# brunohs1993/Nanokappa

Measured on AMD Instinct MI355X. Metric: phonon-steps/sec (whole node), higher is better.
Workload: dtype f64

## Files before the change

nanokappa_amd/csrc/nk_device.h:

```cpp
#pragma once
#include <hip/hip_runtime.h>
#include <stdint.h>

#define NK_WG 256
#ifndef NK_NREP
#define NK_NREP 8
#endif
#define NK_PLANE_DOUBLES 6
#define NK_FACE_DOUBLES 16
#define NK_LDS_FACES 256
#define NK_LDS_RESFACES 64
#define NK_TAU_ROWS 3
#define NK_MAX_SEGMENTS 16384
#define NK_EMIT_CHUNK 128
#define NK_LREC 128
#define NK_NEWBORN 0x80000000u
#define NK_LOST 0x40000000u

#define NK_TAG_REFLECT 0x00000u
#define NK_TAG_EMIT 0x10000u
#define NK_TAG_RESAMP 0x20000u
#define NK_TAG_DICE 0x30000u
#define NK_TAG_INIT 0x40000u

// ... 8 lines not shown
    __host__ __device__ __forceinline__ explicit operator bool() const { return p != nullptr; }
};

template <bool NTS, bool PID>
struct NkBlock {
    static constexpr int NF = 4 + (NTS ? 1 : 0) + (PID ? 1 : 0);
    static constexpr int BD = NF * 64 + 32;
    static constexpr int O_Y = 64, O_Z = 128, O_OCC = 192, O_NTS = 256, O_PID = 64 * (NTS ? 5 : 4), O_W0 = 64 * NF;
    static __device__ __forceinline__ double *slot(double *s0, int64_t i) { return s0 + (i >> 6) * (int64_t)BD + (i & 63); }
    static __device__ __forceinline__ double *tile(double *s0, int64_t i0, int lane) { return s0 + (i0 >> 6) * (int64_t)BD + lane; }
    static __device__ __forceinline__ uint32_t *word(double *s0, int64_t i) { return reinterpret_cast<uint32_t *>(s0 + (i >> 6) * (int64_t)BD + O_W0) + (i & 63); }
};

struct __attribute__((aligned(16))) NkFacet {
    double cx, cy, cz;
    double nx, ny, nz;
    double tx, ty, tz;
    int32_t bc;
    int32_t partner;
    int32_t res;
    int32_t rough;
    int32_t pad[2];
};

struct __attribute__((aligned(64))) NkMode {
    double omega, vx, vy, vz;
    double E0;
    double tau[NK_TAU_ROWS];
};

struct NkDev {
    int32_t Q, J, NT, M;
    const NkMode *modetab;
    const NkMode *modetab_p;
    const int32_t *m2s;
    const int32_t *s2m;
    const int32_t *seg_nl;
    int32_t tau_row0;
    double tau_g[NK_TAU_ROWS];
    double tau_ig[NK_TAU_ROWS - 1];
    double T0, invT0;
    double c_hk;
    const double *tau;
    const double *Tgrid;
    int32_t nE;
    const double *Tarr, *Earr;
    double Tfill_lo, Tfill_hi;
    double hbar, kb, QV;
    double active_modes;
    int32_t F, Fc, NP;
    const float *tree_boxes;
    double tree_bound;
    const int32_t *tree_tags;
    const double *facet_skip;
    const double *tree_faces;
    int32_t tree_base[8];
    int32_t tree_top, tree_leaves;
    int32_t tree_nfam, tree_lds_fam0, tree_lds_off;
    int32_t NG;
    const double *planes;
    const double *faces;
    const NkFacet *facets;
    double tol;
    double bbox[6];
    int32_t box;
    double box_k[6];
    uint64_t box_ids;
    double inv_dt;
    const double *face_verts;
    const int32_t *facet_face_off;
    const int32_t *facet_face_idx;
    const double *facet_face_cdf;
    int32_t nS;
    const double *simplex_pts;
    const double *simplex_cdf;
    int32_t S, sv_kind, sv_axis, sv_interp;
    const double *centers;
    const double *sv_volume;
    double sv_lo, sv_invL;
    double *T_sv;
    const double *rbf_inv;
    int32_t rbf_P, rbf_used[3];
    double rbf_shift[3], rbf_scale[3];
    int32_t R, res_gen;
    const int32_t *res_facet;
    const double *res_T;
    const int32_t *res_face_off;
    const double *res_face_cdf;
    const double *res_face_verts;
    int32_t res_nf;
    int32_t res_lds;
    const double *enter_prob;
    double *res_counter;
    const double *ep_p;
    double *rc_p;
    int64_t rc_len;
    const double *res_roulette;
    int32_t *nleave_prev;
    uint64_t *sp_inbox;
    int32_t *sp_inbox_n;
    int32_t sp_icap;
    int32_t Fr;
    const double *specularity;
    const uint8_t *true_spec;
    const int32_t *spec_map;
    const double *roulette;
    const int32_t *roul_lut;
    int32_t roul_nlut;
    const int32_t *degen_j2;
    double dt;
    int32_t norm_fixed, T_ref_local;
    double particle_density, T_ref;
    uint64_t seed;
    int32_t rank, nranks;
    int64_t cap;
    int32_t nseg, segcap;
    int32_t *seg_count;
    int32_t *seg_new;
    int32_t *seg_lo;
    int32_t down;
    int32_t *seg_bound;
    NkField<double> x, y, z, occ, nts;
    NkField<uint32_t> w0;
    NkField<uint64_t> pid;
    int32_t part;
    int32_t lb;
    int32_t nlmax;
    int32_t nlrec;
    int32_t *ticket;
    int32_t *overflow;
    int32_t *halt;
    double *qx, *qy, *qz, *qocc, *qnts;
    uint32_t *qw0;
    uint64_t *qpid;
    int32_t *seg_evq;
    int32_t *ev_ticket;
    double2 *mig_buf;
    int32_t *mig_n;
    int32_t mig_cap;
    double *partials;
    int32_t NB;
    unsigned long long *stamps;
};

struct NkSlot { int64_t od, ow; };
__device__ __forceinline__ NkSlot nk_slot(const NkDev &d, int64_t i) {
    const int64_t b = i >> 6, l = i & 63;
    NkSlot s;
    s.od = b * (int64_t)d.x.blk + l;
    s.ow = b * (int64_t)d.w0.blk + l;
    return s;
}

__device__ __forceinline__ void nk_philox(uint32_t c0, uint32_t c1, uint32_t c2, uint32_t c3, uint32_t k0, uint32_t k1,
                                          uint32_t o[4]) {
#pragma unroll
    for (int r = 0; r < 10; ++r) {
        uint32_t hi0 = __umulhi(0xD2511F53u, c0), lo0 = 0xD2511F53u * c0;
        uint32_t hi1 = __umulhi(0xCD9E8D57u, c2), lo1 = 0xCD9E8D57u * c2;
        uint32_t n0 = hi1 ^ c1 ^ k0, n2 = hi0 ^ c3 ^ k1;
        c0 = n0; c1 = lo1; c2 = n2; c3 = lo0;
        k0 += 0x9E3779B9u; k1 += 0xBB67AE85u;
    }
    o[0] = c0; o[1] = c1; o[2] = c2; o[3] = c3;
}
__device__ __forceinline__ double nk_u53(uint32_t hi, uint32_t lo) {
    uint64_t w = ((uint64_t)hi << 32) | lo;
    return (double)(w >> 11) * (1.0 / 9007199254740992.0);
}
__device__ __forceinline__ void nk_uniform2_dev(uint64_t seed, uint64_t pid, uint32_t step, uint32_t tag, double &u0,
                                                double &u1) {
    uint32_t o[4];
    nk_philox((uint32_t)pid, (uint32_t)(pid >> 32), step, tag, (uint32_t)seed, (uint32_t)(seed >> 32), o);
    u0 = nk_u53(o[0], o[1]);
    u1 = nk_u53(o[2], o[3]);
}

__device__ __forceinline__ int nk_ss_left(const double *a, int n, double x) {
    int lo = 0, hi = n;
    while (lo < hi) { int mid = (lo + hi) >> 1; if (a[mid] < x) lo = mid + 1; else hi = mid; }
    return lo;
}
__device__ __forceinline__ int nk_ss_right(const double *a, int n, double x) {
    int lo = 0, hi = n;
    while (lo < hi) { int mid = (lo + hi) >> 1; if (a[mid] <= x) lo = mid + 1; else hi = mid; }
    return lo;
}
__device__ __forceinline__ int nk_ss_left_hint(const double *a, int n, double x, int hint) {
    int lo, hi;
    hint = hint < 0 ? 0 : (hint > n - 1 ? n - 1 : hint);
    if (a[hint] < x) {
        int stepw = 1;
        lo = hint + 1; hi = lo;
        while (hi < n && a[hi] < x) { lo = hi + 1; hi += stepw; stepw <<= 1; }
        if (hi > n) hi = n;
    } else {
        int stepw = 1;
        hi = hint; lo = hint;
        while (lo > 0 && !(a[lo - 1] < x)) { hi = lo - 1; lo -= stepw; stepw <<= 1; if (lo < 0) lo = 0; }
        if (lo > 0 && !(a[lo - 1] < x)) lo = 0;
    }
    while (lo < hi) { int mid = (lo + hi) >> 1; if (a[mid] < x) lo = mid + 1; else hi = mid; }
    return lo;
}
__device__ __forceinline__ double nk_interp_lin_hint(const double *xs, const double *ys, int n, double x, int hint, int &idx_out) {
    int idx = nk_ss_left_hint(xs, n, x, hint);
    idx_out = idx;
    idx = idx < 1 ? 1 : (idx > n - 1 ? n - 1 : idx);
    double xlo = xs[idx - 1], xhi = xs[idx], ylo = ys[idx - 1], yhi = ys[idx];
    return (yhi - ylo) / (xhi - xlo) * (x - xlo) + ylo;
}
__device__ __forceinline__ double nk_rcp(double x) {
    double y = __builtin_amdgcn_rcp(x);
    double e = __builtin_fma(-x, y, 1.0);
    y = __builtin_fma(y, e, y);
    e = __builtin_fma(-x, y, 1.0);
    return __builtin_fma(y, e, y);
}
__device__ __forceinline__ double nk_fma_c(double p, double r, double c) {
    double o;
    asm("v_fma_f64 %0, %1, %2, %3" : "=v"(o) : "v"(p), "v"(r), "v"(c));
    return o;
}
__device__ __forceinline__ double nk_exp(double x) {
    const double k = __builtin_rint(x * 1.4426950408889634);
    double r = __builtin_fma(-k, 6.93147180369123816490e-01, x);
    r = __builtin_fma(-k, 1.90821492927058770002e-10, r);
    double p = 1.6059043836821613e-10;
    p = nk_fma_c(p, r, 2.08767569878681e-09);
    p = nk_fma_c(p, r, 2.505210838544172e-08);
    p = nk_fma_c(p, r, 2.755731922398589e-07);
    p = nk_fma_c(p, r, 2.7557319223985893e-06);
    p = nk_fma_c(p, r, 2.48015873015873e-05);
    p = nk_fma_c(p, r, 1.984126984126984e-04);
    p = nk_fma_c(p, r, 0.001388888888888889);
    p = nk_fma_c(p, r, 0.008333333333333333);
    p = nk_fma_c(p, r, 0.041666666666666664);
    p = nk_fma_c(p, r, 0.16666666666666666);
    p = __builtin_fma(p, r, 0.5);
    p = __builtin_fma(p, r, 1.0);
    p = __builtin_fma(p, r, 1.0);
    const double kc = k < -2000.0 ? -2000.0 : (k > 2000.0 ? 2000.0 : k);
    return __builtin_ldexp(p, (int)kc);
}
__device__ __forceinline__ double nk_exp_small(double dl) {
    double p = 2.755731922398589e-07;
    p = nk_fma_c(p, dl, 2.7557319223985893e-06);
    p = nk_fma_c(p, dl, 2.48015873015873e-05);
    p = nk_fma_c(p, dl, 1.984126984126984e-04);
    p = nk_fma_c(p, dl, 0.001388888888888889);
    p = nk_fma_c(p, dl, 0.008333333333333333);
    p = nk_fma_c(p, dl, 0.041666666666666664);
    p = nk_fma_c(p, dl, 0.16666666666666666);
    p = __builtin_fma(p, dl, 0.5);
    p = __builtin_fma(p, dl, 1.0);
    p = __builtin_fma(p, dl, 1.0);
    return p;
}
__device__ __forceinline__ double nk_be(double a, double E0, double invT, double invT0) {
    if (!(a > 0.0) || !(invT > 0.0)) return 0.0;
    const double dl = a * (invT - invT0);
    double em1;
    if (fabs(dl) < 0.125) em1 = __builtin_fma(E0, nk_exp_small(dl), -1.0);
    else {
        const double xx = a * invT;
        if (!(xx < 700.0)) return 0.0;
        em1 = nk_exp(xx) - 1.0;
    }
    return nk_rcp(em1);
}
__device__ __forceinline__ double nk_occupation(const NkDev &d, double T, double omega, double E0) {
    if (!(T > 0.0) || !(omega > 0.0)) return 0.0;
    return nk_be(omega * d.c_hk, E0, 1.0 / T, d.invT0);
}
__device__ __forceinline__ double nk_interp_lin(const double *xs, const double *ys, int n, double x) {
    int idx = nk_ss_left(xs, n, x);
    idx = idx < 1 ? 1 : (idx > n - 1 ? n - 1 : idx);
    double xlo = xs[idx - 1], xhi = xs[idx], ylo = ys[idx - 1], yhi = ys[idx];
    return (yhi - ylo) / (xhi - xlo) * (x - xlo) + ylo;
}
__device__ __forceinline__ double nk_T_of_E(const NkDev &d, double E) {
    if (E < d.Earr[0]) return d.Tfill_lo;
    if (E > d.Earr[d.nE - 1]) return d.Tfill_hi;
    return nk_interp_lin(d.Earr, d.Tarr, d.nE, E);
}
__device__ __forceinline__ double nk_E_of_T(const NkDev &d, double T) {
    if (T < d.Tarr[0]) return d.Earr[0];
    if (T > d.Tarr[d.nE - 1]) return d.Earr[d.nE - 1];
    return nk_interp_lin(d.Tarr, d.Earr, d.nE, T);
}
struct NkTauWin {
    double g0, g1, g2, i0, i1;
    __device__ __forceinline__ void load(const NkDev &d, bool park) {
        g0 = d.tau_g[0]; g1 = d.tau_g[1]; g2 = d.tau_g[2]; i0 = d.tau_ig[0]; i1 = d.tau_ig[1];
        if (park) asm volatile("" : "+v"(g0), "+v"(g1), "+v"(g2), "+v"(i0), "+v"(i1));
    }
};
template <class SegModes>
__device__ __forceinline__ double nk_lifetime(const NkDev &d, const NkTauWin &w, double ta, double tb, double tc, double T, const SegModes &sm, int idx) {
    if (T > w.g0 && T <= w.g2) {
        const bool b = T > w.g1;
        const double glo = b ? w.g1 : w.g0;
        const double ig = b ? w.i1 : w.i0;
        const double t0 = b ? tb : ta, t1 = b ? tc : tb;
        const double y = (T - glo) * ig;
        return t0 * (1.0 - y) + t1 * y;
    }
    const int NT = d.NT;
    const double *g = d.Tgrid;
    if (!(T >= g[0]) || !(T <= g[NT - 1])) return __builtin_nan("");
    int i = (int)((T - g[0]) / (g[1] - g[0]));
    i = i < 0 ? 0 : (i > NT - 1 ? NT - 1 : i);
    while (i < NT && g[i] < T) ++i;
    while (i > 0 && g[i - 1] >= T) --i;
    i -= 1;
    i = i < 0 ? 0 : (i > NT - 2 ? NT - 2 : i);
    const double y = (T - g[i]) / (g[i + 1] - g[i]);
    const int mode = sm.mode(idx);
    const double t0 = d.tau[(int64_t)i * d.M + mode];
    const double t1 = d.tau[(int64_t)(i + 1) * d.M + mode];
    return t0 * (1.0 - y) + t1 * y;
}

struct __attribute__((aligned(16))) NkSv { double c, T, slope, invT; };
struct NkSvTab {
    const double *cen;
// ... 544 lines not shown
```

nanokappa_amd/csrc/nk_engine.hip:

```cpp
#include <hip/hip_runtime.h>
#include <dlfcn.h>
#include <math.h>
#include <stdio.h>
#include <stdlib.h>
#include <string.h>
#include <algorithm>
#include <functional>
#include <queue>
#include <string>
#include <type_traits>
#include <chrono>
#include <time.h>
#include <vector>

#include <rccl/rccl.h>

#include "../../include/nanokappa_hip.h"
#include "nk_kernels.h"
#include "nk_field.h"
#include "nk_fgroups.h"
#include "nk_modes.h"
#include "nk_group.h"
#ifndef NK_PLAIN_IN_ENGINE
extern template __global__ void k_sweep<1, false, false, false, false, true, 1>(NkDev, uint32_t, int, int);
extern template __global__ void k_sweep<1, false, false, false, false, true, 2>(NkDev, uint32_t, int, int);
extern template __global__ void k_sweep<1, false, false, false, false, false, 1>(NkDev, uint32_t, int, int);
extern template __global__ void k_sweep<1, false, false, false, false, false, 2>(NkDev, uint32_t, int, int);
extern template __global__ void k_sweep<1, false, false, false, false, true, 1, true>(NkDev, uint32_t, int, int);
extern template __global__ void k_sweep<1, false, false, false, false, true, 2, true>(NkDev, uint32_t, int, int);
extern template __global__ void k_sweep<1, false, false, false, false, false, 1, true>(NkDev, uint32_t, int, int);
extern template __global__ void k_sweep<1, false, false, false, false, false, 2, true>(NkDev, uint32_t, int, int);
#endif

struct NkRccl {
    void *lib = nullptr;
    ncclResult_t (*GetUniqueId)(ncclUniqueId *) = nullptr;
    ncclResult_t (*CommInitRank)(ncclComm_t *, int, ncclUniqueId, int) = nullptr;
    ncclResult_t (*AllReduce)(const void *, void *, size_t, ncclDataType_t, ncclRedOp_t, ncclComm_t, hipStream_t) = nullptr;
    ncclResult_t (*CommDestroy)(ncclComm_t) = nullptr;
    ncclResult_t (*CommCount)(const ncclComm_t, int *) = nullptr;
    ncclResult_t (*CommUserRank)(const ncclComm_t, int *) = nullptr;
    ncclResult_t (*CommAbort)(ncclComm_t) = nullptr;
};

static thread_local std::string g_create_error;

struct nk_ctx {
    int device = 0;
    hipStream_t stream = nullptr;
    std::string err;
    NkDev d;
    std::vector<void *> allocs;
    std::vector<void *> pallocs;
    void *store_buf = nullptr;
    size_t store_pad = 0;
    bool store_pid = false;
    bool store_nts = true;
    bool mesh_box = false;
    bool box_forbidden = false;
    int32_t *anomalies = nullptr;
    bool have_material = false, have_mesh = false, have_sv = false, have_params = false;
    int64_t step = 0;
    bool pending_relax = false;
    int g_sweep = 0;
    std::vector<int32_t> h_seg_count;
    std::vector<hipEvent_t> evpool;
    int g_sweep_key = -1;
    size_t g_sweep_lds = 0;
    int layout_key = -1;
    std::vector<double> h_enter_prob;
    int64_t spec_M = 0;
    double *spec_v = nullptr, *spec_om = nullptr, *spec_dl = nullptr, *spec_svx = nullptr;
    int32_t *spec_rank = nullptr;
    double spec_vmax = 0.0;
    NkSpecMode *spec_modes = nullptr;
    int32_t *spec_in = nullptr, *spec_out = nullptr;
    unsigned long long *spec_count = nullptr;
    double *ks_kv = nullptr, *ks_mat = nullptr;
    double ks_tol[3] = {0, 0, 0};
    int64_t ks_Q = 0;
    int64_t spec_cap = 0;
    int64_t spec_last = 0;
    int rb_Fr = 0;
    double *rb_k2 = nullptr, *rb_nin = nullptr, *rb_eta = nullptr, *rb_sub = nullptr, *rb_spec = nullptr, *rb_roul = nullptr;
    uint8_t *rb_ts = nullptr;
    unsigned int *rb_map = nullptr;
    std::vector<int32_t> rb_facet;
    int64_t o2o_first = 0;
    bool stepped = false;
    int64_t emitted_for = -1;
    std::vector<double> h_vg;
    std::vector<int32_t> h_m2s, h_s2m;
    int32_t *m2s_dev = nullptr, *s2m_dev = nullptr, *nl_dev = nullptr;
    unsigned int *rbar = nullptr;
    bool walked = false;
    int64_t ev_lds_set = -1;
    int map_nseg = 0;
    NkMode *modetab_p = nullptr;
    int64_t modetab_p_len = 0;
    void *inbox = nullptr, *inbox_n = nullptr;
    void *mig_buf = nullptr, *mig_n = nullptr;
    double *ep_p = nullptr, *rc_p = nullptr;
    int rm_nseg = 0, rm_nlmax = 0;
    void *pin = nullptr;
    size_t pin_bytes = 0;
    int32_t halt_words[4] = {0, 0, 0, 0};
    double *acc = nullptr;
    double *hist = nullptr;
    int hist_cap = 0;
    nk_params params;
    nk_timing timing;
    NkRccl rccl;
    ncclComm_t comm = nullptr;
    int comm_rank = -1, comm_nranks = 0;
    double comm_selftest = 0.0;
    int num_cu = 256;
    std::vector<int32_t> h_ffo, h_ffi;
    std::vector<double> h_fcdf, h_verts;
    std::vector<double> h_rbf_inv;
    std::vector<NkFacet> host_facets;
    const double *d_omega = nullptr, *d_vg = nullptr;
    std::vector<double> h_Tgrid;
    double T_lo = 0.0, T_hi = 0.0;
    int32_t band_B = 0;
    int32_t *band_map = nullptr;
    double *band_slabs = nullptr;
    size_t band_slabs_n = 0;
    double *band_rows_d = nullptr;
    size_t band_rows_n = 0;
    std::vector<double> band_rows;
    std::vector<int64_t> band_steps;
    NkFieldHost field;
    NkFGroupsHost fgroups;
    int64_t map_gen = 0;
    NkModesHost modes;
    double res_T_max = 0.0;
};

#define NK_HIP(call)                                                                                   \
    do {                                                                                               \
        hipError_t e_ = (call);                                                                        \
        if (e_ != hipSuccess) {                                                                        \
            ctx->err = std::string(#call) + ": " + hipGetErrorString(e_);                              \
            return NK_ERR_HIP;                                                                         \
        }                                                                                              \
    } while (0)
#define NK_ARG(cond, msg)                                                                              \
    do {                                                                                               \
        if (!(cond)) { ctx->err = msg; return NK_ERR_ARG; }                                            \
    } while (0)

template <class T>
static int nk_upload(nk_ctx *ctx, const T *src, size_t n, const T **dst, bool particle = false) {
    void *p = nullptr;
    size_t bytes = (n ? n : 1) * sizeof(T);
    NK_HIP(hipMalloc(&p, bytes));
    (particle ? ctx->pallocs : ctx->allocs).push_back(p);
    if (src && n) NK_HIP(hipMemcpy(p, src, n * sizeof(T), hipMemcpyHostToDevice));
    else NK_HIP(hipMemset(p, 0, bytes));
    *dst = (const T *)p;
    return NK_OK;
}
#define NK_UP(src, n, dst)                                                                             \
    do { int rc_ = nk_upload(ctx, src, n, dst); if (rc_) return rc_; } while (0)

static inline bool nk_layout_soa() { return false; }
static inline int nk_particle_bytes(bool with_pid, bool with_nts) { return 36 + (with_nts ? 8 : 0) + (with_pid ? 8 : 0); }
static inline size_t nk_store_bytes(int64_t cap, bool with_pid, bool with_nts) {
    const int64_t nblk = (cap + 63) / 64;
    const int nf = 4 + (with_nts ? 1 : 0) + (with_pid ? 1 : 0);
    const int bd = nf * 64 + 32;
    const size_t bytes = nk_layout_soa() ? (size_t)nblk * 64 * (nf * 8 + 4) : (size_t)nblk * bd * 8;
    return bytes ? bytes : 64;
}
static void nk_point_fields(NkDev &d, double *b, int64_t cap, bool with_pid, bool with_nts) {
    const int64_t nblk = (cap + 63) / 64;
    const int nf = 4 + (with_nts ? 1 : 0) + (with_pid ? 1 : 0);
    const int bd = nf * 64 + 32;
    if (nk_layout_soa()) {
        const int64_t n = nblk * 64;
        int k = 4;
        d.x = {b, 64}; d.y = {b + n, 64}; d.z = {b + 2 * n, 64}; d.occ = {b + 3 * n, 64};
        d.nts = {with_nts ? b + (k++) * n : nullptr, 64};
        d.pid = {with_pid ? (uint64_t *)(b + (k++) * n) : nullptr, 64};
        d.w0 = {(uint32_t *)(b + k * n), 64};
    } else {
        int k = 4;
        d.x = {b, bd}; d.y = {b + 64, bd}; d.z = {b + 128, bd}; d.occ = {b + 192, bd};
        d.nts = {with_nts ? b + 64 * (k++) : nullptr, bd};
        d.pid = {with_pid ? (uint64_t *)(b + 64 * (k++)) : nullptr, bd};
        d.w0 = {(uint32_t *)(b + 64 * k), 2 * bd};
    }
}
static int nk_alloc_fields(nk_ctx *ctx, NkDev &d, int64_t cap, bool with_pid, bool with_nts) {
    const size_t bytes = nk_store_bytes(cap, with_pid, with_nts);
    void *buf = nullptr;
    const size_t pad = getenv("NK_STORE_PAD_KB") ? (size_t)atol(getenv("NK_STORE_PAD_KB")) * 1024 : 0;
    NK_HIP(hipMalloc(&buf, bytes + pad));
    ctx->pallocs.push_back(buf);
    NK_HIP(hipMemsetAsync(buf, 0, bytes + pad, ctx->stream));
    ctx->store_buf = buf; ctx->store_pad = pad; ctx->store_pid = with_pid; ctx->store_nts = with_nts;
    nk_point_fields(d, (double *)((char *)buf + pad), cap, with_pid, with_nts);
    return NK_OK;
}
template <class T>
static int nk_field_download(nk_ctx *ctx, const NkDev &d, const NkField<T> &f, std::vector<T> &out) {
    out.resize((size_t)d.cap);
    const int64_t nblk = d.cap / 64;
    if (nblk == 0) return NK_OK;
    NK_HIP(hipMemcpy2D(out.data(), 64 * sizeof(T), f.p, (size_t)f.blk * sizeof(T), 64 * sizeof(T), (size_t)nblk, hipMemcpyDeviceToHost));
    return NK_OK;
}
template <class T>
static int nk_field_upload(nk_ctx *ctx, const NkDev &d, const NkField<T> &f, const T *src) {
    const int64_t nblk = d.cap / 64;
    if (nblk == 0) return NK_OK;
    NK_HIP(hipMemcpy2D(f.p, (size_t)f.blk * sizeof(T), src, 64 * sizeof(T), 64 * sizeof(T), (size_t)nblk, hipMemcpyHostToDevice));
    return NK_OK;
}

static inline int nk_geom_mode(const nk_ctx *ctx) { return (ctx->d.F <= NK_LDS_FACES && ctx->d.Fc <= NK_LDS_FACES) ? 1 : 2; }
static inline bool nk_want_split(const nk_ctx *ctx);
static inline size_t nk_lds(const nk_ctx *ctx, bool geom, int kind = 0) {
    const NkDev &d = ctx->d;
    const int gm = geom ? nk_geom_mode(ctx) : 0;
    return nk_lds_bytes(d.S, d.R, d.F, d.NP, d.Fc, gm, kind, (gm == 1 && d.res_lds) ? d.res_nf : 0, d.rbf_P, d.nlrec, nk_want_split(ctx) ? 0 : 1);
}
#define NK_GEOM_LAUNCH(kernel, grid, lds, ...)                                                        \
    do {                                                                                               \
        if (nk_geom_mode(ctx) == 1) kernel<1><<<grid, NK_WG, lds, ctx->stream>>>(__VA_ARGS__);         \
        else kernel<2><<<grid, NK_WG, lds, ctx->stream>>>(__VA_ARGS__);                                \
    } while (0)
#define NK_EMIT_LAUNCH(kernel, grid, lds, ...)                                                        \
    do {                                                                                               \
        if (ctx->d.box) kernel<1, true><<<grid, NK_WG, lds, ctx->stream>>>(__VA_ARGS__);               \
        else if (nk_geom_mode(ctx) == 1) kernel<1, false><<<grid, NK_WG, lds, ctx->stream>>>(__VA_ARGS__);   \
        else kernel<2, false><<<grid, NK_WG, lds, ctx->stream>>>(__VA_ARGS__);                         \
    } while (0)
static inline int nk_sweep_grid(const nk_ctx *ctx) { return ctx->num_cu * 8; }
#define NK_SWEEP_CASE(G, R, B, P, S, lrec, STMT) { if (lrec) { auto KERNEL = k_sweep<G, R, B, P, S, true>; STMT; } else { auto KERNEL = k_sweep<G, R, B, P, S, false>; STMT; } }
#define NK_SWEEP_CASE_FAST(lrec, fast, STMT)                                                                                   \
    { if (lrec) { if ((fast) == 1) { auto KERNEL = k_sweep<1, false, false, false, false, true, 1>; STMT; } else { auto KERNEL = k_sweep<1, false, false, false, false, true, 2>; STMT; } } \
      else { if ((fast) == 1) { auto KERNEL = k_sweep<1, false, false, false, false, false, 1>; STMT; } else { auto KERNEL = k_sweep<1, false, false, false, false, false, 2>; STMT; } } }
#define NK_SWEEP_CASE_S(G, R, B, P, split, lrec, STMT) { if (split) NK_SWEEP_CASE(G, R, B, P, true, lrec, STMT) else NK_SWEEP_CASE(G, R, B, P, false, lrec, STMT) }
#define NK_SWEEP_CASE_RP(G, B, rough, pid, split, lrec, STMT)                                         \
    { if (rough) NK_SWEEP_CASE_S(G, true, B, true, split, lrec, STMT) else if (pid) NK_SWEEP_CASE_S(G, false, B, true, split, lrec, STMT) else NK_SWEEP_CASE_S(G, false, B, false, split, lrec, STMT) }
#define NK_SWEEP_CASE_BOX(R, B, P, lrec, STMT) { if (lrec) { auto KERNEL = k_sweep<1, R, B, P, false, true, 0, true>; STMT; } else { auto KERNEL = k_sweep<1, R, B, P, false, false, 0, true>; STMT; } }
#define NK_SWEEP_CASE_BOX_RP(B, rough, pid, lrec, STMT)                                               \
    { if (rough) NK_SWEEP_CASE_BOX(true, B, true, lrec, STMT) else if (pid) NK_SWEEP_CASE_BOX(false, B, true, lrec, STMT) else NK_SWEEP_CASE_BOX(false, B, false, lrec, STMT) }
#define NK_SWEEP_CASE_FAST_BOX(lrec, fast, STMT)                                                                               \
    { if (lrec) { if ((fast) == 1) { auto KERNEL = k_sweep<1, false, false, false, false, true, 1, true>; STMT; } else { auto KERNEL = k_sweep<1, false, false, false, false, true, 2, true>; STMT; } } \
      else { if ((fast) == 1) { auto KERNEL = k_sweep<1, false, false, false, false, false, 1, true>; STMT; } else { auto KERNEL = k_sweep<1, false, false, false, false, false, 2, true>; STMT; } } }
#define NK_SWEEP_DISPATCH(gm, rough, rbf, pid, split, lrec, STMT)                                     \
    do {                                                                                               \
        const int fast_ = ((gm) == 1 && !(rough) && !(rbf) && !(pid) && !(split)) ? nk_sweep_fast(ctx) : 0;   \
        if (ctx->d.box && (gm) == 1 && !(split)) {                                                     \
            if (fast_) { NK_SWEEP_CASE_FAST_BOX(lrec, fast_, STMT) break; }                            \
            if (rbf) NK_SWEEP_CASE_BOX_RP(true, rough, pid, lrec, STMT) else NK_SWEEP_CASE_BOX_RP(false, rough, pid, lrec, STMT)   \
            break;                                                                                     \
        }                                                                                              \
        if (fast_) { NK_SWEEP_CASE_FAST(lrec, fast_, STMT) break; }                                    \
        if ((gm) == 1) { if (rbf) NK_SWEEP_CASE_RP(1, true, rough, pid, split, lrec, STMT) else NK_SWEEP_CASE_RP(1, false, rough, pid, split, lrec, STMT) }   \
        else { if (rbf) NK_SWEEP_CASE_RP(2, true, rough, pid, split, lrec, STMT) else NK_SWEEP_CASE_RP(2, false, rough, pid, split, lrec, STMT) }             \
    } while (0)
static inline int nk_sweep_fast(const nk_ctx *ctx) {
    const NkDev &d = ctx->d;
    if (getenv("NK_NO_FAST")) return 0;
    return (d.sv_kind == 0 && d.T_ref_local && (d.sv_interp == 0 || d.sv_interp == 1)) ? 1 + d.sv_interp : 0;
}
static inline bool nk_want_lrec(const nk_ctx *ctx) { return ctx->d.nlrec > 0; }
#define NK_EVENTS_CASE(G, R, B, P, STMT) { auto KERNEL = k_events<G, R, B, P>; STMT; }
#define NK_EVENTS_CASE_RP(G, B, rough, pid, STMT)                                                     \
    { if (rough) NK_EVENTS_CASE(G, true, B, true, STMT) else if (pid) NK_EVENTS_CASE(G, false, B, true, STMT) else NK_EVENTS_CASE(G, false, B, false, STMT) }
#define NK_EVENTS_DISPATCH(gm, rough, rbf, pid, STMT)                                                 \
    do {                                                                                               \
        if ((gm) == 1) { if (rbf) NK_EVENTS_CASE_RP(1, true, rough, pid, STMT) else NK_EVENTS_CASE_RP(1, false, rough, pid, STMT) }   \
        else { if (rbf) NK_EVENTS_CASE_RP(2, true, rough, pid, STMT) else NK_EVENTS_CASE_RP(2, false, rough, pid, STMT) }             \
    } while (0)

static int nk_update_tau_window(nk_ctx *ctx, bool force) {
    NkDev &d = ctx->d;
    if (!ctx->have_material) return NK_OK;
    const std::vector<double> &g = ctx->h_Tgrid;
    const double Tm = 0.5 * (ctx->T_lo + ctx->T_hi);
    int i = (int)(std::lower_bound(g.begin(), g.end(), Tm) - g.begin()) - 1;
    if (i < 0) i = 0;
    int row0 = (i + 1 < d.NT && ctx->T_hi - g[std::min(i + 1, d.NT - 1)] > g[i] - ctx->T_lo) ? i : i - 1;
    if (row0 > d.NT - NK_TAU_ROWS) row0 = d.NT - NK_TAU_ROWS;
    if (row0 < 0) row0 = 0;
    const bool window_ok = d.tau_row0 >= 0 && ctx->T_lo > g[d.tau_row0] &&
                           ctx->T_hi <= g[std::min(d.tau_row0 + NK_TAU_ROWS - 1, d.NT - 1)];
    const bool window_best = d.tau_row0 == row0;
    const bool t0_ok = d.T0 > 0.0 && fabs(ctx->T_lo - d.T0) <= 0.02 * d.T0 && fabs(ctx->T_hi - d.T0) <= 0.02 * d.T0;
    const bool t0_best = d.T0 > 0.0 && fabs(Tm - d.T0) <= 0.002 * d.T0;
    if (!force && (window_ok || window_best) && (t0_ok || t0_best)) return NK_OK;
    d.T0 = Tm > 0.0 ? Tm : 300.0;
    d.invT0 = 1.0 / d.T0;
    d.c_hk = d.hbar / d.kb;
    NkMode *tp = nullptr;
    if (d.part && d.nseg > 0 && d.m2s) {
        const int64_t need = (int64_t)d.nseg * d.nlmax;
        if (need > ctx->modetab_p_len) {
            if (ctx->modetab_p) hipFree(ctx->modetab_p);
            ctx->modetab_p = nullptr; ctx->modetab_p_len = 0;
            NK_HIP(hipMalloc((void **)&ctx->modetab_p, (size_t)need * sizeof(NkMode)));
            NK_HIP(hipMemset(ctx->modetab_p, 0, (size_t)need * sizeof(NkMode)));
            ctx->modetab_p_len = need;
        }
        tp = ctx->modetab_p;
    }
    d.modetab_p = tp;
    k_build_modetab<<<(d.M + 255) / 256, 256, 0, ctx->stream>>>(ctx->d_omega, ctx->d_vg, d.tau, d.M, d.NT, row0, d.c_hk, d.invT0,
                                                                  d.nseg > 0 ? d.nseg : 1, d.nlmax, d.m2s, (NkMode *)d.modetab, tp);
    NK_HIP(hipGetLastError());
    d.tau_row0 = row0;
    ctx->timing.tau_rebuilds += 1;
    for (int k = 0; k < NK_TAU_ROWS; ++k) d.tau_g[k] = (row0 + k < d.NT) ? g[row0 + k] : INFINITY;
    for (int k = 0; k + 1 < NK_TAU_ROWS; ++k) d.tau_ig[k] = 1.0 / (d.tau_g[k + 1] - d.tau_g[k]);
    if (d.NT < NK_TAU_ROWS) d.tau_g[0] = INFINITY;
    return NK_OK;
}

static void nk_track_T(nk_ctx *ctx, const double *T, int S) {
    double lo = T[0], hi = T[0];
    for (int i = 1; i < S; ++i) { lo = std::min(lo, T[i]); hi = std::max(hi, T[i]); }
    ctx->T_lo = lo; ctx->T_hi = hi;
}

extern "C" {

const char *nk_last_error(const nk_ctx *ctx) { return ctx ? ctx->err.c_str() : g_create_error.c_str(); }

int nk_device_count(void) {
    int ndev = 0;
    return hipGetDeviceCount(&ndev) == hipSuccess ? ndev : 0;
}

int nk_create(nk_ctx **out, int device_id, uint64_t seed) {
    if (!out) { g_create_error = "nk_create: out is NULL"; return NK_ERR_ARG; }
    *out = nullptr;
    int ndev = 0;
    hipError_t e = hipGetDeviceCount(&ndev);
    if (e != hipSuccess || ndev <= 0) {
        g_create_error = std::string("nk_create: no HIP device available (") + hipGetErrorString(e) +
                         "); this library has no CPU fallback";
        return NK_ERR_NODEVICE;
    }
    if (device_id < 0 || device_id >= ndev) { g_create_error = "nk_create: device_id out of range"; return NK_ERR_ARG; }
    nk_ctx *ctx = new nk_ctx();
    memset(&ctx->d, 0, sizeof(NkDev));
    memset(&ctx->params, 0, sizeof(nk_params));
    memset(&ctx->timing, 0, sizeof(nk_timing));
    ctx->device = device_id;
    if ((e = hipSetDevice(device_id)) != hipSuccess || (e = hipStreamCreate(&ctx->stream)) != hipSuccess) {
        g_create_error = std::string("nk_create: ") + hipGetErrorString(e);
        delete ctx;
        return NK_ERR_HIP;
    }
    hipDeviceProp_t prop;
    if (hipGetDeviceProperties(&prop, device_id) == hipSuccess) {
        ctx->num_cu = prop.multiProcessorCount;
        if (strncmp(prop.gcnArchName, "gfx950", 6) != 0) {
            g_create_error = std::string("nk_create: device is ") + prop.gcnArchName + ", this build targets gfx950 only";
            hipStreamDestroy(ctx->stream);
            delete ctx;
            return NK_ERR_NODEVICE;
        }
    }
    ctx->d.seed = seed;
    ctx->d.rank = 0;
    ctx->d.nranks = 1;
    ctx->d.tau_row0 = -1;
    ctx->d.stamps = nullptr;
    ctx->params.dt = 1.0; ctx->params.T_ref_local = 1; ctx->params.flux_every = 10; ctx->params.contains_every = 100;
    ctx->d.dt = 1.0; ctx->d.inv_dt = 1.0; ctx->d.T_ref_local = 1;
    const int32_t *p32 = nullptr;
    int rc;
    if ((rc = nk_upload<int32_t>(ctx, nullptr, 16, &p32))) {
        g_create_error = ctx->err;
        delete ctx;
        return rc;
    }
    ctx->d.halt = (int32_t *)p32;
    ctx->d.overflow = (int32_t *)p32 + 4;
    ctx->d.ticket = (int32_t *)p32 + 5;
    ctx->d.ev_ticket = (int32_t *)p32 + 6;
    ctx->anomalies = (int32_t *)p32 + 7;
    *out = ctx;
    return NK_OK;
}
// ... 704 lines not shown
    NK_HIP(hipStreamSynchronize(ctx->stream));
    std::vector<int32_t> cnt((size_t)d.nseg);
    NK_HIP(hipMemcpy(cnt.data(), d.seg_count, (size_t)d.nseg * 4, hipMemcpyDeviceToHost));
    int64_t live = 0;
    for (int c : cnt) live += c;
    ctx->h_seg_count = cnt;
    if (!want_all) { h.x.resize((size_t)live); return NK_OK; }
    std::vector<double> bd;
    std::vector<uint32_t> bw;
    std::vector<uint64_t> bu;
    auto keep = [&](const auto &all, auto *dst) {
        for (int sgm = 0; sgm < d.nseg; ++sgm) {
            memcpy(dst, all.data() + (size_t)sgm * d.segcap, (size_t)cnt[sgm] * sizeof(*dst));
            dst += cnt[sgm];
        }
    };
    h.x.resize(live); h.y.resize(live); h.z.resize(live); h.occ.resize(live); h.nts.resize(live);
    h.mode.resize(live); h.facet.resize(live); h.pid.assign(live, 0);
    std::vector<uint32_t> w0((size_t)live);
    int rc;
    if ((rc = nk_field_download(ctx, d, d.x, bd))) return rc; keep(bd, h.x.data());
    if ((rc = nk_field_download(ctx, d, d.y, bd))) return rc; keep(bd, h.y.data());
    if ((rc = nk_field_download(ctx, d, d.z, bd))) return rc; keep(bd, h.z.data());
    if ((rc = nk_field_download(ctx, d, d.occ, bd))) return rc; keep(bd, h.occ.data());
    std::vector<int32_t> bfc;
    if (d.nts) { if ((rc = nk_field_download(ctx, d, d.nts, bd))) return rc; keep(bd, h.nts.data()); }
    else {
        if (ctx->have_material && ctx->have_mesh && ctx->have_sv && d.modetab) {
            double *dn = nullptr; int32_t *df = nullptr;
            NK_HIP(hipMalloc((void **)&dn, (size_t)d.cap * 8));
            if (hipMalloc((void **)&df, (size_t)d.cap * 4) != hipSuccess) { hipFree(dn); ctx->err = "nk_gather_live: out of memory"; return NK_ERR_HIP; }
            hipMemsetAsync(dn, 0, (size_t)d.cap * 8, ctx->stream); hipMemsetAsync(df, 0xff, (size_t)d.cap * 4, ctx->stream);
            k_next_hit<1><<<nk_sweep_grid(ctx), NK_WG, nk_lds(ctx, true), ctx->stream>>>(d, dn, df);
            bd.resize((size_t)d.cap); bfc.resize((size_t)d.cap);
            hipError_t e1 = hipGetLastError();
            if (e1 == hipSuccess) e1 = hipMemcpy(bd.data(), dn, (size_t)d.cap * 8, hipMemcpyDeviceToHost);
            if (e1 == hipSuccess) e1 = hipMemcpy(bfc.data(), df, (size_t)d.cap * 4, hipMemcpyDeviceToHost);
            hipFree(dn); hipFree(df);
            if (e1 != hipSuccess) { ctx->err = std::string("nk_gather_live: ") + hipGetErrorString(e1); return NK_ERR_HIP; }
            keep(bd, h.nts.data());
        } else { std::fill(h.nts.begin(), h.nts.end(), 0.0); }
    }
    if ((rc = nk_field_download(ctx, d, d.w0, bw))) return rc; keep(bw, w0.data());
    if (d.pid) { if ((rc = nk_field_download(ctx, d, d.pid, bu))) return rc; keep(bu, h.pid.data()); }
    const uint32_t lbmask = (1u << d.lb) - 1u;
    int64_t k = 0;
    for (int sgm = 0; sgm < d.nseg; ++sgm)
        for (int j = 0; j < cnt[sgm]; ++j, ++k) {
            const uint32_t idx = w0[(size_t)k] & lbmask;
            h.mode[(size_t)k] = d.part ? ctx->h_s2m[(size_t)sgm * d.nlmax + idx] : (int32_t)idx;
            if (d.nts) h.facet[(size_t)k] = (int32_t)(w0[(size_t)k] >> d.lb) - 1;
            else h.facet[(size_t)k] = (w0[(size_t)k] & NK_LOST) ? -1 : (bfc.empty() ? 0 : bfc[(size_t)sgm * d.segcap + j]);
        }
    return NK_OK;
}

static int nk_scatter(nk_ctx *ctx, int64_t N, const double *x, const double *y, const double *z, const int32_t *mode,
                      const double *occ, const double *n_ts, const int32_t *facet, const uint64_t *pid, uint64_t pid_offset) {
    if (ctx) ctx->emitted_for = -1;
    NkDev &d = ctx->d;
    const int M = d.M;
    for (int64_t i = 0; i < N; ++i) NK_ARG(mode[i] >= 0 && mode[i] < M, "nk_upload_particles: mode index out of range");
    std::vector<int64_t> order((size_t)N);
    std::vector<int64_t> start((size_t)d.nseg + 1, 0);
    if (d.part) {
        const std::vector<int32_t> &m2s = ctx->h_m2s;
        for (int64_t i = 0; i < N; ++i) start[(size_t)(m2s[(size_t)mode[i]] % d.nseg) + 1] += 1;
        for (int sgm = 0; sgm < d.nseg; ++sgm) start[(size_t)sgm + 1] += start[(size_t)sgm];
        std::vector<int64_t> key((size_t)N);
        for (int64_t i = 0; i < N; ++i) { order[(size_t)i] = i; key[(size_t)i] = (int64_t)(m2s[(size_t)mode[i]] % d.nseg) * ((int64_t)d.nlmax + 1) + m2s[(size_t)mode[i]] / d.nseg; }
        std::stable_sort(order.begin(), order.end(), [&](int64_t a, int64_t b) { return key[(size_t)a] < key[(size_t)b]; });
    } else {
        std::vector<int64_t> mstart((size_t)M + 1, 0);
        for (int64_t i = 0; i < N; ++i) mstart[(size_t)mode[i] + 1] += 1;
        for (int m = 0; m < M; ++m) mstart[(size_t)m + 1] += mstart[(size_t)m];
        std::vector<int64_t> cur(mstart.begin(), mstart.end() - 1);
        for (int64_t i = 0; i < N; ++i) order[(size_t)cur[(size_t)mode[i]]++] = i;
        for (int sgm = 0; sgm <= d.nseg; ++sgm) start[(size_t)sgm] = (N * sgm) / d.nseg;
    }
    std::vector<int32_t> cnt((size_t)d.nseg);
    for (int sgm = 0; sgm < d.nseg; ++sgm) {
        cnt[(size_t)sgm] = (int32_t)(start[(size_t)sgm + 1] - start[(size_t)sgm]);
        NK_ARG(cnt[(size_t)sgm] <= d.segcap, "nk_upload_particles: segment capacity too small");
    }
    auto put = [&](const auto *src, const auto &field) -> int {
        typedef typename std::remove_const<typename std::remove_pointer<decltype(src)>::type>::type T;
        std::vector<T> all((size_t)d.cap, T(0));
        for (int sgm = 0; sgm < d.nseg; ++sgm) {
            const int64_t lo = start[(size_t)sgm], n = cnt[(size_t)sgm];
            T *o = all.data() + (size_t)sgm * d.segcap;
            for (int64_t k = 0; k < n; ++k) o[k] = src[order[(size_t)(lo + k)]];
        }
        return nk_field_upload(ctx, d, field, all.data());
    };
    int rc;
    if ((rc = put(x, d.x)) || (rc = put(y, d.y)) || (rc = put(z, d.z)) || (rc = put(occ, d.occ))) return rc;
    if (n_ts && d.nts && (rc = put(n_ts, d.nts))) return rc;
    {
        std::vector<uint32_t> w0((size_t)N);
        for (int64_t i = 0; i < N; ++i) {
            const int32_t fc = facet ? facet[i] : -1;
            NK_ARG(fc >= -1 && fc < d.Fc, "nk_upload_particles: facet index out of range");
            const uint32_t idx = d.part ? (uint32_t)(ctx->h_m2s[(size_t)mode[i]] / d.nseg) : (uint32_t)mode[i];
            w0[(size_t)i] = d.nts ? (((uint32_t)(fc + 1) << d.lb) | idx) : (((facet && fc < 0) ? NK_LOST : 0u) | idx);
        }
        if ((rc = put((const uint32_t *)w0.data(), d.w0))) return rc;
    }
    if (d.pid) {
        if (pid) { if ((rc = put(pid, d.pid))) return rc; }
        else {
            std::vector<uint64_t> ids((size_t)N);
            for (int64_t i = 0; i < N; ++i) ids[(size_t)i] = pid_offset + (uint64_t)i;
            if ((rc = put((const uint64_t *)ids.data(), d.pid))) return rc;
        }
    }
    NK_HIP(hipMemcpy(d.seg_count, cnt.data(), (size_t)d.nseg * 4, hipMemcpyHostToDevice));
    if (d.seg_lo) NK_HIP(hipMemset(d.seg_lo, 0, (size_t)d.nseg * 4));
    ctx->walked = false;
    ctx->h_seg_count = cnt;
    return NK_OK;
}

static inline bool nk_want_pid(const nk_ctx *ctx) { return ctx->d.Fr > 0 || ctx->params.track_ids != 0; }
static inline bool nk_want_split(const nk_ctx *ctx) {
    if (const char *e = getenv("NK_SPLIT")) return atoi(e) != 0;
    return ctx->have_mesh && !(ctx->d.F <= NK_LDS_FACES && ctx->d.Fc <= NK_LDS_FACES);
}
static inline bool nk_want_part(const nk_ctx *ctx) { return !getenv("NK_NO_PARTITION"); }

static int nk_sweep_blocks(nk_ctx *ctx) {
    NkDev &d = ctx->d;
    if (!(ctx->have_material && ctx->have_mesh && ctx->have_sv)) return ctx->num_cu * NK_SWEEP_OCC;
    const int gm_ = nk_geom_mode(ctx);
    const bool rough_ = d.Fr > 0, rbf_ = d.sv_interp == 3, pid_ = nk_want_pid(ctx), split_ = nk_want_split(ctx);
    const bool lrec_ = nk_want_lrec(ctx);
    const int key = gm_ | (rough_ << 2) | (rbf_ << 3) | (pid_ << 4) | (split_ << 5) | (lrec_ << 6) | (nk_sweep_fast(ctx) << 7) | ((d.box ? 1 : 0) << 9);
    const size_t lds_w = nk_lds(ctx, true, pid_ ? 3 : 2);
    if (ctx->g_sweep == 0 || ctx->g_sweep_key != key || ctx->g_sweep_lds != lds_w) {
        int per_cu = 0;
        hipError_t e_ = hipSuccess;
        NK_SWEEP_DISPATCH(gm_, rough_, rbf_, pid_, split_, lrec_, (e_ = hipOccupancyMaxActiveBlocksPerMultiprocessor(&per_cu, KERNEL, NK_WG, lds_w)));
        if (e_ != hipSuccess || per_cu < 1) per_cu = 1;
        if (per_cu > 8) per_cu = 8;
        { const int bound = NK_SWEEP_BOUND(gm_, rough_, rbf_, split_); if (per_cu > bound) per_cu = bound; }
        if (const char *e = getenv("NK_SWEEP_PER_CU")) { int v = atoi(e); if (v >= 1 && v < per_cu) per_cu = v; }
        ctx->g_sweep = ctx->num_cu * per_cu;
        ctx->g_sweep_key = key;
        ctx->g_sweep_lds = lds_w;
        if (getenv("NK_VERBOSE")) fprintf(stderr, "[nanokappa_hip] sweep: %d workgroups per CU (occupancy query rc %d), %zu B LDS each\n", per_cu, (int)e_, lds_w);
    }
    return ctx->g_sweep;
}

static inline int nk_mode_seg(const nk_ctx *ctx, int m, int nseg) {
    return (ctx->map_nseg == nseg && !ctx->h_m2s.empty()) ? ctx->h_m2s[(size_t)m] % nseg : m % nseg;
}

static int nk_build_mode_map(nk_ctx *ctx) {
    NkDev &d = ctx->d;
    if (ctx->m2s_dev) { hipFree(ctx->m2s_dev); ctx->m2s_dev = nullptr; }
    if (ctx->s2m_dev) { hipFree(ctx->s2m_dev); ctx->s2m_dev = nullptr; }
    if (ctx->nl_dev) { hipFree(ctx->nl_dev); ctx->nl_dev = nullptr; }
    d.m2s = nullptr; d.s2m = nullptr; d.seg_nl = nullptr;
    ctx->h_m2s.clear(); ctx->h_s2m.clear(); ctx->map_nseg = 0;
    ctx->map_gen += 1;
    if (d.M <= 0 || d.nseg <= 0) return NK_OK;
    const int M = d.M, nseg = d.nseg, nlmax = d.nlmax;
    const bool plain = !d.part;
    std::vector<int32_t> nl((size_t)nseg, 0);
    ctx->h_m2s.assign((size_t)M, 0);
    ctx->h_s2m.assign((size_t)nseg * nlmax, -1);
    auto place = [&](int m, int seg) {
        const int l = nl[(size_t)seg]++;
        ctx->h_m2s[(size_t)m] = l * nseg + seg;
        ctx->h_s2m[(size_t)seg * nlmax + l] = m;
    };
    if (plain) {
        for (int m = 0; m < M; ++m) place(m, m % nseg);
    } else {
        std::vector<double> rate((size_t)M, 0.0);
        std::vector<char> active((size_t)M, 1);
        const bool have_v = ctx->h_vg.size() == (size_t)M * 3;
        if (have_v) {
            double inv[3] = {0, 0, 0};
            if (ctx->have_mesh) for (int a = 0; a < 3; ++a) { const double e = d.bbox[3 + a] - d.bbox[a]; inv[a] = e > 0.0 ? 1.0 / e : 0.0; }
            for (int m = 0; m < M; ++m) {
                const double *v = &ctx->h_vg[3 * (size_t)m];
                active[(size_t)m] = (v[0] != 0.0 || v[1] != 0.0 || v[2] != 0.0) ? 1 : 0;
                rate[(size_t)m] = fabs(v[0]) * inv[0] + fabs(v[1]) * inv[1] + fabs(v[2]) * inv[2];
            }
        }
        double rsum = 0.0; int64_t nact = 0;
        for (int m = 0; m < M; ++m) if (active[(size_t)m]) { rsum += rate[(size_t)m]; ++nact; }
        const double rmean = nact > 0 && rsum > 0.0 ? rsum / (double)nact : 1.0;
        const double beta = getenv("NK_EVENT_WEIGHT") ? atof(getenv("NK_EVENT_WEIGHT")) : 0.45;
        std::vector<double> share((size_t)nseg, 1.0);
        const int g = ctx->g_sweep, per_cu = ctx->num_cu > 0 ? g / ctx->num_cu : 0;
        const double skew = getenv("NK_AGE_SKEW") ? atof(getenv("NK_AGE_SKEW")) : 0.14;
        if (per_cu > 1 && g == per_cu * ctx->num_cu && nseg == g * (NK_WG / 64) && skew != 0.0)
            for (int sg = 0; sg < nseg; ++sg) {
                const int k = (sg / (NK_WG / 64)) / ctx->num_cu;
                share[(size_t)sg] = 1.0 + skew * (1.0 - 2.0 * (double)k / (double)(per_cu - 1));
            }
        std::vector<int32_t> order((size_t)M);
        for (int m = 0; m < M; ++m) order[(size_t)m] = m;
        std::stable_sort(order.begin(), order.end(), [&](int32_t a, int32_t b) {
            if (active[(size_t)a] != active[(size_t)b]) return active[(size_t)a] > active[(size_t)b];
            return rate[(size_t)a] > rate[(size_t)b];
        });
        typedef std::pair<double, int> Key;
        std::priority_queue<Key, std::vector<Key>, std::greater<Key>> heap;
        std::vector<double> load((size_t)nseg, 0.0);
        for (int sg = 0; sg < nseg; ++sg) heap.push(Key(0.0, sg));
        int k = 0;
        for (; k < M && active[(size_t)order[(size_t)k]]; ++k) {
            const int m = order[(size_t)k];
            int sg = -1;
            while (!heap.empty()) { const Key top = heap.top(); heap.pop(); if (nl[(size_t)top.second] < nlmax) { sg = top.second; break; } }
            if (sg < 0) { ctx->err = "nk_build_mode_map: the segments' slot ranges are full (internal sizing error)"; return NK_ERR_ARG; }
            place(m, sg);
            load[(size_t)sg] += 1.0 + beta * rate[(size_t)m] / rmean;
            heap.push(Key(load[(size_t)sg] / share[(size_t)sg], sg));
        }
        std::priority_queue<std::pair<int, int>, std::vector<std::pair<int, int>>, std::greater<std::pair<int, int>>> room;
        for (int sg = 0; sg < nseg; ++sg) room.push(std::make_pair((int)nl[(size_t)sg], sg));
        for (; k < M; ++k) {
            const std::pair<int, int> top = room.top(); room.pop();
            if (top.first >= nlmax) { ctx->err = "nk_build_mode_map: no room for the inactive modes (internal sizing error)"; return NK_ERR_ARG; }
            place(order[(size_t)k], top.second);
            room.push(std::make_pair(top.first + 1, top.second));
        }
    }
    NK_HIP(hipMalloc((void **)&ctx->m2s_dev, (size_t)M * 4));
    NK_HIP(hipMalloc((void **)&ctx->s2m_dev, (size_t)nseg * nlmax * 4));
    NK_HIP(hipMalloc((void **)&ctx->nl_dev, (size_t)nseg * 4));
    NK_HIP(hipMemcpy(ctx->m2s_dev, ctx->h_m2s.data(), (size_t)M * 4, hipMemcpyHostToDevice));
    NK_HIP(hipMemcpy(ctx->s2m_dev, ctx->h_s2m.data(), (size_t)nseg * nlmax * 4, hipMemcpyHostToDevice));
    NK_HIP(hipMemcpy(ctx->nl_dev, nl.data(), (size_t)nseg * 4, hipMemcpyHostToDevice));
    d.m2s = ctx->m2s_dev; d.s2m = ctx->s2m_dev; d.seg_nl = ctx->nl_dev;
    ctx->map_nseg = nseg;
    return NK_OK;
}

static int64_t nk_spawn_bound(const nk_ctx *ctx, int nseg) {
    const NkDev &d = ctx->d;
    if (d.R <= 0) return 0;
    if (d.res_gen == 2) return 4 * (ctx->o2o_first / std::max(nseg, 1) + 64);
    std::vector<int64_t> per((size_t)nseg, 0);
    for (int r = 0; r < d.R; ++r)
        for (int m = 0; m < d.M; ++m) per[(size_t)(nk_mode_seg(ctx, m, nseg))] += (int64_t)floor(ctx->h_enter_prob[(size_t)r * d.M + m]) + 1;
    int64_t mx = 0;
    for (int64_t v : per) mx = std::max(mx, v);
    return (mx + d.nranks - 1) / d.nranks + d.R;
}

static int nk_place_store(nk_ctx *ctx) {
    NkDev &d = ctx->d;
    ctx->timing.place_tries = 0; ctx->timing.place_gbps = 0.0; ctx->timing.place_worst_gbps = 0.0;
    const int tries = getenv("NK_PLACE_TRIES") ? atoi(getenv("NK_PLACE_TRIES")) : 1;
    const size_t bytes = nk_store_bytes(d.cap, ctx->store_pid, ctx->store_nts);
    const int pbytes = nk_particle_bytes(ctx->store_pid, ctx->store_nts);
    const size_t min_mb = getenv("NK_PLACE_MIN_MB") ? (size_t)atol(getenv("NK_PLACE_MIN_MB")) : 64;
    const bool force = getenv("NK_PLACE_FORCE") != nullptr;
    if (tries < 1 || !ctx->store_buf || ctx->store_pad != 0 || bytes < (min_mb << 20) || d.nseg <= 0 || d.segcap < 64) return NK_OK;
    size_t free_b = 0, total_b = 0;
    NK_HIP(hipMemGetInfo(&free_b, &total_b));
    const auto wall0 = std::chrono::steady_clock::now();
    const int g = std::max(1, std::min(nk_sweep_blocks(ctx), (d.nseg + NK_WG / 64 - 1) / (NK_WG / 64)));
    const int tiles = d.segcap / 64;
    hipEvent_t e0, e1;
    NK_HIP(hipEventCreate(&e0)); NK_HIP(hipEventCreate(&e1));
    auto probe = [&](void *buf, double &ms) -> int {
        NkDev t = d;
        nk_point_fields(t, (double *)buf, d.cap, ctx->store_pid, ctx->store_nts);
        k_probe_place<<<g, NK_WG, 0, ctx->stream>>>(t, tiles);
        NK_HIP(hipEventRecord(e0, ctx->stream));
        for (int k = 0; k < 3; ++k) k_probe_place<<<g, NK_WG, 0, ctx->stream>>>(t, tiles);
        NK_HIP(hipEventRecord(e1, ctx->stream));
        NK_HIP(hipGetLastError());
        NK_HIP(hipStreamSynchronize(ctx->stream));
        float f = 0.f;
        NK_HIP(hipEventElapsedTime(&f, e0, e1));
        ms = (double)f / 3.0;
        return NK_OK;
    };
    std::vector<void *> cand(1, ctx->store_buf);
    std::vector<double> ms(1, 0.0);
    int rc = probe(cand[0], ms[0]);
    while (!rc && (int)cand.size() < tries) {
        double lo = ms[0], hi = ms[0];
        for (double v : ms) { lo = std::min(lo, v); hi = std::max(hi, v); }
        if (hi > 1.12 * lo && !force) break;
        if (bytes * cand.size() > free_b / 3) break;
        if (std::chrono::duration<double, std::milli>(std::chrono::steady_clock::now() - wall0).count() > 1000.0) break;
        void *buf = nullptr;
        if (hipMalloc(&buf, bytes) != hipSuccess) { (void)hipGetLastError(); break; }
        cand.push_back(buf); ms.push_back(0.0);
        if (hipMemsetAsync(buf, 0, bytes, ctx->stream) != hipSuccess) { rc = NK_ERR_HIP; ctx->err = "nk_place_store: hipMemsetAsync failed"; break; }
        rc = probe(buf, ms.back());
    }
    hipEventDestroy(e0); hipEventDestroy(e1);
    size_t best = 0, worst = 0;
    for (size_t k = 1; k < cand.size(); ++k) { if (ms[k] < ms[best]) best = k; if (ms[k] > ms[worst]) worst = k; }
    if (force) best = cand.size() - 1;
    if (!rc && best != 0 && (ms[best] < 0.97 * ms[0] || force)) {
        if (hipMemcpyAsync(cand[best], cand[0], bytes, hipMemcpyDeviceToDevice, ctx->stream) != hipSuccess ||
// ... 399 lines not shown
    NkFieldHost &F = ctx->field;
    NK_HIP(hipMemcpy(st, F.status, 4 * sizeof(long long), hipMemcpyDeviceToHost));
    if (st[2] || st[3]) {
        long long z[2] = {0, 0};
        NK_HIP(hipMemcpy(F.status + 2, z, sizeof(z), hipMemcpyHostToDevice));
        ctx->err = std::string(who) + ": field overflow: " + std::to_string(st[2]) + " term(s) of E above B_E = " + std::to_string(F.BE) +
                   " eV, " + std::to_string(st[3]) + " term(s) of F above B_F = " + std::to_string(F.BF) +
                   " (occupations outside the material's temperature range?); they were left out of the sums";
        return NK_ERR_CAPACITY;
    }
    return NK_OK;
}

static int nk_fgroups_refresh(nk_ctx *ctx) {
    const hipError_t e = nk_fgroups_permute(ctx->fgroups, ctx->d, ctx->map_gen, ctx->stream);
    if (e != hipSuccess) {
        (void)hipGetLastError();
        ctx->err = "nk_set_field_groups: the table in the segments' order (" + std::to_string((long long)ctx->d.nseg * ctx->d.nlmax * 4) +
                   " bytes): " + hipGetErrorString(e);
        return NK_ERR_HIP;
    }
    return NK_OK;
}
static int nk_fgroups_sample(nk_ctx *ctx, bool state) {
    NkFGroupsHost &Gh = ctx->fgroups;
    NK_HIP(nk_fgroups_pass(Gh, ctx->field, ctx->d, state, nk_lds(ctx, false), ctx->num_cu, ctx->stream));
    if (ctx->comm) {
        ncclResult_t nrc = ctx->rccl.AllReduce(Gh.grid, Gh.grid, ((size_t)Gh.lines + 1) * 8, ncclInt64, ncclSum, ctx->comm, ctx->stream);
        if (nrc != ncclSuccess) { ctx->err = "ncclAllReduce of the field groups' grid failed"; return NK_ERR_COMM; }
    }
    return NK_OK;
}
static std::string nk_fgroups_overflow(const nk_ctx *ctx, const char *who, long long ovE, long long ovF) {
    return std::string(who) + ": field groups overflow: " + std::to_string(ovE) + " term(s) of E above B_E = " + std::to_string(ctx->field.BE) +
           " eV, " + std::to_string(ovF) + " term(s) of F above B_F = " + std::to_string(ctx->field.BF) +
           " (occupations outside the material's temperature range?); they were left out of the sums";
}
static int nk_fgroups_status(nk_ctx *ctx, long long st[8], const char *who) {
    NkFGroupsHost &Gh = ctx->fgroups;
    NK_HIP(hipMemcpy(st, Gh.status, 8 * sizeof(long long), hipMemcpyDeviceToHost));
    if (st[NK_FG_ST_OVE] || st[NK_FG_ST_OVF]) {
        long long z[2] = {0, 0};
        NK_HIP(hipMemcpy(Gh.status + NK_FG_ST_OVE, z, sizeof(z), hipMemcpyHostToDevice));
        ctx->err = nk_fgroups_overflow(ctx, who, st[NK_FG_ST_OVE], st[NK_FG_ST_OVF]);
        return NK_ERR_CAPACITY;
    }
    return NK_OK;
}

static double nk_modes_T_hi(const nk_ctx *ctx) {
    const NkDev &d = ctx->d;
    double T_hi = std::max(ctx->h_Tgrid.empty() ? 0.0 : ctx->h_Tgrid.back(), d.Tfill_hi);
    if (!d.T_ref_local) T_hi = std::max(T_hi, d.T_ref);
    if (d.R > 0) T_hi = std::max(T_hi, ctx->res_T_max);
    return T_hi;
}
static int nk_modes_refresh(nk_ctx *ctx) {
    NkModesHost &Mo = ctx->modes;
    const NkDev &d = ctx->d;
    const int fe = ctx->params.flux_every;
    NK_ARG(fe > 0 && Mo.cfg.every % fe == 0, "modes: every must be a positive multiple of flux_every");
    const double T_hi = nk_modes_T_hi(ctx);
    if (T_hi != Mo.T_hi) nk_modes_bound(Mo, d.kb, T_hi);
    double cap = (double)d.cap;
    if (ctx->comm) { int rc = nk_comm_allreduce(ctx, &cap, 1); if (rc) return rc; }
    const int64_t slots = std::max<int64_t>((int64_t)cap, Mo.cfg.capacity);
    if (slots != Mo.capacity) nk_modes_scale(Mo, slots);
    return NK_OK;
}
static int nk_modes_sample(nk_ctx *ctx, bool state) {
    NkModesHost &Mo = ctx->modes;
    NK_HIP(nk_modes_pass(Mo, ctx->d, state, nk_lds(ctx, false), ctx->num_cu, ctx->stream));
    if (ctx->comm) {
        ncclResult_t nrc = ctx->rccl.AllReduce(Mo.hdr, Mo.hdr, 8, ncclInt64, ncclSum, ctx->comm, ctx->stream);
        if (nrc != ncclSuccess) { ctx->err = "ncclAllReduce of the mode tally's header failed"; return NK_ERR_COMM; }
    }
    return NK_OK;
}
static int nk_modes_status(nk_ctx *ctx, long long st[4], const char *who) {
    NkModesHost &Mo = ctx->modes;
    NK_HIP(hipMemcpy(st, Mo.status, 4 * sizeof(long long), hipMemcpyDeviceToHost));
    if (st[2]) {
        long long z = 0;
        NK_HIP(hipMemcpy(Mo.status + 2, &z, sizeof(z), hipMemcpyHostToDevice));
        ctx->err = std::string(who) + ": mode tally overflow: " + std::to_string(st[2]) + " term(s) of E above B_E = " + std::to_string(Mo.BE) +
                   " eV (occupations outside the material's temperature range?); they were left out of the sums";
        return NK_ERR_CAPACITY;
    }
    return NK_OK;
}

extern "C++" {
template <typename TI, typename TO>
static void nk_modes_transpose(const TI *in, TO *out, int M, int S) {
    for (int m = 0; m < M; ++m)
        for (int s = 0; s < S; ++s) out[(size_t)s * M + m] = (TO)in[(size_t)m * S + s];
}
}

static int nk_batch_hist(nk_ctx *ctx, int32_t nsteps) {
    const int HROW = ctx->d.NB + 2 * ctx->d.S + 8;
    if (nsteps > ctx->hist_cap) {
        if (ctx->hist) hipHostFree(ctx->hist);
        ctx->hist = nullptr;
        ctx->hist_cap = 0;
        const int rows_alloc = nsteps < 1024 ? 1024 : nsteps;
        NK_HIP(hipHostMalloc((void **)&ctx->hist, (size_t)rows_alloc * HROW * sizeof(double), hipHostMallocMapped));
        ctx->hist_cap = rows_alloc;
    }
    ctx->timing.batches += 1;
    memset(ctx->hist, 0, (size_t)nsteps * HROW * sizeof(double));
    return NK_OK;
}
static int nk_batch_prelude(nk_ctx *ctx, int64_t stepno, bool &pending, bool &flushed, int64_t *launches) {
    NkDev &d = ctx->d;
    if (!(ctx->params.contains_every > 0 && (stepno % ctx->params.contains_every) == 0 && d.nS > 0)) return NK_OK;
    const bool anchors = ctx->walked && d.seg_lo;
    { int rcn_ = nk_normalize(ctx, 1); if (rcn_) return rcn_; }
    int64_t n = anchors ? 1 : 0;
    if (pending) {
        k_relax<<<nk_sweep_grid(ctx), NK_WG, nk_lds(ctx, false), ctx->stream>>>(d, 1);
        pending = false;
        flushed = true;
        n += 1;
    }
    NK_GEOM_LAUNCH(k_contains, nk_sweep_grid(ctx), nk_lds(ctx, true), d, (uint32_t)stepno);
    if (launches) *launches += n + 1;
    return NK_OK;
}
static int nk_batch_collect(nk_ctx *ctx, int32_t nsteps, std::vector<double> &h, int32_t *done) {
    const NkDev &d = ctx->d;
    const int S = d.S, NB = d.NB, HROW = NB + 2 * S + 8;
    h.resize((size_t)nsteps * HROW);
    memcpy(h.data(), ctx->hist, (size_t)nsteps * HROW * sizeof(double));
    int32_t nd = 0;
    while (nd < nsteps && h[(size_t)nd * HROW + NB + 2 * S + 1] != 0.0) ++nd;
    if (nd > 0) for (int k_ = 0; k_ < 4; ++k_) ctx->halt_words[k_] = (int32_t)h[(size_t)(nd - 1) * HROW + NB + 2 * S + 4 + k_];
    else NK_HIP(hipMemcpy(ctx->halt_words, d.halt, 16, hipMemcpyDeviceToHost));
    *done = nd;
    return NK_OK;
}
static void nk_batch_leave(nk_ctx *ctx, int32_t nsteps, int32_t nd, bool tail_emit, bool relax0, bool flushed_first) {
    const int32_t *hw_ = ctx->halt_words;
    ctx->emitted_for = (tail_emit && nd == nsteps && !hw_[0] && !hw_[2] && !hw_[3]) ? ctx->step + nsteps : -1;
    if (nd > 0) ctx->pending_relax = true;
    else ctx->pending_relax = relax0 && !flushed_first;
}

static int nk_step_batch(nk_ctx *ctx, int32_t nsteps, std::vector<double> &h, int32_t *done) {
    NkDev &d = ctx->d;
    const int S = d.S, R = d.R, NB = d.NB;
    const int HROW = NB + 2 * S + 8;
    { int rch_ = nk_batch_hist(ctx, nsteps); if (rch_) return rch_; }
    const size_t lds_g = nk_lds(ctx, true), lds_w = nk_lds(ctx, true, d.pid ? 3 : 2), lds_e = nk_lds(ctx, true, 1);
    const int gm_ = nk_geom_mode(ctx);
    const bool rough_ = d.Fr > 0, rbf_ = d.sv_interp == 3, pid_ = (bool)d.pid, split_ = d.qx != nullptr;
    const bool lrec_ = nk_want_lrec(ctx);
    (void)nk_sweep_blocks(ctx);
    const int g_sweep = ctx->g_sweep < (d.nseg + 3) / 4 ? ctx->g_sweep : (d.nseg + 3) / 4;
    const int g_emit = ctx->num_cu * 8 < (d.nseg + 3) / 4 ? ctx->num_cu * 8 : (d.nseg + 3) / 4;
    const int g_ev = split_ ? ctx->num_cu * NK_EV_PER_CU : 0;
    size_t lds_ev = lds_g;
    d.tree_lds_fam0 = d.tree_nfam; d.tree_lds_off = 0;
    if (split_ && gm_ == 2 && d.NG > 0 && d.tree_nfam > 0) {
        const size_t off = (lds_g + 15) & ~(size_t)15, fixed = off + (size_t)NK_EVENTS_PEND * NK_EV_WG * 4 + 1024;
        size_t budget = (size_t)160 * 1024 / NK_EV_PER_CU > fixed ? (size_t)160 * 1024 / NK_EV_PER_CU - fixed : 0;
        if (const char *e = getenv("NK_EVENTS_TREE_LDS")) { const size_t v = (size_t)atol(e); if (v < budget) budget = v; }
        for (int l = 0; l <= d.tree_top; ++l) {
            const int fam0 = d.tree_base[l] >> 2;
            const size_t bytes = (size_t)(d.tree_nfam - fam0) * NK_TREE_FAMILY_FLOATS * 4;
            if (bytes <= budget) { d.tree_lds_fam0 = fam0; d.tree_lds_off = (int32_t)off; lds_ev = off + bytes; break; }
        }
        if (getenv("NK_VERBOSE") && ctx->timing.batches <= 1)
            fprintf(stderr, "[nanokappa_hip] k_events: families %d .. %d of the face tree in LDS (%zu B of %zu B per workgroup)\n", d.tree_lds_fam0, d.tree_nfam, lds_ev - off, lds_ev);
    }
    const int rows = g_sweep + g_ev;
    const int nev = nsteps < 4 ? 0 : 4;
    if (ctx->evpool.empty()) {
        ctx->evpool.resize(16 * 4 + 2);
        for (auto &e : ctx->evpool) NK_HIP(hipEventCreate(&e));
    }
    hipEvent_t *ev = ctx->evpool.data();
    hipEvent_t t0 = ctx->evpool[64], t1 = ctx->evpool[65];
    const bool relax0 = ctx->pending_relax;
    NK_HIP(hipEventRecord(t0, ctx->stream));
    bool pending = ctx->pending_relax;
    std::vector<char> relax_flushed((size_t)nsteps, 0);
    const bool tail_emit = R > 0 && d.res_gen != 2 && !getenv("NK_NO_TAIL_EMIT");
    const size_t lds_t = lds_e > (size_t)(NK_WG * 8 + 16) ? lds_e : (size_t)(NK_WG * 8 + 16);
    bool emitted_ahead = tail_emit && ctx->emitted_for == ctx->step;
    ctx->emitted_for = -1;
    ctx->timing.emit_fused = tail_emit ? 1 : 0;
    const bool alt = d.seg_lo && gm_ == 1 && !split_ && !getenv("NK_NO_ALTERNATE");
    if (!alt) { int rcn_ = nk_normalize(ctx); if (rcn_) return rcn_; }
    d.down = 0;
    const bool bands_ = ctx->band_B > 0;
    std::vector<int> band_s;
    if (bands_) {
        const int fe = ctx->params.flux_every;
        int nflux = 0;
        for (int s = 0; s < nsteps; ++s) nflux += (fe > 0 && ((ctx->step + s + 1) % fe) == 0) ? 1 : 0;
        if (nflux > 0) { int rcb_ = nk_band_ensure(ctx, nflux); if (rcb_) return rcb_; }
    }
    for (int s = 0; s < nsteps; ++s) {
        const int64_t stepno = ctx->step + s;
        const uint32_t step = (uint32_t)stepno;
        { bool fl_ = false; int rcp_ = nk_batch_prelude(ctx, stepno, pending, fl_, nullptr); if (rcp_) return rcp_; if (fl_) relax_flushed[(size_t)s] = 1; }
        const int fe = ctx->params.flux_every;
        const int do_flux = (fe > 0 && ((stepno + 1) % fe) == 0) ? 1 : 0;
        if (s < nev) NK_HIP(hipEventRecord(ev[4 * s], ctx->stream));
        if (R > 0 && d.res_gen == 2) k_emit_one_to_one<<<ctx->num_cu * 4, NK_WG, 0, ctx->stream>>>(d, step);
        if (R > 0 && !emitted_ahead) NK_EMIT_LAUNCH(k_emit, g_emit, lds_e, d, step);
        if (s < nev) NK_HIP(hipEventRecord(ev[4 * s + 1], ctx->stream));
        {
            const int rl = pending ? 1 : 0;
            if (alt) { d.down = (int32_t)(stepno & 1); ctx->walked = true; }
            NK_SWEEP_DISPATCH(gm_, rough_, rbf_, pid_, split_, lrec_, (KERNEL<<<g_sweep, NK_WG, lds_w, ctx->stream>>>(d, step, rl, do_flux)));
            d.down = 0;
            if (split_) {
                k_events_begin<<<1, 1024, 0, ctx->stream>>>(d);
                const int64_t ev_key = (int64_t)lds_ev * 64 + (gm_ | (rough_ << 2) | (rbf_ << 3) | (pid_ << 4));
                if (ctx->ev_lds_set != ev_key) {
                    hipError_t ea_ = hipSuccess;
                    NK_EVENTS_DISPATCH(gm_, rough_, rbf_, pid_, (ea_ = hipFuncSetAttribute((const void *)KERNEL, hipFuncAttributeMaxDynamicSharedMemorySize, (int)lds_ev)));
                    NK_HIP(ea_);
                    ctx->ev_lds_set = ev_key;
                }
                NK_EVENTS_DISPATCH(gm_, rough_, rbf_, pid_, (KERNEL<<<g_ev, NK_EV_WG, lds_ev, ctx->stream>>>(d, step, do_flux, g_sweep)));
                k_events_end<<<(d.nseg + 255) / 256, 256, 0, ctx->stream>>>(d);
            }
        }
        if (d.mig_buf) k_deliver<<<g_emit, NK_WG, 0, ctx->stream>>>(d, 1);
        if (s < nev) NK_HIP(hipEventRecord(ev[4 * s + 2], ctx->stream));
        if (bands_ && do_flux) {
            int rcb_ = nk_band_pass(ctx, false, ctx->band_rows_d + band_s.size() * 4 * (size_t)S * ctx->band_B);
            if (rcb_) return rcb_;
            band_s.push_back(s);
        }
        if (ctx->field.on && do_flux && ((stepno + 1) % ctx->field.cfg.every) == 0) {
            int rcf_ = nk_field_sample(ctx, false);
            if (rcf_) return rcf_;
            NK_HIP(nk_field_accumulate(ctx->field, ctx->comm ? ctx->comm_nranks : 1, ctx->stream));
            if (ctx->fgroups.on) {
                int rcg_ = nk_fgroups_sample(ctx, false);
                if (rcg_) return rcg_;
                NK_HIP(nk_fgroups_accumulate(ctx->fgroups, ctx->field, ctx->comm ? ctx->comm_nranks : 1, ctx->stream));
            }
        }
        if (ctx->modes.on && do_flux && ((stepno + 1) % ctx->modes.cfg.every) == 0) {
            int rcm_ = nk_modes_sample(ctx, false);
            if (rcm_) return rcm_;
            NK_HIP(nk_modes_accumulate(ctx->modes, ctx->comm ? ctx->comm_nranks : 1, ctx->num_cu, ctx->stream));
        }
        double *hrow = ctx->hist + (size_t)s * HROW;
        const bool ahead = tail_emit;
        if (ctx->comm) {
            if (ahead) NK_EMIT_LAUNCH(k_tail, NB + g_emit, lds_t, d, step + 1u, rows, ctx->acc, hrow, do_flux, 0, NB);
            else k_reduce<<<NB, NK_WG, 0, ctx->stream>>>(d, rows, ctx->acc, hrow, do_flux, 0);
            ncclResult_t nrc = ctx->rccl.AllReduce(ctx->acc, ctx->acc, (size_t)NB + 2, ncclDouble, ncclSum, ctx->comm, ctx->stream);
            if (nrc != ncclSuccess) { ctx->err = "ncclAllReduce failed"; return NK_ERR_COMM; }
            k_update<<<1, NK_WG, 0, ctx->stream>>>(d, ctx->acc, hrow, do_flux);
        } else if (ahead) {
            NK_EMIT_LAUNCH(k_tail, NB + g_emit, lds_t, d, step + 1u, rows, ctx->acc, hrow, do_flux, 1, NB);
        } else {
            k_reduce<<<NB, NK_WG, 0, ctx->stream>>>(d, rows, ctx->acc, hrow, do_flux, 1);
        }
        emitted_ahead = ahead;
        if (s < nev) NK_HIP(hipEventRecord(ev[4 * s + 3], ctx->stream));
        pending = true;
        if ((s & 63) == 0) NK_HIP(hipGetLastError());
    }
    NK_HIP(hipEventRecord(t1, ctx->stream));
    NK_HIP(hipGetLastError());
    if (nsteps <= 4) { hipError_t q_; while ((q_ = hipStreamQuery(ctx->stream)) == hipErrorNotReady) { } if (q_ != hipSuccess) { ctx->err = std::string("hipStreamQuery: ") + hipGetErrorString(q_); return NK_ERR_HIP; } }
    NK_HIP(hipStreamSynchronize(ctx->stream));
    { int rcc_ = nk_batch_collect(ctx, nsteps, h, done); if (rcc_) return rcc_; }
#ifdef NK_STAMPS
    if (d.stamps) {
        std::vector<unsigned long long> st((size_t)d.nseg * 16);
        NK_HIP(hipMemcpy(st.data(), d.stamps, st.size() * 8, hipMemcpyDeviceToHost));
        double sum[7] = {0, 0, 0, 0, 0, 0, 0};
        for (int sgm = 0; sgm < d.nseg; ++sgm) for (int k = 0; k < 7; ++k) sum[k] += (double)st[(size_t)sgm * 8 + k];
        double tot = 0; for (int k = 0; k < 6; ++k) tot += sum[k];
        {
            std::vector<unsigned long long> clk;
            for (int sgm = 0; sgm < d.nseg; ++sgm) clk.push_back(st[(size_t)sgm * 8 + 7]);
            std::sort(clk.begin(), clk.end());
            unsigned long long e0 = ~0ull, x1 = 0;
            std::vector<double> pro, loop, epi, fin;
            for (int sgm = 0; sgm < d.nseg; ++sgm) {
                const unsigned long long *w = &st[((size_t)d.nseg + sgm) * 8];
                if (!w[0] || !w[3]) continue;
                e0 = std::min(e0, w[0]); x1 = std::max(x1, w[3]);
            }
            for (int sgm = 0; sgm < d.nseg; ++sgm) {
                const unsigned long long *w = &st[((size_t)d.nseg + sgm) * 8];
                if (!w[0] || !w[3]) continue;
                pro.push_back((double)(w[1] - w[0]) * 0.01); loop.push_back((double)(w[2] - w[1]) * 0.01);
                epi.push_back((double)(w[3] - w[2]) * 0.01); fin.push_back((double)(w[3] - e0) * 0.01);
            }
            auto q = [](std::vector<double> v, const char *nm) {
                if (v.empty()) return;
                std::sort(v.begin(), v.end());
                double sm = 0; for (double x : v) sm += x;
                fprintf(stderr, "[stamps] %s [us]: min %.1f  p10 %.1f  median %.1f  mean %.1f  p90 %.1f  max %.1f\n", nm, v.front(), v[v.size() / 10], v[v.size() / 2], sm / v.size(), v[v.size() * 9 / 10], v.back());
            };
            {
                unsigned long long m0 = ~0ull, m3 = 0;
                std::vector<double> a, b, c, fin2;
                for (int sgm = 0; sgm < d.nseg; ++sgm) { const unsigned long long *w = &st[((size_t)d.nseg + sgm) * 8 + 4]; if (w[0] && w[3]) { m0 = std::min(m0, w[0]); m3 = std::max(m3, w[3]); } }
                for (int sgm = 0; sgm < d.nseg; ++sgm) {
                    const unsigned long long *w = &st[((size_t)d.nseg + sgm) * 8 + 4];
                    if (!w[0] || !w[3]) continue;
                    a.push_back((double)(w[1] - w[0]) * 0.01); b.push_back((double)(w[2] - w[1]) * 0.01); c.push_back((double)(w[3] - w[2]) * 0.01);
                    fin2.push_back((double)(w[3] - m0) * 0.01);
                }
                auto q2 = [](std::vector<double> v, const char *nm) {
                    if (v.empty()) return;
                    std::sort(v.begin(), v.end());
                    double sm = 0; for (double x : v) sm += x;
                    fprintf(stderr, "[stamps] k_emit %s [us]: min %.1f  median %.1f  mean %.1f  p90 %.1f  max %.1f\n", nm, v.front(), v[v.size() / 2], sm / v.size(), v[v.size() * 9 / 10], v.back());
                };
                if (!a.empty()) {
                    fprintf(stderr, "[stamps] k_emit first entry -> last wave done: %.1f us\n", (double)(m3 - m0) * 0.01);
                    q2(a, "entry -> tables in LDS"); q2(b, "-> first chunk of entries evaluated"); q2(c, "-> particles built and stored"); q2(fin2, "wave done, after the first entry");
                }
            }
            fprintf(stderr, "[stamps] first entry -> last exit: %.1f us over %zu waves\n", (double)(x1 - e0) * 0.01, pro.size());
            {
                double xs[8] = {0}, xn[8] = {0}, ws[4] = {0}, wn[4] = {0}, gs[4] = {0}, gn[4] = {0}, rs[8] = {0}, rn[8] = {0};
                for (int sgm = 0; sgm < d.nseg; ++sgm) {
                    const unsigned long long *w = &st[((size_t)d.nseg + sgm) * 8];
                    if (!w[0] || !w[3]) continue;
                    const double t = (double)(w[2] - w[1]) * 0.01;
                    const int wg = sgm / 4;
                    xs[wg % 8] += t; xn[wg % 8] += 1; ws[sgm % 4] += t; wn[sgm % 4] += 1;
                    const int third = (int)((int64_t)sgm * 4 / d.nseg); gs[third] += t; gn[third] += 1;
                    const int rk = wg / ctx->num_cu; if (rk < 8) { rs[rk] += t; rn[rk] += 1; }
                }
                fprintf(stderr, "[stamps] tile loop mean [us] by workgroup %% 8:");
                for (int k = 0; k < 8; ++k) fprintf(stderr, " %.1f", xn[k] ? xs[k] / xn[k] : 0.0);
                fprintf(stderr, " | by wave of the workgroup:");
                for (int k = 0; k < 4; ++k) fprintf(stderr, " %.1f", wn[k] ? ws[k] / wn[k] : 0.0);
                fprintf(stderr, " | by quarter of the grid:");
                for (int k = 0; k < 4; ++k) fprintf(stderr, " %.1f", gn[k] ? gs[k] / gn[k] : 0.0);
                fprintf(stderr, " | by workgroup / CUs (the k-th workgroup of a CU under in-order dispatch):");
                for (int k = 0; k < 8; ++k) if (rn[k]) fprintf(stderr, " %.1f", rs[k] / rn[k]);
                fprintf(stderr, "\n");
            }
            q(pro, "entry -> tile loop (tables into LDS, records)"); q(loop, "tile loop"); q(epi, "tile loop end -> wave through (flush, workgroup barrier, tally row)");
            q(fin, "wave through, after the first entry");
            fprintf(stderr, "[stamps] shader clock inside k_sweep: median %.0f MHz (min %.0f, max %.0f)\n", clk[clk.size() / 2] / 10.0, clk.front() / 10.0, clk.back() / 10.0);
        }
        fprintf(stderr, "[stamps] cycles per tile: arrive %.0f  relax+drift %.0f  tally+store %.0f  pack/merge %.0f  event %.0f  event tally/store/repack %.0f  | total %.0f (tiles %.0f)\n",
                sum[0] / sum[6], sum[1] / sum[6], sum[2] / sum[6], sum[3] / sum[6], sum[4] / sum[6], sum[5] / sum[6], tot / sum[6], sum[6]);
        if (d.qx) {
            std::vector<double> cyc, wk, qq, ps;
            for (int sgm = 0; sgm < d.nseg; ++sgm) {
                cyc.push_back((double)st[(size_t)sgm * 8 + 3]); wk.push_back((double)st[(size_t)sgm * 8 + 4]);
                qq.push_back((double)(st[(size_t)sgm * 8 + 5] >> 32)); ps.push_back((double)(st[(size_t)sgm * 8 + 5] & 0xffffffffull));
            }
            auto stat = [](std::vector<double> v, const char *nm) {
                std::sort(v.begin(), v.end());
                double sm = 0; for (double x : v) sm += x;
                fprintf(stderr, "[stamps] k_events per segment %s: min %.0f  median %.0f  mean %.0f  p99 %.0f  max %.0f\n", nm, v.front(), v[v.size() / 2], sm / v.size(), v[(size_t)(v.size() * 0.99)], v.back());
            };
            stat(cyc, "cycles"); stat(wk, "cycles in walks"); stat(qq, "queue entries"); stat(ps, "walk passes");
            std::vector<double> lc, ln;
            for (int sgm = 0; sgm < d.nseg; ++sgm) { lc.push_back((double)(st[(size_t)sgm * 8 + 6] & ((1ull << 40) - 1))); ln.push_back((double)(st[(size_t)sgm * 8 + 6] >> 40)); }
            stat(lc, "cycles in faces passes"); stat(ln, "faces passes");
        }
    }
#endif
    const int32_t nd = *done;
    if (!band_s.empty()) {
        const size_t rl = 4 * (size_t)S * ctx->band_B;
        std::vector<double> br(band_s.size() * rl);
        NK_HIP(hipMemcpyAsync(br.data(), ctx->band_rows_d, br.size() * sizeof(double), hipMemcpyDeviceToHost, ctx->stream));
        NK_HIP(hipStreamSynchronize(ctx->stream));
        const int unseen = ctx->halt_words[2] ? nd - 1 : -1;
        for (size_t r = 0; r < band_s.size(); ++r) {
            if (band_s[r] >= nd || band_s[r] == unseen) continue;
            ctx->band_rows.insert(ctx->band_rows.end(), br.begin() + r * rl, br.begin() + (r + 1) * rl);
            ctx->band_steps.push_back(ctx->step + band_s[r]);
        }
    }
    nk_batch_leave(ctx, nsteps, nd, tail_emit, relax0, nsteps > 0 && relax_flushed[0]);
    float ms = 0.f;
    double sk = 0.0, ek = 0.0, vk = 0.0;
    const int nt = nd < nev ? nd : nev;
    for (int s = 0; s < nt; ++s) {
        NK_HIP(hipEventElapsedTime(&ms, ev[4 * s], ev[4 * s + 1])); ek += ms;
        NK_HIP(hipEventElapsedTime(&ms, ev[4 * s + 1], ev[4 * s + 2])); sk += ms;
        NK_HIP(hipEventElapsedTime(&ms, ev[4 * s + 2], ev[4 * s + 3])); vk += ms;
    }
    NK_HIP(hipEventElapsedTime(&ms, t0, t1));
    if (nt > 0 && nd == nsteps) {
        ctx->timing.step_kernel_ms = sk / nt;
        ctx->timing.emit_kernel_ms = ek / nt;
        ctx->timing.events_kernel_ms = vk / nt;
        ctx->timing.total_ms = ms;
    }
    return NK_OK;
}

static inline bool nk_want_resident(const nk_ctx *ctx) {
    const NkDev &d = ctx->d;
    if (!getenv("NK_RESIDENT") || getenv("NK_NO_RESIDENT") || ctx->comm || d.nranks != 1 || d.Fr > 0 || d.mig_buf || d.qx || nk_geom_mode(ctx) != 1) return false;
    if (ctx->band_B > 0) return false;
    if (ctx->field.on) return false;
    if (ctx->modes.on) return false;
    if (d.res_gen == 2 || d.sv_interp == 3 || d.NB > 254 || d.S > 128 || d.nseg <= 0) return false;
    const int64_t lim = getenv("NK_RESIDENT_MAX") ? atoll(getenv("NK_RESIDENT_MAX")) : 1200000;
    return d.cap <= lim && nk_lds(ctx, true, 5) <= 160 * 1024;
}
#define NK_RESIDENT_CASE(B, P, lrec, STMT) { if (lrec) { auto KERNEL = k_resident<B, P, true>; STMT; } else { auto KERNEL = k_resident<B, P, false>; STMT; } }
// ... 175 lines not shown
            NK_HIP(hipStreamSynchronize(ctx->stream));
            int32_t again[4];
            NK_HIP(hipMemcpy(again, d.halt, 16, hipMemcpyDeviceToHost));
            if (again[2]) { ctx->err = "nk_step: migrating particles do not fit their segment after growing it"; return NK_ERR_CAPACITY; }
            NK_HIP(hipMemcpy(d.halt, zero4, 16, hipMemcpyHostToDevice));
        }
        if (d.mig_buf && (hw[3] || !only_inbox)) {
            const int64_t want = std::max<int64_t>(hw[3] ? 2 * (int64_t)d.mig_cap : 0, d.segcap / 2);
            if ((rc = nk_ensure_migration(ctx, want))) return rc;
        }
        if ((rc = nk_update_tau_window(ctx, false))) return rc;
        if (ctx->field.on && (rc = nk_field_refresh(ctx))) return rc;
        if (ctx->fgroups.on && (rc = nk_fgroups_refresh(ctx))) return rc;
        if (ctx->modes.on && (rc = nk_modes_refresh(ctx))) return rc;
    }
    return NK_OK;
}
static int nk_step_end(nk_ctx *ctx, int overflow) {
    int rc = NK_OK;
    ctx->timing.slots = ctx->d.cap;
    if (overflow & 256) {
        uint32_t z2[2] = {0u, 0u};
        NK_HIP(hipMemcpy(ctx->anomalies + 1, z2, 8, hipMemcpyHostToDevice));
        int32_t z = 0;
        NK_HIP(hipMemcpy(ctx->d.overflow, &z, 4, hipMemcpyHostToDevice));
        ctx->err = "nk_step: the resident kernel's grid barrier timed out; set NK_NO_RESIDENT=1";
        return NK_ERR_HIP;
    }
    if (overflow) {
        ctx->err = "particle capacity exceeded during nk_step (reason mask " + std::to_string(overflow) +
                   "): particles were dropped; call nk_reserve with a larger capacity";
        return NK_ERR_CAPACITY;
    }
    if (ctx->comm && !ctx->band_rows.empty()) {
        if ((rc = nk_comm_allreduce(ctx, ctx->band_rows.data(), (int64_t)ctx->band_rows.size()))) return rc;
    }
    if (ctx->field.on) {
        long long st[4];
        rc = nk_field_status(ctx, st, "nk_step");
        if (ctx->fgroups.on) {
            const std::string ef = ctx->err;
            long long sg[8];
            const int rcg = nk_fgroups_status(ctx, sg, "nk_step");
            if (rc && rcg == NK_ERR_CAPACITY) ctx->err = ef + "; " + ctx->err;
            else if (rc) ctx->err = ef;
            if (!rc) rc = rcg;
        }
        if (rc) return rc;
    }
    if (ctx->modes.on) {
        long long st[4];
        if ((rc = nk_modes_status(ctx, st, "nk_step"))) return rc;
    }
    return NK_OK;
}

int nk_step(nk_ctx *ctx, int32_t nsteps, nk_tally *out) {
    NK_ARG(ctx && nsteps > 0, "nk_step: bad arguments");
    int rc = nk_step_begin(ctx);
    if (rc) return rc;
    NkStepRun run;
    std::vector<double> h;
    while (run.s_out < nsteps) {
        int32_t nd = 0;
        if ((rc = nk_want_resident(ctx) ? nk_step_resident(ctx, nsteps - run.s_out, h, &nd) : nk_step_batch(ctx, nsteps - run.s_out, h, &nd))) return rc;
        if ((rc = nk_step_consume(ctx, nsteps, out, run, h, nd))) return rc;
    }
    return nk_step_end(ctx, run.overflow);
}

struct nk_group {
    int R = 0;
    std::vector<nk_ctx *> m;
    int device = 0;
    std::string err;
    unsigned char *dev = nullptr;
    unsigned char *stage = nullptr;
    NkGroupRec *recs_d = nullptr, *recs_h = nullptr;
    int recs_cap = 0;
    std::vector<hipEvent_t> ev;
    std::vector<char> halted, alone;
    nk_group_report rep = {};
};
static thread_local std::string g_group_error;

#define NK_GHIP(call)                                                                                  \
    do {                                                                                               \
        hipError_t e_ = (call);                                                                        \
        if (e_ != hipSuccess) {                                                                        \
            g->err = std::string(#call) + ": " + hipGetErrorString(e_);                                \
            return NK_ERR_HIP;                                                                         \
        }                                                                                              \
    } while (0)

struct NkGroupKey {
    NkGroupKind kind;
    int S, R, NB, flux_every, contains_every, res_gen;
    double dt;
    int64_t step;
};
static NkGroupKey nk_group_key(nk_ctx *ctx) {
    const NkDev &d = ctx->d;
    NkGroupKey k;
    k.kind.pid = (bool)d.pid;
    k.kind.lrec = nk_want_lrec(ctx);
    k.kind.fast = k.kind.pid ? 0 : nk_sweep_fast(ctx);
    k.kind.box = d.box != 0;
    k.S = d.S; k.R = d.R; k.NB = d.NB;
    k.flux_every = ctx->params.flux_every; k.contains_every = ctx->params.contains_every; k.res_gen = d.res_gen;
    k.dt = d.dt;
    k.step = ctx->step;
    return k;
}
struct NkGroupPlan { NkGroupKey key; size_t lds_w = 0, lds_t = 0; int device = 0; };
static std::string nk_group_scope(nk_ctx *ctx) {
    const NkDev &d = ctx->d;
    if (!(ctx->have_material && ctx->have_mesh && ctx->have_sv && ctx->have_params)) return "it is not ready (engine not configured: need material, mesh, subvolumes and params)";
    if (ctx->comm || d.nranks != 1) return "it belongs to a communicator (several ranks)";
    if (d.Fr > 0 || d.mig_buf) return "it has rough facets (their migrants are delivered between the sweep and the tail)";
    if (nk_geom_mode(ctx) != 1) return "its mesh is too large for tables in LDS";
    if (nk_want_split(ctx) || d.qx) return "it uses the split sweep";
    if (d.sv_interp == 3) return "it uses RBF temperatures";
    if (d.res_gen == 2) return "its generator is 'one_to_one'";
    if (ctx->band_B > 0) return "its band-resolved flux is on (nk_set_bands)";
    if (ctx->field.on) return "its field maps are on (nk_set_field)";
    if (ctx->modes.on) return "its mode tally is on (nk_set_modes)";
    if (d.R > 0 && getenv("NK_NO_TAIL_EMIT")) return "NK_NO_TAIL_EMIT is set (the emission would need a launch of its own)";
    return "";
}
static int nk_group_check(nk_ctx *const *m, int R, NkGroupPlan *plan, std::string &err) {
    if (R < 1 || R > NK_GROUP_MAX_MEMBERS) { err = "nk_group: R = " + std::to_string(R) + " is outside 1 .. " + std::to_string(NK_GROUP_MAX_MEMBERS); return NK_ERR_ARG; }
    if (!m) { err = "nk_group: NULL members"; return NK_ERR_ARG; }
    for (int r = 0; r < R; ++r) {
        if (!m[r]) { err = "nk_group: member " + std::to_string(r) + " is NULL"; return NK_ERR_ARG; }
        for (int q = 0; q < r; ++q)
            if (m[q] == m[r]) { err = "nk_group: member " + std::to_string(r) + " is the same context as member " + std::to_string(q) + " (given twice)"; return NK_ERR_ARG; }
    }
    for (int r = 1; r < R; ++r)
        if (m[r]->device != m[0]->device) {
            err = "nk_group: member " + std::to_string(r) + " is on device " + std::to_string(m[r]->device) + ", member 0 on device " + std::to_string(m[0]->device);
            return NK_ERR_ARG;
        }
    for (int r = 0; r < R; ++r) {
        const std::string why = nk_group_scope(m[r]);
        if (!why.empty()) { err = "nk_group: member " + std::to_string(r) + " is outside the grouped path: " + why; return NK_ERR_ARG; }
    }
    for (int r = 0; r < R; ++r) {
        if (nk_check_ready(m[r])) { err = "nk_group: member " + std::to_string(r) + " is not ready: " + m[r]->err; return NK_ERR_ARG; }
        const std::string why = nk_group_scope(m[r]);
        if (!why.empty()) { err = "nk_group: member " + std::to_string(r) + " is outside the grouped path: " + why; return NK_ERR_ARG; }
    }
    size_t lds_w = 0, lds_t = 0;
    for (int r = 0; r < R; ++r) {
        const size_t w = nk_lds(m[r], true, m[r]->d.pid ? 3 : 2), e = nk_lds(m[r], true, 1);
        const size_t tl = e > (size_t)(NK_WG * 8 + 16) ? e : (size_t)(NK_WG * 8 + 16);
        if (w > 64 * 1024 || tl > 64 * 1024) { err = "nk_group: member " + std::to_string(r) + " is outside the grouped path: its tables need more than 64 KB of LDS"; return NK_ERR_ARG; }
        lds_w = std::max(lds_w, w); lds_t = std::max(lds_t, tl);
    }
    const NkGroupKey k0 = nk_group_key(m[0]);
    for (int r = 1; r < R; ++r) {
        const NkGroupKey k = nk_group_key(m[r]);
        const char *what = nullptr;
        std::string a, b;
#define NK_GROUP_SAME(field, name) if (!what && !(k.field == k0.field)) { what = name; a = std::to_string(k.field); b = std::to_string(k0.field); }
        NK_GROUP_SAME(step, "current step")
        NK_GROUP_SAME(S, "subvolumes")
        NK_GROUP_SAME(R, "reservoirs")
        NK_GROUP_SAME(NB, "tally bins")
        NK_GROUP_SAME(flux_every, "flux_every")
        NK_GROUP_SAME(contains_every, "contains_every")
        NK_GROUP_SAME(dt, "dt")
        NK_GROUP_SAME(res_gen, "generator")
        NK_GROUP_SAME(kind.pid, "kernel instantiation (particle ids)")
        NK_GROUP_SAME(kind.lrec, "kernel instantiation (mode records in LDS)")
        NK_GROUP_SAME(kind.fast, "kernel instantiation (subvolume fast path)")
        NK_GROUP_SAME(kind.box, "kernel instantiation (box store)")
#undef NK_GROUP_SAME
        if (what) {
            err = "nk_group: member " + std::to_string(r) + " disagrees with member 0 on the " + what + " (" + a + " against " + b + ")";
            return NK_ERR_ARG;
        }
    }
    if (plan) { plan->key = k0; plan->lds_w = lds_w; plan->lds_t = lds_t; plan->device = m[0]->device; }
    return NK_OK;
}

int nk_group_create(nk_group **out, nk_ctx *const *members, int32_t R) {
    if (!out) { g_group_error = "nk_group_create: NULL out"; return NK_ERR_ARG; }
    *out = nullptr;
    NkGroupPlan plan;
    int rc = nk_group_check(members, R, &plan, g_group_error);
    if (rc) return rc;
    const int device = plan.device;
    nk_group *g = new nk_group();
    g->R = R;
    g->m.assign(members, members + R);
    g->halted.assign((size_t)R, 0);
    g->alone.assign((size_t)R, 0);
    g->device = device;
    g->rep.R = R;
    const size_t bytes = sizeof(NkGroupHead) + (size_t)NK_GROUP_MAX * sizeof(NkDev);
    hipError_t e = hipSetDevice(device);
    if (e == hipSuccess) e = hipMalloc((void **)&g->dev, bytes);
    if (e == hipSuccess) e = hipHostMalloc((void **)&g->stage, bytes, hipHostMallocDefault);
    if (e == hipSuccess) {
        g->ev.resize(3 * 4 + 2);
        for (auto &v : g->ev) { v = nullptr; if (e == hipSuccess) e = hipEventCreate(&v); }
    }
    if (e != hipSuccess) {
        g_group_error = std::string("nk_group_create: ") + hipGetErrorString(e);
        (void)hipGetLastError();
        nk_group_destroy(g);
        return NK_ERR_HIP;
    }
    *out = g;
    return NK_OK;
}

void nk_group_destroy(nk_group *g) {
    if (!g) return;
    (void)hipSetDevice(g->device);
    for (auto &v : g->ev) if (v) hipEventDestroy(v);
    if (g->dev) hipFree(g->dev);
    if (g->stage) hipHostFree(g->stage);
    if (g->recs_d) hipFree(g->recs_d);
    if (g->recs_h) hipHostFree(g->recs_h);
    delete g;
}

const char *nk_group_last_error(const nk_group *g) { return g ? g->err.c_str() : g_group_error.c_str(); }

int nk_group_info(nk_group *g, nk_group_report *out) {
    if (!g || !out) { if (g) g->err = "nk_group_info: NULL argument"; return NK_ERR_ARG; }
    *out = g->rep;
    return NK_OK;
}

static int nk_group_batch(nk_group *g, const NkGroupPlan &plan, hipStream_t stream, int32_t nsteps, std::vector<std::vector<double>> &hs,
                          std::vector<int32_t> &nds) {
    const int R = g->R;
    const NkGroupKey &key = plan.key;
    const size_t lds_w = plan.lds_w, lds_t = plan.lds_t;
    const int S = key.S, NB = key.NB, HROW = NB + 2 * S + 8;
    NkGroupHead *head = reinterpret_cast<NkGroupHead *>(g->stage);
    NkDev *devs = reinterpret_cast<NkDev *>(g->stage + sizeof(NkGroupHead));
    for (int k = 0; k <= NK_GROUP_MAX; ++k) head->pre_sweep[k] = head->pre_tail[k] = INT32_MAX;
    for (int k = 0; k < NK_GROUP_MAX; ++k) head->rows[k] = 0;
    head->NB = NB; head->pad_ = 0;
    if (nsteps > g->recs_cap) {
        if (g->recs_d) hipFree(g->recs_d);
        if (g->recs_h) hipHostFree(g->recs_h);
        g->recs_d = g->recs_h = nullptr; g->recs_cap = 0;
        const int cap = nsteps < 1024 ? 1024 : nsteps;
        NK_GHIP(hipMalloc((void **)&g->recs_d, (size_t)cap * R * sizeof(NkGroupRec)));
        NK_GHIP(hipHostMalloc((void **)&g->recs_h, (size_t)cap * R * sizeof(NkGroupRec), hipHostMallocDefault));
        g->recs_cap = cap;
    }
    struct Member { int g_sweep = 0, g_emit = 0; bool alt = false, pending = false, relax0 = false, flushed0 = false, emitted_ahead = false, tail_emit = false; };
    std::vector<Member> mem((size_t)R);
    int grid_sweep = 0, grid_tail = 0;
    for (int r = 0; r < R; ++r) {
        nk_ctx *ctx = g->m[r];
        NkDev &d = ctx->d;
        Member &me = mem[(size_t)r];
        if (nk_batch_hist(ctx, nsteps)) { g->err = "member " + std::to_string(r) + ": " + ctx->err; return NK_ERR_HIP; }
        (void)nk_sweep_blocks(ctx);
        me.g_sweep = ctx->g_sweep < (d.nseg + 3) / 4 ? ctx->g_sweep : (d.nseg + 3) / 4;
        me.tail_emit = d.R > 0;
        me.g_emit = me.tail_emit ? (ctx->num_cu * 8 < (d.nseg + 3) / 4 ? ctx->num_cu * 8 : (d.nseg + 3) / 4) : 0;
        d.tree_lds_fam0 = d.tree_nfam; d.tree_lds_off = 0;
        me.relax0 = me.pending = ctx->pending_relax;
        me.emitted_ahead = me.tail_emit && ctx->emitted_for == ctx->step;
        ctx->emitted_for = -1;
        ctx->timing.emit_fused = me.tail_emit ? 1 : 0;
        me.alt = d.seg_lo && !getenv("NK_NO_ALTERNATE");
        if (!me.alt) {
            const bool launches = ctx->walked && d.seg_lo;
            if (nk_normalize(ctx)) { g->err = "member " + std::to_string(r) + ": " + ctx->err; return NK_ERR_HIP; }
            if (launches) g->rep.member_launches += 1;
        }
        d.down = 0;
        head->pre_sweep[r] = grid_sweep; head->pre_tail[r] = grid_tail; head->rows[r] = me.g_sweep;
        grid_sweep += me.g_sweep;
        grid_tail += NB + me.g_emit;
        devs[r] = d;
    }
    head->pre_sweep[R] = grid_sweep; head->pre_tail[R] = grid_tail;
    for (int r = 0; r < R; ++r) {
        nk_ctx *ctx = g->m[r];
        const NkDev &d = ctx->d;
        bool pending = mem[(size_t)r].pending;
        for (int s = 0; s < nsteps; ++s) {
            const int64_t stepno = ctx->step + s;
            if (key.contains_every > 0 && (stepno % key.contains_every) == 0 && d.nS > 0) pending = false;
            NkGroupRec &rec = g->recs_h[(size_t)s * R + r];
            rec.step = (uint32_t)stepno;
            rec.do_relax = pending ? 1 : 0;
            rec.do_flux = (key.flux_every > 0 && ((stepno + 1) % key.flux_every) == 0) ? 1 : 0;
            rec.down = mem[(size_t)r].alt ? (int32_t)(stepno & 1) : 0;
            rec.hist_row = ctx->hist + (size_t)s * HROW;
            rec.acc = ctx->acc;
            pending = true;
        }
    }
    NkGroupHead *head_d = reinterpret_cast<NkGroupHead *>(g->dev);
    NkDev *devs_d = reinterpret_cast<NkDev *>(g->dev + sizeof(NkGroupHead));
    NK_GHIP(hipMemcpyAsync(g->dev, g->stage, sizeof(NkGroupHead) + (size_t)R * sizeof(NkDev), hipMemcpyHostToDevice, stream));
    NK_GHIP(hipMemcpyAsync(g->recs_d, g->recs_h, (size_t)nsteps * R * sizeof(NkGroupRec), hipMemcpyHostToDevice, stream));
    const int nev = nsteps < 4 ? 0 : 4;
    hipEvent_t *ev = g->ev.data();
    hipEvent_t t0 = g->ev[12], t1 = g->ev[13];
    NK_GHIP(hipEventRecord(t0, stream));
    for (int s = 0; s < nsteps; ++s) {
        for (int r = 0; r < R; ++r) {
            nk_ctx *ctx = g->m[r];
            NkDev &d = ctx->d;
            Member &me = mem[(size_t)r];
            const int64_t stepno = ctx->step + s;
            {
                bool fl_ = false;
                if (nk_batch_prelude(ctx, stepno, me.pending, fl_, &g->rep.member_launches)) { g->err = "member " + std::to_string(r) + ": " + ctx->err; return NK_ERR_HIP; }
                if (fl_ && s == 0) me.flushed0 = true;
            }
            if (d.R > 0 && !me.emitted_ahead) {
                NK_EMIT_LAUNCH(k_emit, me.g_emit, nk_lds(ctx, true, 1), d, (uint32_t)stepno);
                g->rep.member_launches += 1;
            }
            if (me.alt) ctx->walked = true;
            me.emitted_ahead = me.tail_emit;
            me.pending = true;
        }
        if (s < nev) NK_GHIP(hipEventRecord(ev[3 * s], stream));
        NK_GHIP(nk_group_launch_sweep(key.kind, grid_sweep, lds_w, stream, head_d, devs_d, g->recs_d + (size_t)s * R));
        if (s < nev) NK_GHIP(hipEventRecord(ev[3 * s + 1], stream));
        NK_GHIP(nk_group_launch_tail(key.kind.box, grid_tail, lds_t, stream, head_d, devs_d, g->recs_d + (size_t)s * R));
        if (s < nev) NK_GHIP(hipEventRecord(ev[3 * s + 2], stream));
        g->rep.sweep_launches += 1;
        g->rep.tail_launches += 1;
    }
    NK_GHIP(hipEventRecord(t1, stream));
    NK_GHIP(hipGetLastError());
    g->rep.grid_sweep = grid_sweep;
    g->rep.grid_tail = grid_tail;
    if (nsteps <= 4) { hipError_t q_; while ((q_ = hipStreamQuery(stream)) == hipErrorNotReady) { } if (q_ != hipSuccess) { g->err = std::string("hipStreamQuery: ") + hipGetErrorString(q_); return NK_ERR_HIP; } }
    NK_GHIP(hipStreamSynchronize(stream));
    bool all_ran = true;
    for (int r = 0; r < R; ++r) {
        nk_ctx *ctx = g->m[r];
        const Member &me = mem[(size_t)r];
        int32_t nd = 0;
        if (nk_batch_collect(ctx, nsteps, hs[(size_t)r], &nd)) { g->err = "member " + std::to_string(r) + ": " + ctx->err; return NK_ERR_HIP; }
        nds[(size_t)r] = nd;
        nk_batch_leave(ctx, nsteps, nd, me.tail_emit, me.relax0, me.flushed0);
        if (nd < nsteps) all_ran = false;
    }
    float ms = 0.f;
    if (nev > 0 && all_ran) {
        double sk = 0.0, tk = 0.0;
        for (int s = 0; s < nev; ++s) {
            NK_GHIP(hipEventElapsedTime(&ms, ev[3 * s], ev[3 * s + 1])); sk += ms;
            NK_GHIP(hipEventElapsedTime(&ms, ev[3 * s + 1], ev[3 * s + 2])); tk += ms;
        }
        g->rep.sweep_kernel_ms = sk / nev;
        g->rep.tail_kernel_ms = tk / nev;
    }
    NK_GHIP(hipEventElapsedTime(&ms, t0, t1));
    g->rep.total_ms = ms;
    return NK_OK;
}

int nk_group_step(nk_group *g, int32_t nsteps, nk_tally *outs) {
    if (!g) return NK_ERR_ARG;
    if (nsteps <= 0) { g->err = "nk_group_step: bad arguments"; return NK_ERR_ARG; }
    const int R = g->R;
    NkGroupPlan plan;
    int rc = nk_group_check(g->m.data(), R, &plan, g->err);
    if (rc) return rc;
    NK_GHIP(hipSetDevice(g->device));
    const hipStream_t stream = g->m[0]->stream;
    std::vector<hipStream_t> own((size_t)R);
    for (int r = 0; r < R; ++r) { own[(size_t)r] = g->m[r]->stream; g->m[r]->stream = stream; }
    auto leave = [&](int code) { for (int r = 0; r < R; ++r) g->m[r]->stream = own[(size_t)r]; return code; };
    for (int r = 0; r < R; ++r)
        if ((rc = nk_step_begin(g->m[r]))) { g->err = "member " + std::to_string(r) + ": " + g->m[r]->err; return leave(rc); }
    std::vector<std::vector<double>> hs((size_t)R);
    std::vector<int32_t> nds((size_t)R, 0);
    if ((rc = nk_group_batch(g, plan, stream, nsteps, hs, nds))) return leave(rc);
    g->rep.steps += nsteps;
    for (int r = 0; r < R; ++r) {
        nk_ctx *ctx = g->m[r];
        NkStepRun run;
        nk_tally *out = outs ? &outs[r] : nullptr;
        const int64_t halts0 = ctx->timing.halts;
        if ((rc = nk_step_consume(ctx, nsteps, out, run, hs[(size_t)r], nds[(size_t)r]))) { g->err = "member " + std::to_string(r) + ": " + ctx->err; return leave(rc); }
        if (ctx->timing.halts != halts0 && !g->halted[(size_t)r]) { g->halted[(size_t)r] = 1; g->rep.halted += 1; }
        if (run.s_out < nsteps) {
            if (!g->alone[(size_t)r]) { g->alone[(size_t)r] = 1; g->rep.finished_alone += 1; }
            std::vector<double> h;
            while (run.s_out < nsteps) {
                int32_t nd = 0;
                if ((rc = nk_step_batch(ctx, nsteps - run.s_out, h, &nd)) || (rc = nk_step_consume(ctx, nsteps, out, run, h, nd))) {
                    g->err = "member " + std::to_string(r) + ": " + ctx->err;
                    return leave(rc);
                }
                g->rep.member_launches += 2 * (int64_t)nd;
            }
        }
        if ((rc = nk_step_end(ctx, run.overflow))) { g->err = "member " + std::to_string(r) + ": " + ctx->err; return leave(rc); }
    }
    return leave(NK_OK);
}

int nk_download_particles(nk_ctx *ctx, int64_t capacity, double *x, double *y, double *z, int32_t *mode, double *occ,
                          double *n_ts, int32_t *facet, uint64_t *pid, int64_t *N_out) {
    NK_ARG(ctx && N_out, "nk_download_particles: NULL argument");
    NK_HIP(hipSetDevice(ctx->device));
    NkDev &d = ctx->d;
    *N_out = 0;
    if (d.cap == 0) return NK_OK;
    if (ctx->have_material && ctx->have_sv && ctx->have_mesh) { int rc = nk_flush_relax(ctx, 0); if (rc) return rc; }
    NkHostParticles h;
    int rc = nk_gather_live(ctx, h, capacity != 0);
    if (rc) return rc;
    const int64_t live = (int64_t)h.x.size();
    *N_out = live;
    if (capacity == 0) return NK_OK;
    NK_ARG(capacity >= live, "nk_download_particles: capacity smaller than the live particle count");
    if (x) memcpy(x, h.x.data(), live * 8);
    if (y) memcpy(y, h.y.data(), live * 8);
    if (z) memcpy(z, h.z.data(), live * 8);
    if (occ) memcpy(occ, h.occ.data(), live * 8);
    if (n_ts) memcpy(n_ts, h.nts.data(), live * 8);
    if (mode) memcpy(mode, h.mode.data(), live * 4);
    if (facet) memcpy(facet, h.facet.data(), live * 4);
    if (pid) memcpy(pid, h.pid.data(), live * 8);
    return NK_OK;
}

int nk_get_subvol_temperature(nk_ctx *ctx, double *T_sv) {
    NK_ARG(ctx && T_sv && ctx->have_sv, "nk_get_subvol_temperature: bad arguments");
    NK_HIP(hipSetDevice(ctx->device));
    NK_HIP(hipStreamSynchronize(ctx->stream));
    NK_HIP(hipMemcpy(T_sv, ctx->d.T_sv, (size_t)ctx->d.S * 8, hipMemcpyDeviceToHost));
    return NK_OK;
}
int nk_set_subvol_temperature(nk_ctx *ctx, const double *T_sv) {
    NK_ARG(ctx && T_sv && ctx->have_sv, "nk_set_subvol_temperature: bad arguments");
    NK_HIP(hipSetDevice(ctx->device));
    NK_HIP(hipStreamSynchronize(ctx->stream));
    std::vector<double> t(T_sv, T_sv + ctx->d.S);
    if (ctx->d.sv_interp == 3) nk_rbf_coefficients(ctx, t);
    NK_HIP(hipMemcpy(ctx->d.T_sv, t.data(), t.size() * 8, hipMemcpyHostToDevice));
    nk_track_T(ctx, T_sv, ctx->d.S);
    return NK_OK;
}
int nk_get_step(nk_ctx *ctx, int64_t *step) {
    NK_ARG(ctx && step, "nk_get_step: NULL argument");
    *step = ctx->step;
    return NK_OK;
}
int nk_get_timing(nk_ctx *ctx, nk_timing *t) {
    NK_ARG(ctx && t, "nk_get_timing: NULL argument");
    *t = ctx->timing;
    t->box_store = (ctx->d.cap > 0 && ctx->d.box) ? 1 : 0;
    return NK_OK;
}

static int nk_load_rccl(NkRccl &r, std::string &err) {
    if (r.lib) return NK_OK;
    const char *names[] = {"librccl.so.1", "librccl.so", "/opt/rocm/lib/librccl.so.1", "/opt/rocm/lib/librccl.so"};
    for (const char *n : names) { r.lib = dlopen(n, RTLD_NOW | RTLD_GLOBAL); if (r.lib) break; }
    if (!r.lib) { err = std::string("cannot load librccl: ") + dlerror(); return NK_ERR_COMM; }
    r.GetUniqueId = (decltype(r.GetUniqueId))dlsym(r.lib, "ncclGetUniqueId");
    r.CommInitRank = (decltype(r.CommInitRank))dlsym(r.lib, "ncclCommInitRank");
    r.AllReduce = (decltype(r.AllReduce))dlsym(r.lib, "ncclAllReduce");
    r.CommDestroy = (decltype(r.CommDestroy))dlsym(r.lib, "ncclCommDestroy");
    r.CommCount = (decltype(r.CommCount))dlsym(r.lib, "ncclCommCount");
    r.CommUserRank = (decltype(r.CommUserRank))dlsym(r.lib, "ncclCommUserRank");
// ... 901 lines not shown
```

nanokappa_amd/csrc/nk_group.h:

```cpp
#pragma once
#include <hip/hip_runtime.h>
#include <stdint.h>

struct NkDev;

#define NK_GROUP_MAX 32

struct NkGroupHead {
    int32_t pre_sweep[NK_GROUP_MAX + 1];
    int32_t pre_tail[NK_GROUP_MAX + 1];
    int32_t rows[NK_GROUP_MAX];
    int32_t NB;
    int32_t pad_;
};
struct NkGroupRec {
    uint32_t step;
    int32_t do_relax, do_flux;
    int32_t down;
    double *hist_row, *acc;
};

struct NkGroupKind { bool pid, lrec; int fast; bool box; };

hipError_t nk_group_launch_sweep(const NkGroupKind &k, int grid, size_t lds, hipStream_t stream, const NkGroupHead *head, const NkDev *devs,
                                 const NkGroupRec *recs);
hipError_t nk_group_launch_sweep_fast(const NkGroupKind &k, int grid, size_t lds, hipStream_t stream, const NkGroupHead *head, const NkDev *devs,
                                      const NkGroupRec *recs);
hipError_t nk_group_launch_tail(bool box, int grid, size_t lds, hipStream_t stream, const NkGroupHead *head, const NkDev *devs, const NkGroupRec *recs);
```

nanokappa_amd/csrc/nk_group.hip:

```cpp
#include <hip/hip_runtime.h>
#include <stdint.h>
#include "../../include/nanokappa_hip.h"
#define NK_KERNEL_LINKAGE template <int NK_NOT_IN_THIS_TU = 0>
#include "nk_kernels.h"
#include "nk_group.h"

#define NK_CONSTANT_AS __attribute__((address_space(4)))

__device__ __forceinline__ int nk_group_member(const NK_CONSTANT_AS int32_t *pre, int b) {
    int r = 0;
#pragma unroll
    for (int k = 1; k < NK_GROUP_MAX; ++k) r += (b >= pre[k]) ? 1 : 0;
    return r;
}
__device__ __forceinline__ void nk_group_dev(NkDev &d, const NkDev *devs, int r) {
    const NK_CONSTANT_AS NkDev *c = (const NK_CONSTANT_AS NkDev *)devs + r;
    __builtin_memcpy(&d, c, sizeof(NkDev));
}

template <bool PID, bool LREC, int FAST, bool BOX>
__global__ __launch_bounds__(NK_WG, NK_SWEEP_BOUND(1, false, false, false)) void k_sweep_group(const NkGroupHead *head_, const NkDev *devs,
                                                                                               const NkGroupRec *recs_) {
    extern __shared__ __align__(16) unsigned char smem[];
    const NK_CONSTANT_AS NkGroupHead *head = (const NK_CONSTANT_AS NkGroupHead *)head_;
    const int b = (int)blockIdx.x;
    const int r = nk_group_member(head->pre_sweep, b);
    const int wg = b - head->pre_sweep[r], nwg = head->pre_sweep[r + 1] - head->pre_sweep[r];
    const NK_CONSTANT_AS NkGroupRec *rec = (const NK_CONSTANT_AS NkGroupRec *)recs_ + r;
    NkDev d;
    nk_group_dev(d, devs, r);
    if (d.halt[0]) return;
    d.down = rec->down;
    if (FAST) { d.sv_kind = 0; d.sv_interp = FAST - 1; d.T_ref_local = 1; }
    NkLds L;
    nk_lds_setup<1, PID ? 3 : 2>(d, smem, L);
    nk_sweep_body<1, false, false, PID, false, LREC, FAST, BOX>(d, L, rec->step, rec->do_relax, rec->do_flux, wg, nwg);
    nk_lds_flush(d, L, wg);
}

#ifdef NK_GROUP_PLAIN

#define NK_GROUP_SWEEP(P, L, F, B) k_sweep_group<P, L, F, B><<<grid, NK_WG, lds, stream>>>(head, devs, recs)
hipError_t nk_group_launch_sweep_fast(const NkGroupKind &k, int grid, size_t lds, hipStream_t stream, const NkGroupHead *head, const NkDev *devs,
                                      const NkGroupRec *recs) {
    if (k.pid || (k.fast != 1 && k.fast != 2)) return hipErrorInvalidValue;
    if (k.box) {
        if (k.lrec) { if (k.fast == 1) NK_GROUP_SWEEP(false, true, 1, true); else NK_GROUP_SWEEP(false, true, 2, true); }
        else { if (k.fast == 1) NK_GROUP_SWEEP(false, false, 1, true); else NK_GROUP_SWEEP(false, false, 2, true); }
    } else {
        if (k.lrec) { if (k.fast == 1) NK_GROUP_SWEEP(false, true, 1, false); else NK_GROUP_SWEEP(false, true, 2, false); }
        else { if (k.fast == 1) NK_GROUP_SWEEP(false, false, 1, false); else NK_GROUP_SWEEP(false, false, 2, false); }
    }
    return hipGetLastError();
}

#else

template <bool BOX>
__global__ __launch_bounds__(NK_WG) void k_tail_group(const NkGroupHead *head_, const NkDev *devs, const NkGroupRec *recs_) {
    extern __shared__ __align__(16) unsigned char smem[];
    const NK_CONSTANT_AS NkGroupHead *head = (const NK_CONSTANT_AS NkGroupHead *)head_;
    const int b = (int)blockIdx.x;
    const int r = nk_group_member(head->pre_tail, b);
    const int wg = b - head->pre_tail[r], nwg = head->pre_tail[r + 1] - head->pre_tail[r];
    const int n_reduce = head->NB;
    const NK_CONSTANT_AS NkGroupRec *rec = (const NK_CONSTANT_AS NkGroupRec *)recs_ + r;
    NkDev d;
    nk_group_dev(d, devs, r);
    if (wg < n_reduce) {
        double *sh = reinterpret_cast<double *>(smem);
        int &last = *reinterpret_cast<int *>(smem + NK_WG * sizeof(double));
        nk_reduce_body(d, head->rows[r], rec->acc, rec->hist_row, rec->do_flux, 1, wg, n_reduce, sh, last);
    } else {
        nk_emit_body<1, BOX>(d, rec->step + 1u, smem, wg - n_reduce, nwg - n_reduce, true);
    }
}

#define NK_GROUP_SWEEP(P, L, B) k_sweep_group<P, L, 0, B><<<grid, NK_WG, lds, stream>>>(head, devs, recs)
hipError_t nk_group_launch_sweep(const NkGroupKind &k, int grid, size_t lds, hipStream_t stream, const NkGroupHead *head, const NkDev *devs,
                                 const NkGroupRec *recs) {
    if (k.fast) return nk_group_launch_sweep_fast(k, grid, lds, stream, head, devs, recs);
    if (k.box) {
        if (k.pid) { if (k.lrec) NK_GROUP_SWEEP(true, true, true); else NK_GROUP_SWEEP(true, false, true); }
        else { if (k.lrec) NK_GROUP_SWEEP(false, true, true); else NK_GROUP_SWEEP(false, false, true); }
    } else {
        if (k.pid) { if (k.lrec) NK_GROUP_SWEEP(true, true, false); else NK_GROUP_SWEEP(true, false, false); }
        else { if (k.lrec) NK_GROUP_SWEEP(false, true, false); else NK_GROUP_SWEEP(false, false, false); }
    }
    return hipGetLastError();
}

hipError_t nk_group_launch_tail(bool box, int grid, size_t lds, hipStream_t stream, const NkGroupHead *head, const NkDev *devs, const NkGroupRec *recs) {
    if (box) k_tail_group<true><<<grid, NK_WG, lds, stream>>>(head, devs, recs);
    else k_tail_group<false><<<grid, NK_WG, lds, stream>>>(head, devs, recs);
    return hipGetLastError();
}

#endif
```

nanokappa_amd/csrc/nk_kernels.h:

```cpp
#pragma once
#ifndef NK_KERNEL_LINKAGE
#define NK_KERNEL_LINKAGE
#endif
#include "nk_device.h"

#define NK_TILE 64
#ifndef NK_NT
#define NK_NT 0
#endif
#if NK_NT
#define NK_LD(p) __builtin_nontemporal_load(p)
#define NK_ST(p, v) __builtin_nontemporal_store(v, p)
#else
#define NK_LD(p) (*(p))
#define NK_ST(p, v) (*(p) = (v))
#endif
#ifdef NK_STAMPS
#define NK_STAMP(k)                                                                                    \
    do {                                                                                               \
        unsigned long long t_;                                                                         \
        __builtin_amdgcn_sched_barrier(0);                                                             \
        asm volatile("s_memtime %0\n\ts_waitcnt lgkmcnt(0)" : "=s"(t_)::"memory");                     \
        __builtin_amdgcn_sched_barrier(0);                                                             \
        st_acc[k] += t_ - st_last;                                                                     \
        st_last = t_;                                                                                  \
    } while (0)
#else
#define NK_STAMP(k) do { } while (0)
#endif

__device__ __forceinline__ int nk_rank(unsigned long long m) {
    return (int)__builtin_amdgcn_mbcnt_hi((unsigned int)(m >> 32), __builtin_amdgcn_mbcnt_lo((unsigned int)m, 0u));
}

struct NkLds {
    NkSvTab tb;
    NkBins bins;
    const double *planes, *faces;
    const NkFacet *facets;
    const double *resT;
    const int *rf_off;
    const double *rf_cdf, *rf_verts;
    unsigned int *sp_pref, *sp_cnt, *sp_rm;
    double *sp_cv, *sp_pr;
    double *lrec;
    double *carry;
    double *oring;
    unsigned int *oring_w;
    double *colsum;
};

#ifndef NK_LREC_STRIDE
#define NK_LREC_STRIDE 5
#endif
#ifndef NK_OUT_RING
#define NK_OUT_RING 0
#endif
#define NK_ORING (NK_OUT_RING ? 128 : 0)
#define NK_CARRY_DOUBLES(kind) (((kind) == 3 || (kind) == 5) ? 576 : 448)
#ifndef NK_BOX_GENERAL_CAST
#define NK_BOX_GENERAL_CAST 0
#endif
#define NK_COLSUM_DOUBLES 768
__host__ __device__ inline size_t nk_lds_bytes(int S, int R, int F, int NP, int Fc, int geom, int kind, int nrf, int rbfP, int nlrec = 0, int carry = 0) {
    const bool emit = kind == 1 || kind >= 4;
    int Fl = geom == 1 ? F : 0;
    int Pl = Fl ? NP : 0;
    int Fcl = geom == 1 ? Fc : 0;
    size_t nd = (size_t)S + (size_t)((rbfP + 1) & ~1) + 3 * S + ((3 * S) & 1) + 4 * (size_t)S + NK_NREP * S + NK_NREP * 3 * S + 4 * R +
                (size_t)Fl * NK_FACE_DOUBLES + (size_t)Pl * NK_PLANE_DOUBLES + 2 * (size_t)R + 10 * (size_t)nrf +
                (emit ? 2 * (size_t)(NK_WG / 64) * NK_EMIT_CHUNK : 0) + (kind >= 2 ? (size_t)(NK_WG / 64) * ((size_t)nlrec * 2 * NK_LREC_STRIDE + (carry ? NK_CARRY_DOUBLES(kind) : 0) + NK_ORING * ((kind == 3 || kind == 5) ? 6 : 5)) : 0) +
                (kind >= 4 ? NK_COLSUM_DOUBLES : 0) + 4;
    size_t bytes = nd * 8 + (size_t)Fcl * sizeof(NkFacet) +
                   (size_t)(NK_NREP * S + R + 1 + (R + 1) + (emit ? 3 * (NK_WG / 64) * NK_EMIT_CHUNK : 0) + (kind >= 2 ? (NK_WG / 64) * NK_ORING : 0)) * 4 + 32;
    return (bytes + 15) & ~(size_t)15;
}

template <int GEOM, int KIND>
__device__ __forceinline__ void nk_lds_carve(const NkDev &d, unsigned char *smem, NkLds &L) {
    constexpr bool EMIT = KIND == 1 || KIND >= 4;
    const int S = d.S, R = d.R;
    const int Fl = GEOM == 1 ? d.F : 0;
    const int Pl = Fl ? d.NP : 0;
    const int Fcl = GEOM == 1 ? d.Fc : 0;
    const int nrf = (GEOM == 1 && d.res_lds) ? d.res_nf : 0;
    double *p = (double *)smem;
    L.tb.Tsv = p; p += S + ((d.rbf_P + 1) & ~1);
    L.tb.cen = p; p += 3 * S + ((3 * S) & 1);
    p += ((size_t)S & 1);
    L.tb.sv = (const NkSv *)p; p += 4 * S;
    L.bins.E = p; p += NK_NREP * S;
    L.bins.flux = p; p += NK_NREP * 3 * S;
    L.bins.resb = p; p += 4 * R;
    p += ((size_t)(p - (double *)smem) & 1);
    double *faces = p; p += (size_t)Fl * NK_FACE_DOUBLES;
    double *planes = p; p += (size_t)Pl * NK_PLANE_DOUBLES;
    double *resT = p; p += 2 * R;
    double *rf_cdf = p; p += nrf;
    double *rf_verts = p; p += 9 * (size_t)nrf;
    if (EMIT) { L.sp_cv = p; p += (NK_WG / 64) * NK_EMIT_CHUNK; L.sp_pr = p; p += (NK_WG / 64) * NK_EMIT_CHUNK; } else L.sp_cv = L.sp_pr = nullptr;
    p += ((size_t)(p - (double *)smem) & 1);
    if (KIND >= 2) {
        L.lrec = p; p += (NK_WG / 64) * (size_t)d.nlrec * 2 * NK_LREC_STRIDE;
        L.carry = p; p += d.qx ? 0 : (NK_WG / 64) * NK_CARRY_DOUBLES(KIND);
        L.oring = p; p += (NK_WG / 64) * NK_ORING * ((KIND == 3 || KIND == 5) ? 6 : 5);
    } else { L.lrec = nullptr; L.carry = nullptr; L.oring = nullptr; }
    if (KIND >= 4) { L.colsum = p; p += NK_COLSUM_DOUBLES; } else L.colsum = nullptr;
    NkFacet *facets = (NkFacet *)p;
    unsigned int *u = (unsigned int *)(facets + Fcl);
    L.bins.N = u; u += NK_NREP * S;
    L.bins.nleave = u; u += R;
    L.bins.misc = u; u += 1;
    int *rf_off = (int *)u; u += R + 1;
    if (EMIT) {
        L.sp_pref = u; u += (NK_WG / 64) * NK_EMIT_CHUNK;
        L.sp_cnt = u; u += (NK_WG / 64) * NK_EMIT_CHUNK;
        L.sp_rm = u; u += (NK_WG / 64) * NK_EMIT_CHUNK;
    } else { L.sp_pref = L.sp_cnt = L.sp_rm = nullptr; }
    if (KIND >= 2) { L.oring_w = u; u += (NK_WG / 64) * NK_ORING; } else L.oring_w = nullptr;
    L.resT = resT;
    L.rf_off = rf_off; L.rf_cdf = rf_cdf; L.rf_verts = rf_verts;
    if (GEOM == 1) { L.faces = faces; L.planes = planes; L.facets = facets; }
    else { L.faces = d.faces; L.planes = d.planes; L.facets = d.facets; }
}
template <int GEOM, int KIND>
__device__ __forceinline__ void nk_lds_setup(const NkDev &d, unsigned char *smem, NkLds &L) {
    nk_lds_carve<GEOM, KIND>(d, smem, L);
    const int S = d.S, R = d.R;
    const int Fl = GEOM == 1 ? d.F : 0;
    const int Pl = Fl ? d.NP : 0;
    const int Fcl = GEOM == 1 ? d.Fc : 0;
    const int nrf = (GEOM == 1 && d.res_lds) ? d.res_nf : 0;
    double *faces = const_cast<double *>(L.faces), *planes = const_cast<double *>(L.planes);
    NkFacet *facets = const_cast<NkFacet *>(L.facets);
    double *resT = const_cast<double *>(L.resT), *rf_cdf = const_cast<double *>(L.rf_cdf), *rf_verts = const_cast<double *>(L.rf_verts);
    int *rf_off = const_cast<int *>(L.rf_off);
    double *Tsv = const_cast<double *>(L.tb.Tsv), *cen = const_cast<double *>(L.tb.cen);
    NkSv *sv = const_cast<NkSv *>(L.tb.sv);
    const int t = threadIdx.x, nth = blockDim.x;
    const int nT = S + d.rbf_P, a = d.sv_axis, nface = Fl * NK_FACE_DOUBLES, nplane = Pl * NK_PLANE_DOUBLES;
    const int nfw = Fcl * (int)(sizeof(NkFacet) / 4);
    const int jn = t + 1 < S ? t + 1 : t;
    const double l_T = t < nT ? d.T_sv[t] : 0.0;
    const double l_cen = t < 3 * S ? d.centers[t] : 0.0;
    const double l_c = t < S ? d.centers[3 * t + a] : 0.0, l_cn = t < S ? d.centers[3 * jn + a] : 0.0, l_Tn = t < S ? d.T_sv[jn] : 0.0;
    const double l_rT = t < R ? d.res_T[t] : 1.0;
    const double l_face = t < nface ? d.faces[t] : 0.0;
    const double l_plane = t < nplane ? d.planes[t] : 0.0;
    const int l_off = (nrf > 0 && t <= R) ? d.res_face_off[t] : 0;
    const double l_cdf = t < nrf ? d.res_face_cdf[t] : 0.0;
    const double l_vert = t < 9 * nrf ? d.res_face_verts[t] : 0.0;
    const int32_t l_fw = t < nfw ? ((const int32_t *)d.facets)[t] : 0;
    if (t < nT) Tsv[t] = l_T;
    if (t < 3 * S) cen[t] = l_cen;
    if (t < S) {
        NkSv q;
        q.c = l_c; q.T = l_T; q.slope = jn > t ? (l_Tn - l_T) / (l_cn - l_c) : 0.0; q.invT = 1.0 / l_T;
        sv[t] = q;
    }
    if (t < R) { L.bins.nleave[t] = 0u; resT[2 * t] = l_rT; resT[2 * t + 1] = 1.0 / l_rT; }
    if (t < nface) faces[t] = l_face;
    if (t < nplane) planes[t] = l_plane;
    if (nrf > 0 && t <= R) rf_off[t] = l_off;
    if (t < nrf) rf_cdf[t] = l_cdf;
    if (t < 9 * nrf) rf_verts[t] = l_vert;
    if (t < nfw) ((int32_t *)facets)[t] = l_fw;
    for (int i = t; i < NK_NREP * S; i += nth) { L.bins.E[i] = 0.0; L.bins.N[i] = 0u; }
    for (int i = t; i < NK_NREP * 3 * S; i += nth) L.bins.flux[i] = 0.0;
    for (int i = t; i < 4 * R; i += nth) L.bins.resb[i] = 0.0;
    if (t == 0) L.bins.misc[0] = 0u;
    for (int i = t + nth; i < nT; i += nth) Tsv[i] = d.T_sv[i];
    for (int i = t + nth; i < 3 * S; i += nth) cen[i] = d.centers[i];
    for (int i = t + nth; i < S; i += nth) {
        const int j = i + 1 < S ? i + 1 : i;
        const double c = d.centers[3 * i + a], cn = d.centers[3 * j + a], T = d.T_sv[i], Tn = d.T_sv[j];
        NkSv q;
        q.c = c; q.T = T; q.slope = j > i ? (Tn - T) / (cn - c) : 0.0; q.invT = 1.0 / T;
        sv[i] = q;
    }
    for (int i = t + nth; i < R; i += nth) { L.bins.nleave[i] = 0u; const double T = d.res_T[i]; resT[2 * i] = T; resT[2 * i + 1] = 1.0 / T; }
    for (int i = t + nth; i < nface; i += nth) faces[i] = d.faces[i];
    for (int i = t + nth; i < nplane; i += nth) planes[i] = d.planes[i];
    if (nrf > 0) {
        for (int i = t + nth; i <= R; i += nth) rf_off[i] = d.res_face_off[i];
        for (int i = t + nth; i < nrf; i += nth) rf_cdf[i] = d.res_face_cdf[i];
        for (int i = t + nth; i < 9 * nrf; i += nth) rf_verts[i] = d.res_face_verts[i];
    }
    for (int i = t + nth; i < nfw; i += nth) ((int32_t *)facets)[i] = ((const int32_t *)d.facets)[i];
    __syncthreads();
}

__device__ __forceinline__ void nk_lds_flush(const NkDev &d, const NkLds &L, int64_t row) {
    __syncthreads();
    const int S = d.S, R = d.R;
    double *out = d.partials + row * d.NB;
    for (int b = threadIdx.x; b < d.NB; b += blockDim.x) {
        double v = 0.0;
        if (b < S) { for (int r = 0; r < NK_NREP; ++r) v += L.bins.E[r * S + b]; }
        else if (b < 2 * S) { unsigned int c = 0; for (int r = 0; r < NK_NREP; ++r) c += L.bins.N[r * S + (b - S)]; v = (double)c; }
        else if (b < 5 * S) { int k = b - 2 * S; for (int r = 0; r < NK_NREP; ++r) v += L.bins.flux[r * 3 * S + k]; }
        else if (b < 5 * S + R) v = (double)L.bins.nleave[b - 5 * S];
        else if (b < 5 * S + 2 * R) v = L.bins.resb[4 * (b - 5 * S - R)];
        else if (b < 5 * S + 5 * R) { int k = b - 5 * S - 2 * R; v = L.bins.resb[4 * (k / 3) + 1 + (k % 3)]; }
        else v = (double)L.bins.misc[0];
        out[b] = v;
    }
}

struct NkSegModes {
    const NkMode *rec;
    const int32_t *gm;
    int nl;
    int estride, eoff;
    __device__ __forceinline__ int mode(int i) const { return gm ? gm[i] : i; }
    __device__ __forceinline__ int entry_mode(int l) const { return gm ? gm[l] : l * estride + eoff; }
};
struct NkPlainModes { __device__ __forceinline__ int mode(int i) const { return i; } };
__device__ __forceinline__ void nk_mode_home(const NkDev &d, int mode, int &seg, int &idx) {
    const uint32_t slot = (uint32_t)d.m2s[mode], n = (uint32_t)d.nseg;
    const uint32_t q = slot / n;
    idx = (int)q;
    seg = (int)(slot - q * n);
}
__device__ __forceinline__ NkSegModes nk_seg_modes(const NkDev &d, int seg) {
    NkSegModes sm;
    sm.rec = d.part ? d.modetab_p + (int64_t)seg * d.nlmax : d.modetab;
    sm.gm = d.part ? d.s2m + (int64_t)seg * d.nlmax : nullptr;
    sm.nl = d.seg_nl[seg];
    sm.estride = d.nseg; sm.eoff = seg;
    return sm;
}

template <bool RBF = true>
__device__ __forceinline__ double nk_relax(const NkDev &d, const NkLds &L, const NkTauWin &tw, const double4 &ra, const double4 &rb, double x,
                                           double y, double z, double occ, const NkSegModes &sm, int idx) {
    double invT;
    const double T = nk_interp_T<RBF>(d, L.tb, x, y, z, invT);
    const double tau = nk_lifetime(d, tw, rb.y, rb.z, rb.w, T, sm, idx);
    const double n0 = (T > 0.0) ? nk_be(ra.x * d.c_hk, rb.x, invT, d.invT0) : 0.0;
    const double xr = -d.dt * nk_rcp(tau);
    double er;
    if (__builtin_expect(__ballot(tau > 0.0 && !(xr > -0.125)) == 0ull, 1)) er = nk_exp_small(xr);
    else er = nk_exp(xr);
    return (tau > 0.0) ? n0 + (occ - n0) * er : n0;
}

__device__ __forceinline__ void nk_sample_res_face(const int *off, const double *cdf, const double *verts, int r, double uf,
                                                   double us, double ur, double &x0, double &y0, double &z0) {
    const int f0 = off[r], nf = off[r + 1] - f0;
    int a = nk_ss_right(cdf + f0, nf, uf);
    a = a > nf - 1 ? nf - 1 : a;
    const double *fv = verts + 9 * (f0 + a);
    const double sq = sqrt(us);
    const double a0 = 1.0 - sq, a1 = (1.0 - ur) * sq, a2 = ur * sq;
    x0 = a0 * fv[0] + a1 * fv[3] + a2 * fv[6];
    y0 = a0 * fv[1] + a1 * fv[4] + a2 * fv[7];
    z0 = a0 * fv[2] + a1 * fv[5] + a2 * fv[8];
}

#define NK_RAY(GEOM, d, L, skip, x, y, z, vx, vy, vz, tc, fc)                                                        \
    do {                                                                                                              \
        if ((GEOM) == 2 && (d).NG > 0) nk_find_boundary_tree(d, skip, x, y, z, vx, vy, vz, tc, fc);                      \
        else nk_find_boundary((L).planes, (L).faces, (d).NP, (d).tol, x, y, z, vx, vy, vz, tc, fc);                   \
    } while (0)

__device__ __forceinline__ void nk_emit_entry(const NkDev &d, uint32_t step, int64_t rm, int64_t at, double prob, int &c, int &c_mine, double &cv) {
    const double fixed = floor(prob);
    int mask;
    if (d.res_gen == 0) {
        cv = d.rc_p[(int64_t)(step & 1u) * d.rc_len + at] + (prob - fixed);
        mask = cv >= 1.0;
        cv -= (double)mask;
        d.rc_p[(int64_t)((step + 1u) & 1u) * d.rc_len + at] = cv;
    } else {
        double d1;
        nk_uniform2_dev(d.seed, (uint64_t)rm | 0xFFFFFFFF00000000ull, step, NK_TAG_DICE, cv, d1);
        mask = cv <= (prob - fixed);
    }
    c = (int)fixed + mask;
    c_mine = c;
    if (d.nranks > 1) {
        c_mine = 0;
        for (int level = c; level >= 1; --level)
            c_mine += (((uint32_t)rm + (uint32_t)level + step) % (uint32_t)d.nranks) == (uint32_t)d.rank;
    }
}

NK_KERNEL_LINKAGE __global__ __launch_bounds__(NK_WG) void k_emit_one_to_one(NkDev d, uint32_t step) {
    if (d.halt[0]) return;
    int64_t total = 0;
    for (int r = 0; r < d.R; ++r) total += d.nleave_prev[r];
    for (int64_t c = (int64_t)blockIdx.x * NK_WG + threadIdx.x; c < total; c += (int64_t)gridDim.x * NK_WG) {
        int r = 0;
        int64_t i = c;
        while (r < d.R - 1 && i >= d.nleave_prev[r]) { i -= d.nleave_prev[r]; ++r; }
        if (((uint32_t)((uint64_t)i + step) % (uint32_t)d.nranks) != (uint32_t)d.rank) continue;
        const uint64_t pid = ((uint64_t)((step + 1u) & 0xFFFFFFu) << 40) | ((uint64_t)r << 32) | (uint64_t)i;
        double um, u1;
        nk_uniform2_dev(d.seed, pid, step, NK_TAG_DICE, um, u1);
        int m = nk_ss_left(d.res_roulette + (int64_t)r * d.M, d.M, um);
        m = m > d.M - 1 ? d.M - 1 : m;
        if (i >= (1ll << 24)) { atomicOr(d.overflow, 16); continue; }
        int seg, lidx;
        if (d.part) nk_mode_home(d, m, seg, lidx); else seg = m % d.nseg;
        const int at = atomicAdd(d.sp_inbox_n + seg, 1);
        if (at < d.sp_icap) d.sp_inbox[(int64_t)seg * d.sp_icap + at] = ((uint64_t)i << 40) | ((uint64_t)((int64_t)r * d.M + m) << 12);
        else atomicOr(d.overflow, 8);
    }
}

__device__ __forceinline__ void nk_newborn_place(const NkDev &d, double x0, double y0, double z0, double vx, double vy, double vz,
                                                 double dt_in, double tc, double &x, double &y, double &z, double &nts) {
    x = x0 + vx * dt_in; y = y0 + vy * dt_in; z = z0 + vz * dt_in;
    nts = tc / d.dt - dt_in / d.dt;
}

template <int GEOM, bool BOX>
__device__ __forceinline__ int nk_emit_one(const NkDev &d, const NkLds &L, uint32_t step, int seg, int lane, unsigned int *sp_pref,
                                           unsigned int *sp_cnt, unsigned int *sp_rm, double *sp_cv, double *sp_pr, bool ahead, bool to_queue,
                                           int &bound_out
#ifdef NK_STAMPS
                                           , unsigned long long em_t0, unsigned long long em_t1, unsigned long long &em_t2
#endif
) {
    const int plo = d.seg_lo ? d.seg_lo[seg] : 0;
    const int64_t base = (int64_t)seg * d.segcap;
    const int count = d.seg_count[seg];
    const NkSegModes sm = nk_seg_modes(d, seg);
    const int nent = d.res_gen != 2 ? d.R * sm.nl : 0;
    int made = 0;
    int sp_bound = 0;
    for (int e0 = 0; e0 < nent || (d.res_gen == 2 && e0 == 0); e0 += NK_EMIT_CHUNK) {
        int spn = 0;
        if (d.res_gen == 2) {
            spn = d.sp_inbox_n[seg];
            spn = spn < d.sp_icap ? spn : d.sp_icap;
            sp_bound = lane == 0 ? 2 * spn + 64 : 0;
        } else {
            unsigned int run = 0;
#pragma unroll
            for (int k = 0; k < 2; ++k) {
                const int e = e0 + k * 64 + lane;
                int c = 0, cmine = 0;
                double cv = 0.0, prob = 0.0;
                unsigned int rm32 = 0, rl = 0;
                if (e < nent) {
                    const int r = e / sm.nl, l = e - r * sm.nl;
                    rl = ((unsigned int)r << 12) | ((unsigned int)l << 18);
                    const int64_t rm = (int64_t)r * d.M + sm.entry_mode(l);
                    const int64_t at = ((int64_t)seg * d.R + r) * d.nlmax + l;
                    prob = d.ep_p[at];
                    nk_emit_entry(d, step, rm, at, prob, c, cmine, cv);
                    rm32 = (unsigned int)rm;
                    sp_bound += ((int)floor(prob) + 1 + d.nranks - 1) / d.nranks;
                }
                unsigned int v = (unsigned int)cmine;
#pragma unroll
                for (int o = 1; o < 64; o <<= 1) { const unsigned int u = __shfl_up(v, o, 64); if (lane >= o) v += u; }
                sp_cnt[k * 64 + lane] = (unsigned int)c | rl;
                sp_rm[k * 64 + lane] = rm32;
                sp_cv[k * 64 + lane] = cv;
                sp_pr[k * 64 + lane] = prob;
                sp_pref[k * 64 + lane] = v + run - (unsigned int)cmine;
                run += __shfl(v, 63, 64);
            }
            __builtin_amdgcn_fence(__ATOMIC_SEQ_CST, "wavefront");
            spn = (int)run;
        }
#ifdef NK_STAMPS
        if (!em_t2) em_t2 = __builtin_amdgcn_s_memrealtime();
#endif
        for (int spj = 0; spj < spn; spj += NK_TILE) {
            const int j = spj + lane;
            if (j >= spn) continue;
            int64_t rm;
            int level, r, idx;
            double prob = 0.0, cval = 0.0;
            uint64_t o2o = 0;
            if (d.res_gen == 2) {
                const uint64_t recd = d.sp_inbox[(int64_t)seg * d.sp_icap + j];
                rm = (int64_t)((recd >> 12) & 0xFFFFFFFull);
                level = 0;
                o2o = recd >> 40;
                r = (int)((uint32_t)rm / (uint32_t)d.M);
                const int mode = (int)((uint32_t)rm - (uint32_t)r * (uint32_t)d.M);
                idx = d.part ? (int)((uint32_t)d.m2s[mode] / (uint32_t)d.nseg) : mode;
            } else {
                int lo = 0, hi = NK_EMIT_CHUNK;
                while (hi - lo > 1) { const int mid = (lo + hi) >> 1; if ((int)sp_pref[mid] <= j) lo = mid; else hi = mid; }
                const unsigned int cw = sp_cnt[lo];
                const int q = j - (int)sp_pref[lo], c = (int)(cw & 0xFFFu);
                r = (int)((cw >> 12) & 0x3Fu);
                rm = (int64_t)sp_rm[lo];
                idx = d.part ? (int)(cw >> 18) : (int)((uint32_t)rm - (uint32_t)r * (uint32_t)d.M);
                cval = sp_cv[lo];
                prob = sp_pr[lo];
                if (d.nranks == 1) level = c - q;
                else {
                    const uint32_t n = (uint32_t)d.nranks;
                    const uint32_t tq = ((uint32_t)d.rank + n - (((uint32_t)rm + step) % n)) % n;
                    const uint32_t top = (uint32_t)c - (((uint32_t)c + n - tq) % n);
                    level = (int)(top - (uint32_t)q * n);
                }
            }
            const NkMode *rec = sm.rec + idx;
            const double4 ra = *reinterpret_cast<const double4 *>(rec);
            const double E0 = rec->E0;
            const uint64_t pid = level > 0 ? ((uint64_t)((step + 1u) & 0xFFFFFFu) << 40) | ((uint64_t)rm << 12) | (uint64_t)level
                                           : ((uint64_t)((step + 1u) & 0xFFFFFFu) << 40) | ((uint64_t)r << 32) | o2o;
            double uf, us, ur, ut;
            nk_uniform2_dev(d.seed, pid, step, NK_TAG_EMIT, uf, us);
            nk_uniform2_dev(d.seed, pid, step, NK_TAG_EMIT + 1, ur, ut);
            const double iprob = level > 0 ? nk_rcp(prob) : 0.0;
            const double dt_in = (level == 0) ? d.dt * ut
                               : (level == 1) ? d.dt * (1.0 - cval * iprob)
                                              : d.dt * (1.0 - ((double)(level - 1) + ut) * iprob);
            double x0, y0, z0;
            if (GEOM == 1 && d.res_lds) nk_sample_res_face(L.rf_off, L.rf_cdf, L.rf_verts, r, uf, us, ur, x0, y0, z0);
            else nk_sample_res_face(d.res_face_off, d.res_face_cdf, d.res_face_verts, r, uf, us, ur, x0, y0, z0);
            const double omega = ra.x, vx = ra.y, vy = ra.z, vz = ra.w;
            const double occ = nk_be(omega * d.c_hk, E0, L.resT[2 * r + 1], d.invT0);
            if (GEOM == 2 && to_queue) {
                const int o = made + j;
                if (o < d.segcap) {
                    const int64_t i = base + o;
                    const int rf = d.res_facet[r];
                    const NkFacet &fq = d.facets[rf];
                    const int skip = nk_tree_skip(d, rf, fq.cx, fq.cy, fq.cz, fq.nx, fq.ny, fq.nz, x0, y0, z0, vx, vy, vz);
                    d.qx[i] = x0; d.qy[i] = y0; d.qz[i] = z0; d.qocc[i] = occ; d.qnts[i] = dt_in;
                    d.qw0[i] = NK_NEWBORN | ((uint32_t)((skip == rf ? rf : -1) + 1) << d.lb) | (uint32_t)idx;
                    if (d.qpid) d.qpid[i] = pid;
                } else if (!(ahead && d.halt[1])) atomicOr(d.overflow, 1);
                continue;
            }
            double tc = 0.0;
            int facet = -1;
            int skip = NK_TREE_NO_SKIP;
            if (GEOM == 2 && d.NG > 0) {
                const int rf = d.res_facet[r];
                const NkFacet &fq = d.facets[rf];
                skip = nk_tree_skip(d, rf, fq.cx, fq.cy, fq.cz, fq.nx, fq.ny, fq.nz, x0, y0, z0, vx, vy, vz);
            }
            if (!BOX) NK_RAY(GEOM, d, L, skip, x0, y0, z0, vx, vy, vz, tc, facet);
            const int o = count + made + j;
            if (plo + o < d.segcap) {
                const int64_t i = base + plo + o;
                const NkSlot q = nk_slot(d, i);
                double xa, ya, za, na;
                nk_newborn_place(d, x0, y0, z0, vx, vy, vz, dt_in, tc, xa, ya, za, na);
                d.x.p[q.od] = xa; d.y.p[q.od] = ya; d.z.p[q.od] = za;
                d.occ.p[q.od] = occ;
                if (!BOX) d.nts.p[q.od] = na;
                d.w0.p[q.ow] = BOX ? (NK_NEWBORN | (uint32_t)idx) : (NK_NEWBORN | ((uint32_t)(facet + 1) << d.lb) | (uint32_t)idx);
                if (d.pid) d.pid.p[q.od] = pid;
            } else if (!(ahead && d.halt[1])) atomicOr(d.overflow, 1);
        }
        made += spn;
        __builtin_amdgcn_fence(__ATOMIC_SEQ_CST, "wavefront");
    }
#pragma unroll
    for (int o = 32; o > 0; o >>= 1) sp_bound += __shfl_xor(sp_bound, o, 64);
    const int room = d.segcap - plo - count;
    const int put = (GEOM == 2 && to_queue) ? 0 : (made < room ? made : (room > 0 ? room : 0));
    if (lane == 0) {
        if (GEOM == 2 && to_queue) { d.seg_new[seg] = 0; d.seg_evq[seg] = made < d.segcap ? made : d.segcap; }
        else d.seg_new[seg] = put;
        d.seg_bound[seg] = sp_bound;
        if (d.res_gen == 2) d.sp_inbox_n[seg] = 0;
#ifdef NK_STAMPS
        if (d.stamps) { unsigned long long *w = d.stamps + ((int64_t)d.nseg + seg) * 8 + 4; w[0] = em_t0; w[1] = em_t1; w[2] = em_t2; w[3] = __builtin_amdgcn_s_memrealtime(); }
#endif
    }
    bound_out = sp_bound;
    return put;
}

template <int GEOM, bool BOX = false>
__device__ __forceinline__ void nk_emit_segments(const NkDev &d, NkLds L, uint32_t step, int bid, int nblocks, bool ahead
#ifdef NK_STAMPS
                                                 , unsigned long long em_t0, unsigned long long em_t1
#endif
) {
#ifdef NK_STAMPS
    unsigned long long em_t2 = 0;
#endif
    const int tid = threadIdx.x, lane = tid & 63, wave = __builtin_amdgcn_readfirstlane(tid >> 6);
    unsigned int *sp_pref = L.sp_pref + wave * NK_EMIT_CHUNK, *sp_cnt = L.sp_cnt + wave * NK_EMIT_CHUNK,
                 *sp_rm = L.sp_rm + wave * NK_EMIT_CHUNK;
    double *sp_cv = L.sp_cv + wave * NK_EMIT_CHUNK, *sp_pr = L.sp_pr + wave * NK_EMIT_CHUNK;
    const int nwaves = nblocks * (NK_WG / 64);
    const bool to_queue = GEOM == 2 && d.NG > 0 && d.qx != nullptr;
    for (int seg = bid * (NK_WG / 64) + wave; seg < d.nseg; seg += nwaves) {
        int bound_;
#ifdef NK_STAMPS
        (void)nk_emit_one<GEOM, BOX>(d, L, step, seg, lane, sp_pref, sp_cnt, sp_rm, sp_cv, sp_pr, ahead, to_queue, bound_, em_t0, em_t1, em_t2);
#else
        (void)nk_emit_one<GEOM, BOX>(d, L, step, seg, lane, sp_pref, sp_cnt, sp_rm, sp_cv, sp_pr, ahead, to_queue, bound_);
#endif
    }
}

template <int GEOM, bool BOX = false>
__device__ __forceinline__ void nk_emit_body(const NkDev &d, uint32_t step, unsigned char *smem, int bid, int nblocks, bool ahead = false) {
#ifdef NK_STAMPS
    const unsigned long long em_t0 = __builtin_amdgcn_s_memrealtime();
#endif
    if (d.halt[0]) return;
    NkLds L;
    nk_lds_setup<GEOM, 1>(d, smem, L);
#ifdef NK_STAMPS
    nk_emit_segments<GEOM, BOX>(d, L, step, bid, nblocks, ahead, em_t0, __builtin_amdgcn_s_memrealtime());
#else
    nk_emit_segments<GEOM, BOX>(d, L, step, bid, nblocks, ahead);
#endif
}

template <int GEOM, bool BOX = false>
__global__ __launch_bounds__(NK_WG) void k_emit(NkDev d, uint32_t step) {
    extern __shared__ __align__(16) unsigned char smem[];
    nk_emit_body<GEOM, BOX>(d, step, smem, (int)blockIdx.x, (int)gridDim.x);
}

template <bool PID>
struct NkOut {
    double *x, *y, *z, *occ, *nts, *pid;
    unsigned int *w0;
    int on, ob, wout;
    int64_t m0; int ms, mroom;
    __device__ __forceinline__ void place(int64_t first, int sign, int room) { m0 = first; ms = sign; mroom = room; }
    __device__ __forceinline__ void init(const NkLds &L, int wave) {
        double *p = L.oring + wave * NK_ORING * (PID ? 6 : 5);
        x = p; y = p + NK_ORING; z = p + 2 * NK_ORING; occ = p + 3 * NK_ORING; nts = p + 4 * NK_ORING; pid = PID ? p + 5 * NK_ORING : nullptr;
        w0 = L.oring_w + wave * NK_ORING;
        on = ob = wout = 0;
    }
    __device__ __forceinline__ int reserve(int rank, int n) { const int o = wout + rank; wout += n; return o; }
    template <bool BOX>
    static __device__ __forceinline__ void put_slot(const NkDev &d, int64_t i, double px, double py, double pz, double pocc, double pnts,
                                                    uint32_t pw0, unsigned long long ppid) {
        typedef NkBlock<!BOX, PID> B;
        double *q = B::slot(d.x.p, i);
        NK_ST(q, px); NK_ST(q + B::O_Y, py); NK_ST(q + B::O_Z, pz); NK_ST(q + B::O_OCC, pocc);
        if (!BOX) NK_ST(q + B::O_NTS, pnts);
        if (PID) NK_ST(reinterpret_cast<unsigned long long *>(q + B::O_PID), ppid);
        NK_ST(B::word(d.x.p, i), pw0);
    }
    template <bool BOX = false>
    __device__ __forceinline__ void store(const NkDev &d, int64_t base, bool put, int o, double px, double py, double pz, double pocc,
                                          double pnts, uint32_t pw0, unsigned long long ppid) {
        if (put) {
            if (o < mroom) put_slot<BOX>(d, m0 + ms * (int64_t)o, px, py, pz, pocc, pnts, pw0, ppid);
            else atomicOr(d.overflow, 2);
        }
    }
    template <bool BOX = false>
    __device__ __forceinline__ void push(const NkDev &d, int64_t base, int lane, bool put, int rank, int n, double px, double py,
                                         double pz, double pocc, double pnts, uint32_t pw0, unsigned long long ppid) {
        if (!NK_OUT_RING) {
            if (put) {
                const int o = wout + rank;
                if (o < mroom) put_slot<BOX>(d, m0 + ms * (int64_t)o, px, py, pz, pocc, pnts, pw0, ppid);
                else atomicOr(d.overflow, 2);
            }
            wout += n;
            return;
        }
        if (put) {
            const int e = (ob + on + rank) & (NK_ORING - 1);
            x[e] = px; y[e] = py; z[e] = pz; occ[e] = pocc; nts[e] = pnts; w0[e] = pw0;
            if (PID) pid[e] = __longlong_as_double((long long)ppid);
        }
        on += n;
        __builtin_amdgcn_fence(__ATOMIC_SEQ_CST, "wavefront");
        if (on >= NK_TILE) flush(d, base, lane, NK_TILE);
    }
    __device__ __forceinline__ void flush(const NkDev &d, int64_t base, int lane, int n) {
        if (wout + n <= d.segcap) {
            if (lane < n) {
                const int e = (ob + lane) & (NK_ORING - 1);
                const int64_t i = base + wout + lane;
                d.x[i] = x[e]; d.y[i] = y[e]; d.z[i] = z[e]; d.occ[i] = occ[e]; d.nts[i] = nts[e]; d.w0[i] = w0[e];
                if (PID) d.pid[i] = (unsigned long long)__double_as_longlong(pid[e]);
            }
            wout += n;
        } else if (lane == 0) atomicOr(d.overflow, 2);
        ob = (ob + n) & (NK_ORING - 1);
        on -= n;
        __builtin_amdgcn_fence(__ATOMIC_SEQ_CST, "wavefront");
    }
};

typedef double nk_v2d __attribute__((ext_vector_type(2)));
typedef const __attribute__((address_space(3))) nk_v2d *NkLdsRec;
__device__ __forceinline__ NkLdsRec nk_lds_rec(const double2 *q) { return (NkLdsRec)(const void *)q; }

#ifndef NK_SWEEP_OCC
#define NK_SWEEP_OCC 3
#endif
#ifndef NK_PREFETCH2
#define NK_PREFETCH2 0
#endif
#ifndef NK_PARK_TAU
#define NK_PARK_TAU 1
#endif
#ifndef NK_PRIO_ROT
#define NK_PRIO_ROT 0
#endif
#ifndef NK_DEFER_STORE
#define NK_DEFER_STORE 0
#endif
#ifndef NK_SWEEP_OCC_BIG
#define NK_SWEEP_OCC_BIG 2
#endif
#ifndef NK_SWEEP_OCC_SPLIT
#define NK_SWEEP_OCC_SPLIT 4
#endif
#define NK_SWEEP_BOUND(GEOM, ROUGH, RBF, SPLIT) ((SPLIT) ? NK_SWEEP_OCC_SPLIT : (((GEOM) == 2 || (RBF)) ? NK_SWEEP_OCC_BIG : NK_SWEEP_OCC))
template <int GEOM, bool ROUGH, bool RBF, bool PID, bool SPLIT, bool LREC, int FAST = 0, bool BOX = false>
__device__ __forceinline__ void nk_sweep_body(const NkDev &d, NkLds L, uint32_t step, int do_relax, int flags, int wg, int nwg
#ifdef NK_STAMPS
                                              , unsigned long long st_entry_r
#endif
) {
    static_assert(!BOX || (GEOM == 1 && !SPLIT && !NK_PREFETCH2 && !NK_OUT_RING), "the box store goes with the fused sweep over LDS tables");
    const bool do_flux = (flags & 1) != 0;
    const int tid = threadIdx.x, lane = tid & 63, wave = __builtin_amdgcn_readfirstlane(tid >> 6);
    const int rep = lane & (NK_NREP - 1);
    const uint32_t lbmask = (1u << d.lb) - 1u;
    NkBoxWalls bw;
    if (BOX) bw.load(d);
    NkTauWin tw;
    tw.load(d, NK_PARK_TAU != 0);
    double2 *lrec = reinterpret_cast<double2 *>(L.lrec) + wave * d.nlrec * NK_LREC_STRIDE;
    double *const cX = L.carry ? L.carry + wave * NK_CARRY_DOUBLES(PID ? 3 : 2) : nullptr;
    double *const cP = cX + 6 * 64;
    uint32_t *const cW = reinterpret_cast<uint32_t *>(cX + (PID ? 7 : 6) * 64);
    const int nwaves = nwg * (NK_WG / 64);
#if NK_PRIO_ROT
    const int prio_phase = (int)(wg / (nwg > 3 ? (nwg + 3) / 4 : 1));
#endif
    for (int seg = wg * (NK_WG / 64) + wave; seg < d.nseg; seg += nwaves) {
        const int64_t base = (int64_t)seg * d.segcap;
        const int nnew = d.R > 0 ? d.seg_new[seg] : 0;
        const int count = d.seg_count[seg] + nnew;
        if (lane == 0 && nnew > 0) atomicAdd(&L.bins.misc[0], (unsigned int)nnew);
        const NkSegModes sm = nk_seg_modes(d, seg);
        constexpr bool use_lrec = LREC;
        if (use_lrec) {
            for (int r0 = lane; r0 < sm.nl; r0 += 64) {
                const double4 *g = reinterpret_cast<const double4 *>(sm.rec + r0);
                const double4 a = g[0], b = g[1];
                double2 *q = lrec + r0 * NK_LREC_STRIDE;
                q[0] = make_double2(a.x, a.y); q[1] = make_double2(a.z, a.w); q[2] = make_double2(b.x, b.y); q[3] = make_double2(b.z, b.w);
                if (NK_LREC_STRIDE > 4 && (ROUGH || PID)) *reinterpret_cast<int *>(q + 4) = sm.mode(r0);
            }
            __builtin_amdgcn_fence(__ATOMIC_SEQ_CST, "wavefront");
        }
        auto mode_of = [&](int i) -> int {
            if (use_lrec && NK_LREC_STRIDE > 4) return *(const __attribute__((address_space(3))) int *)(const void *)(lrec + i * NK_LREC_STRIDE + 4);
            return sm.mode(i);
        };
        constexpr bool ALT = GEOM == 1 || SPLIT;
        const bool down = ALT && d.down != 0;
        const int lo = (ALT && d.seg_lo) ? d.seg_lo[seg] : 0, hi = lo + count;
        const int blo = lo & ~(NK_TILE - 1), bhi = count > 0 ? ((hi - 1) & ~(NK_TILE - 1)) : blo;
        const int nA = count > 0 ? (bhi - blo) / NK_TILE + 1 : 0;
        const int wlo = (!down && lo > (d.segcap - count) / 2) ? 0 : lo;
        NkOut<PID> O;
        O.init(L, wave);
        O.place(down ? base + hi - 1 : base + wlo, down ? -1 : 1, down ? count : d.segcap - wlo);
        int qn = SPLIT ? d.seg_evq[seg] : 0;
        if (SPLIT && lane == 0 && qn > 0) atomicAdd(&L.bins.misc[0], (unsigned int)qn);
        int cn = 0;
// ... 566 lines not shown
}

NK_KERNEL_LINKAGE __global__ __launch_bounds__(NK_WG) void k_regrow(NkDev o, NkDev n) {
    for (int seg = blockIdx.x; seg < o.nseg; seg += gridDim.x) {
        const int cnt = o.seg_count[seg];
        const int64_t a = (int64_t)seg * o.segcap, b = (int64_t)seg * n.segcap;
        for (int i = threadIdx.x; i < cnt; i += blockDim.x) {
            n.x[b + i] = o.x[a + i]; n.y[b + i] = o.y[a + i]; n.z[b + i] = o.z[a + i];
            n.occ[b + i] = o.occ[a + i]; if (o.nts && n.nts) n.nts[b + i] = o.nts[a + i];
            n.w0[b + i] = o.w0[a + i];
            if (o.pid && n.pid) n.pid[b + i] = o.pid[a + i];
        }
        if (threadIdx.x == 0) n.seg_count[seg] = cnt;
    }
}

NK_KERNEL_LINKAGE __global__ __launch_bounds__(NK_WG) void k_deliver(NkDev d, int in_step) {
    const int lane = threadIdx.x & 63, wave = __builtin_amdgcn_readfirstlane(threadIdx.x >> 6);
    const int nwaves = gridDim.x * (NK_WG / 64);
    for (int seg = blockIdx.x * (NK_WG / 64) + wave; seg < d.nseg; seg += nwaves) {
        int n = d.mig_n[seg];
        if (n <= 0) continue;
        if (n > d.mig_cap) n = d.mig_cap;
        const int count = d.seg_count[seg];
        const int lo = d.seg_lo ? d.seg_lo[seg] : 0;
        if (lo + count + n > d.segcap) { if (lane == 0 && !in_step) { atomicOr(d.halt + 2, 1); atomicOr(d.halt, 1); } continue; }
        const int64_t base = (int64_t)seg * d.segcap + lo + count;
        for (int j = lane; j < n; j += 64) {
            const double2 *r = d.mig_buf + ((int64_t)seg * d.mig_cap + j) * 4;
            const double2 a = r[0], b = r[1], c = r[2], e = r[3];
            d.x[base + j] = a.x; d.y[base + j] = a.y; d.z[base + j] = b.x; d.occ[base + j] = b.y; if (d.nts) d.nts[base + j] = c.x;
            d.pid[base + j] = (uint64_t)__double_as_longlong(c.y);
            d.w0[base + j] = (uint32_t)__double_as_longlong(e.x);
        }
        if (lane == 0) {
            d.seg_count[seg] = count + n;
            d.mig_n[seg] = 0;
            const int bound = d.R > 0 ? d.seg_bound[seg] : 0;
            if ((int64_t)lo + count + n + 2 * (bound + 2 * n) + NK_TILE > (int64_t)d.segcap) atomicOr(d.halt + 1, 1);
            if (2 * n > d.mig_cap) atomicOr(d.halt + 3, 1);
        }
    }
}

__device__ __forceinline__ void nk_update_sv(const NkDev &d, double Eraw, double Ns, double Told, int t, double Ta, double Tb, double Tz,
                                             double Ea, double Ez, double &Tnew_out, double &E_out) {
    const int n = d.nE;
        double norm;
        if (d.norm_fixed) norm = d.active_modes / (d.particle_density * d.sv_volume[t]);
        else { norm = d.active_modes / Ns; if (isnan(norm)) norm = 0.0; }
        double E = Eraw * norm / d.QV;
        int it = (int)((Told - Ta) / (Tb - Ta));
        it = it < 0 ? 0 : (it > n - 1 ? n - 1 : it);
        int base = it - 1;
        base = base < 0 ? 0 : (base > n - 4 ? n - 4 : base);
        double wT[4], wE[4];
#pragma unroll
        for (int j = 0; j < 4; ++j) { const int q = n >= 4 ? base + j : 0; wT[j] = d.Tarr[q]; wE[j] = d.Earr[q]; }
        double ref;
        if (Told < Ta) ref = Ea;
        else if (Told > Tz) ref = Ez;
        else if (n >= 4 && wT[0] < Told && !(wT[3] < Told)) {
            const int c = (wT[1] < Told) + (wT[2] < Told);
            const double xlo = c == 0 ? wT[0] : (c == 1 ? wT[1] : wT[2]), xhi = c == 0 ? wT[1] : (c == 1 ? wT[2] : wT[3]);
            const double ylo = c == 0 ? wE[0] : (c == 1 ? wE[1] : wE[2]), yhi = c == 0 ? wE[1] : (c == 1 ? wE[2] : wE[3]);
            ref = (yhi - ylo) / (xhi - xlo) * (Told - xlo) + ylo;
        } else { int io; ref = nk_interp_lin_hint(d.Tarr, d.Earr, n, Told, it, io); }
        E += ref;
        double Tnew;
        if (E < Ea) Tnew = d.Tfill_lo;
        else if (E > Ez) Tnew = d.Tfill_hi;
        else if (n >= 4 && wE[0] < E && !(wE[3] < E)) {
            const int c = (wE[1] < E) + (wE[2] < E);
            const double xlo = c == 0 ? wE[0] : (c == 1 ? wE[1] : wE[2]), xhi = c == 0 ? wE[1] : (c == 1 ? wE[2] : wE[3]);
            const double ylo = c == 0 ? wT[0] : (c == 1 ? wT[1] : wT[2]), yhi = c == 0 ? wT[1] : (c == 1 ? wT[2] : wT[3]);
            Tnew = (yhi - ylo) / (xhi - xlo) * (E - xlo) + ylo;
        } else { int io; Tnew = nk_interp_lin_hint(d.Earr, d.Tarr, n, E, it, io); }
        Tnew_out = Tnew;
        E_out = E;
}
__device__ __forceinline__ void nk_update_body(const NkDev &d, const double *acc, double *hist_row, int do_flux) {
    const int tid = threadIdx.x, nth = blockDim.x;
    const int S = d.S, NB = d.NB, n = d.nE;
    const double Ta = d.Tarr[0], Tb = d.Tarr[1], Tz = d.Tarr[n - 1], Ea = d.Earr[0], Ez = d.Earr[n - 1];
    for (int t = tid; t < S; t += nth) {
        double Tnew, E;
        nk_update_sv(d, acc[t], acc[S + t], d.T_ref_local ? d.T_sv[t] : d.T_ref, t, Ta, Tb, Tz, Ea, Ez, Tnew, E);
        hist_row[NB + t] = Tnew;
        hist_row[NB + S + t] = E;
        d.T_sv[t] = Tnew;
    }
    for (int b = tid; b < NB; b += nth) hist_row[b] = acc[b];
    if (d.sv_interp == 3) {
        __syncthreads();
        const int P = d.rbf_P;
        for (int j = tid; j < P; j += nth) {
            double a = 0.0;
            for (int i = 0; i < S; ++i) a += d.rbf_inv[(int64_t)j * P + i] * d.T_sv[i];
            d.T_sv[S + j] = a;
        }
    }
    if (d.res_gen == 2) for (int r = tid; r < d.R; r += nth) d.nleave_prev[r] = (int32_t)acc[5 * S + r];
    if (tid == 0) {
        hist_row[NB + 2 * S + 0] = (double)do_flux;
        hist_row[NB + 2 * S + 1] = 1.0;
        const bool hdel = acc[NB + 1] > 0.0;
        const bool hreq = acc[NB] > 0.0 || hdel;
        hist_row[NB + 2 * S + 2] = hreq ? 1.0 : 0.0;
        hist_row[NB + 2 * S + 3] = (double)*d.overflow;
        if (hreq) d.halt[0] = 1;
        if (hdel) d.halt[2] = 1;
        hist_row[NB + 2 * S + 4] = hreq ? 1.0 : 0.0;
        hist_row[NB + 2 * S + 5] = (double)d.halt[1];
        hist_row[NB + 2 * S + 6] = (hdel || d.halt[2]) ? 1.0 : 0.0;
        hist_row[NB + 2 * S + 7] = (double)d.halt[3];
    }
}

__device__ __forceinline__ void nk_reduce_body(const NkDev &d, int rows, double *acc, double *hist_row, int do_flux, int fuse, int b,
                                               int nblocks, double *sh, int &last) {
    if (d.halt[0]) return;
    const int NB = d.NB;
    double v = 0.0;
    for (int r = threadIdx.x; r < rows; r += NK_WG) v += d.partials[(int64_t)r * NB + b];
    sh[threadIdx.x] = v;
    __syncthreads();
    for (int o = NK_WG / 2; o > 0; o >>= 1) {
        if (threadIdx.x < o) sh[threadIdx.x] += sh[threadIdx.x + o];
        __syncthreads();
    }
    if (threadIdx.x == 0) acc[b] = sh[0];
    if (b == 0) {
        int stuck = 0;
        if (d.mig_n) for (int sg = threadIdx.x; sg < d.nseg; sg += NK_WG) { const int n = d.mig_n[sg]; stuck |= (n > 0 && d.seg_count[sg] + (n < d.mig_cap ? n : d.mig_cap) > d.segcap) ? 1 : 0; }
        stuck = __syncthreads_or(stuck);
        if (threadIdx.x == 0) { acc[NB] = (double)d.halt[1]; acc[NB + 1] = (double)stuck; }
    }
    if (!fuse) return;
    if (threadIdx.x == 0) {
        __threadfence();
        last = (atomicAdd(d.ticket, 1) == nblocks - 1);
    }
    __syncthreads();
    if (!last) return;
    if (threadIdx.x == 0) *d.ticket = 0;
    __threadfence();
    nk_update_body(d, acc, hist_row, do_flux);
}
NK_KERNEL_LINKAGE __global__ __launch_bounds__(NK_WG) void k_reduce(NkDev d, int rows, double *acc, double *hist_row, int do_flux, int fuse) {
    __shared__ double sh[NK_WG];
    __shared__ int last;
    nk_reduce_body(d, rows, acc, hist_row, do_flux, fuse, (int)blockIdx.x, (int)gridDim.x, sh, last);
}
template <int GEOM, bool BOX = false>
__global__ __launch_bounds__(NK_WG) void k_tail(NkDev d, uint32_t step_next, int rows, double *acc, double *hist_row, int do_flux, int fuse,
                                                int n_reduce) {
    extern __shared__ __align__(16) unsigned char smem[];
    if ((int)blockIdx.x < n_reduce) {
        double *sh = reinterpret_cast<double *>(smem);
        int &last = *reinterpret_cast<int *>(smem + NK_WG * sizeof(double));
        nk_reduce_body(d, rows, acc, hist_row, do_flux, fuse, (int)blockIdx.x, n_reduce, sh, last);
    } else {
        nk_emit_body<GEOM, BOX>(d, step_next, smem, (int)blockIdx.x - n_reduce, (int)gridDim.x - n_reduce, true);
    }
}

__device__ __forceinline__ bool nk_wait_word(const unsigned int *w, unsigned int atleast) {
    int spins = 0;
    while (__hip_atomic_load(w, __ATOMIC_RELAXED, __HIP_MEMORY_SCOPE_AGENT) < atleast) {
        __builtin_amdgcn_s_sleep(1);
        if (++spins > 1000000) return false;
    }
    return true;
}
template <bool BOX, bool PID, bool LREC>
__global__ __launch_bounds__(NK_WG, 2) void k_resident(NkDev d, uint32_t step0, int nsteps, int relax0, int flux_every, double *hist, int hrow,
                                                       unsigned int *bar) {
    extern __shared__ __align__(16) unsigned char smem[];
    if (d.halt[0]) return;
    NkLds L;
    nk_lds_setup<1, PID ? 5 : 4>(d, smem, L);
    const int tid = threadIdx.x, wg = (int)blockIdx.x, G = (int)gridDim.x;
    const int S = d.S, R = d.R, NB = d.NB, a = d.sv_axis;
    double *Tsv = const_cast<double *>(L.tb.Tsv);
    NkSv *sv = const_cast<NkSv *>(L.tb.sv);
    const int nE = d.nE;
    const double Ta = d.Tarr[0], Tb = d.Tarr[1], Tz = d.Tarr[nE - 1], Ea = d.Earr[0], Ez = d.Earr[nE - 1];
    unsigned int *flags = bar + 32, *flagsT = bar + 32 + 1024;
    unsigned long long *rows = reinterpret_cast<unsigned long long *>(d.partials);
    unsigned long long *Tpub = reinterpret_cast<unsigned long long *>(d.T_sv);
    const int NBP = (NB + 1) & ~1;
    unsigned long long *dbg = reinterpret_cast<unsigned long long *>(bar + 8);
#ifdef NK_STAMPS
    if (R > 0) nk_emit_segments<1, BOX>(d, L, step0, wg, G, false, 0ull, 0ull);
#else
    if (R > 0) nk_emit_segments<1, BOX>(d, L, step0, wg, G, false);
#endif
    for (int s = 0; s < nsteps; ++s) {
        const uint32_t step = step0 + (uint32_t)s;
        const int do_flux = (flux_every > 0 && ((step + 1u) % (uint32_t)flux_every) == 0u) ? 1 : 0;
        const bool mark = s == nsteps - 1 && tid == 0 && (wg == 0 || wg == G / 2);
        unsigned long long *mk = dbg + (wg == 0 ? 0 : 8);
        if (mark) mk[0] = __builtin_amdgcn_s_memrealtime();
#ifdef NK_STAMPS
        nk_sweep_body<1, false, false, PID, false, LREC, 0, BOX>(d, L, step, s == 0 ? relax0 : 1, do_flux, wg, G, 0ull);
#else
        nk_sweep_body<1, false, false, PID, false, LREC, 0, BOX>(d, L, step, s == 0 ? relax0 : 1, do_flux, wg, G);
#endif
        unsigned long long *rows_s = rows + (size_t)(s & 1) * G * NBP;
        __syncthreads();
        if (mark) mk[1] = __builtin_amdgcn_s_memrealtime();
        for (int b = tid; b < NB; b += NK_WG) {
            double v = 0.0;
            if (b < S) { for (int r = 0; r < NK_NREP; ++r) v += L.bins.E[r * S + b]; }
            else if (b < 2 * S) { unsigned int c = 0; for (int r = 0; r < NK_NREP; ++r) c += L.bins.N[r * S + (b - S)]; v = (double)c; }
            else if (b < 5 * S) { const int k = b - 2 * S; for (int r = 0; r < NK_NREP; ++r) v += L.bins.flux[r * 3 * S + k]; }
            else if (b < 5 * S + R) v = (double)L.bins.nleave[b - 5 * S];
            else if (b < 5 * S + 2 * R) v = L.bins.resb[4 * (b - 5 * S - R)];
            else if (b < 5 * S + 5 * R) { const int k = b - 5 * S - 2 * R; v = L.bins.resb[4 * (k / 3) + 1 + (k % 3)]; }
            else v = (double)L.bins.misc[0];
            __hip_atomic_store(rows_s + (size_t)wg * NBP + b, (unsigned long long)__double_as_longlong(v), __ATOMIC_RELAXED, __HIP_MEMORY_SCOPE_AGENT);
        }
        if (tid == 0 && NBP > NB) __hip_atomic_store(rows_s + (size_t)wg * NBP + NB, 0ull, __ATOMIC_RELAXED, __HIP_MEMORY_SCOPE_AGENT);
        asm volatile("s_waitcnt vmcnt(0) lgkmcnt(0)" ::: "memory");
        __builtin_amdgcn_fence(__ATOMIC_RELEASE, "workgroup");
        __syncthreads();
        if (tid == 0) __hip_atomic_store(flags + wg, (unsigned int)(s + 1), __ATOMIC_RELAXED, __HIP_MEMORY_SCOPE_AGENT);
        for (int i = tid; i < NK_NREP * S; i += NK_WG) { L.bins.E[i] = 0.0; L.bins.N[i] = 0u; }
        for (int i = tid; i < NK_NREP * 3 * S; i += NK_WG) L.bins.flux[i] = 0.0;
        for (int i = tid; i < 4 * R; i += NK_WG) L.bins.resb[i] = 0.0;
        for (int i = tid; i < R; i += NK_WG) L.bins.nleave[i] = 0u;
        if (tid == 0) L.bins.misc[0] = 0u;
        __syncthreads();
        if (mark && wg == 0) mk[2] = __builtin_amdgcn_s_memrealtime();
#ifdef NK_STAMPS
        if (R > 0 && s + 1 < nsteps) nk_emit_segments<1, BOX>(d, L, step + 1u, wg, G, true, 0ull, 0ull);
#else
        if (R > 0 && s + 1 < nsteps) nk_emit_segments<1, BOX>(d, L, step + 1u, wg, G, true);
#endif
        int ok = 1, hreq = 0;
        if (mark) mk[wg == 0 ? 3 : 2] = __builtin_amdgcn_s_memrealtime();
        double *hrowp = hist + (size_t)s * hrow;
        const int ntask = S + (NB - 2 * S);
        if (wg < ntask) {
            for (int g = tid; g < G; g += NK_WG) if (!nk_wait_word(flags + g, (unsigned int)(s + 1))) ok = 0;
            ok = __syncthreads_and(ok);
            if (!ok) {
                if (tid == 0) atomicOr(d.overflow, 256);
                return;
            }
            if (mark) mk[4] = __builtin_amdgcn_s_memrealtime();
            if (wg == 0) hreq = __hip_atomic_load(d.halt + 1, __ATOMIC_RELAXED, __HIP_MEMORY_SCOPE_AGENT);
            for (int k = wg; k < ntask; k += G) {
                const int c0 = k < S ? k : 2 * S + (k - S), c1 = k < S ? S + k : -1;
                double v0 = 0.0, v1 = 0.0;
                for (int g = tid; g < G; g += NK_WG) {
                    v0 += __longlong_as_double((long long)__hip_atomic_load(rows_s + (size_t)g * NBP + c0, __ATOMIC_RELAXED, __HIP_MEMORY_SCOPE_AGENT));
                    if (c1 >= 0) v1 += __longlong_as_double((long long)__hip_atomic_load(rows_s + (size_t)g * NBP + c1, __ATOMIC_RELAXED, __HIP_MEMORY_SCOPE_AGENT));
                }
                double *red = L.colsum;
                red[tid] = v0; red[NK_WG + tid] = v1;
                __syncthreads();
                for (int o = NK_WG / 2; o > 0; o >>= 1) {
                    if (tid < o) { red[tid] += red[tid + o]; red[NK_WG + tid] += red[NK_WG + tid + o]; }
                    __syncthreads();
                }
                if (tid == 0) {
                    const double t0 = red[0], t1 = red[NK_WG];
                    if (k < S) {
                        double Tnew, E;
                        nk_update_sv(d, t0, t1, d.T_ref_local ? Tsv[k] : d.T_ref, k, Ta, Tb, Tz, Ea, Ez, Tnew, E);
                        __hip_atomic_store(Tpub + k, (unsigned long long)__double_as_longlong(Tnew), __ATOMIC_RELAXED, __HIP_MEMORY_SCOPE_AGENT);
                        if (k == 0 && hreq) { d.halt[0] = 1; __hip_atomic_store(bar + 1, 1u, __ATOMIC_RELAXED, __HIP_MEMORY_SCOPE_AGENT); }
                        asm volatile("s_waitcnt vmcnt(0) lgkmcnt(0)" ::: "memory");
                        __hip_atomic_store(flagsT + k, (unsigned int)(s + 1), __ATOMIC_RELAXED, __HIP_MEMORY_SCOPE_AGENT);
                        hrowp[k] = t0; hrowp[S + k] = t1; hrowp[NB + k] = Tnew; hrowp[NB + S + k] = E;
                        if (k == 0) {
                            hrowp[NB + 2 * S + 0] = (double)do_flux;
                            hrowp[NB + 2 * S + 1] = 1.0;
                            hrowp[NB + 2 * S + 2] = hreq ? 1.0 : 0.0;
                            hrowp[NB + 2 * S + 3] = (double)__hip_atomic_load(d.overflow, __ATOMIC_RELAXED, __HIP_MEMORY_SCOPE_AGENT);
                            hrowp[NB + 2 * S + 4] = hreq ? 1.0 : 0.0;
                            hrowp[NB + 2 * S + 5] = (double)hreq;
                            hrowp[NB + 2 * S + 6] = (double)d.halt[2];
                            hrowp[NB + 2 * S + 7] = (double)d.halt[3];
                        }
                    } else hrowp[c0] = t0;
                }
                __syncthreads();
            }
            if (mark) mk[5] = __builtin_amdgcn_s_memrealtime();
        }
        for (int t = tid; t < S; t += NK_WG) {
            if (!nk_wait_word(flagsT + t, (unsigned int)(s + 1))) ok = 0;
            else Tsv[t] = __longlong_as_double((long long)__hip_atomic_load(Tpub + t, __ATOMIC_RELAXED, __HIP_MEMORY_SCOPE_AGENT));
        }
        ok = __syncthreads_and(ok);
        if (!ok) { if (tid == 0) atomicOr(d.overflow, 256); return; }
        if (wg != 0) hreq = (int)__hip_atomic_load(bar + 1, __ATOMIC_RELAXED, __HIP_MEMORY_SCOPE_AGENT);
        hreq = __syncthreads_or(hreq);
        if (mark) mk[wg == 0 ? 6 : 3] = __builtin_amdgcn_s_memrealtime();
        __builtin_amdgcn_s_dcache_inv();
        __syncthreads();
        for (int t = tid; t < S; t += NK_WG) {
            const int jn = t + 1 < S ? t + 1 : t;
            NkSv q;
            q.c = L.tb.cen[3 * t + a]; q.T = Tsv[t];
            q.slope = jn > t ? (Tsv[jn] - Tsv[t]) / (L.tb.cen[3 * jn + a] - L.tb.cen[3 * t + a]) : 0.0;
            q.invT = 1.0 / Tsv[t];
            sv[t] = q;
        }
        __syncthreads();
        if (hreq) return;
    }
}

// ... 882 lines not shown
```

Measured before the change: 53.44 billion.

## Add two-wave-per-segment emission, emit-only LDS setup for box, wide-multiply Philox

Adds an optional HALVES=2 emission mode in which two waves share one segment and split the emit tiles between them. The grid for that mode is sized from an occupancy query. For box meshes the emit kernel gets a slimmed LDS layout holding only the reservoir tables, which cuts LDS footprint and setup cost. Philox in the emit path now uses 64-bit products instead of umulhi plus mul. Halves mode is opt-in through an env var, while the emit-only LDS layout and wide Philox are on by default; overflow and rc_p write ownership are reassigned to half 0, which adds correctness risk.

```diff
diff --git a/nanokappa_amd/csrc/nk_device.h b/nanokappa_amd/csrc/nk_device.h
--- a/nanokappa_amd/csrc/nk_device.h
+++ b/nanokappa_amd/csrc/nk_device.h
@@ -184,12 +184,19 @@
     return s;
 }
 
+template <bool WIDE = false>
 __device__ __forceinline__ void nk_philox(uint32_t c0, uint32_t c1, uint32_t c2, uint32_t c3, uint32_t k0, uint32_t k1,
                                           uint32_t o[4]) {
 #pragma unroll
     for (int r = 0; r < 10; ++r) {
-        uint32_t hi0 = __umulhi(0xD2511F53u, c0), lo0 = 0xD2511F53u * c0;
-        uint32_t hi1 = __umulhi(0xCD9E8D57u, c2), lo1 = 0xCD9E8D57u * c2;
+        uint32_t hi0, lo0, hi1, lo1;
+        if (WIDE) {
+            const uint64_t p0 = (uint64_t)0xD2511F53u * c0, p1 = (uint64_t)0xCD9E8D57u * c2;
+            hi0 = (uint32_t)(p0 >> 32); lo0 = (uint32_t)p0; hi1 = (uint32_t)(p1 >> 32); lo1 = (uint32_t)p1;
+        } else {
+            hi0 = __umulhi(0xD2511F53u, c0); lo0 = 0xD2511F53u * c0;
+            hi1 = __umulhi(0xCD9E8D57u, c2); lo1 = 0xCD9E8D57u * c2;
+        }
         uint32_t n0 = hi1 ^ c1 ^ k0, n2 = hi0 ^ c3 ^ k1;
         c0 = n0; c1 = lo1; c2 = n2; c3 = lo0;
         k0 += 0x9E3779B9u; k1 += 0xBB67AE85u;
@@ -200,10 +207,11 @@
     uint64_t w = ((uint64_t)hi << 32) | lo;
     return (double)(w >> 11) * (1.0 / 9007199254740992.0);
 }
+template <bool WIDE = false>
 __device__ __forceinline__ void nk_uniform2_dev(uint64_t seed, uint64_t pid, uint32_t step, uint32_t tag, double &u0,
                                                 double &u1) {
     uint32_t o[4];
-    nk_philox((uint32_t)pid, (uint32_t)(pid >> 32), step, tag, (uint32_t)seed, (uint32_t)(seed >> 32), o);
+    nk_philox<WIDE>((uint32_t)pid, (uint32_t)(pid >> 32), step, tag, (uint32_t)seed, (uint32_t)(seed >> 32), o);
     u0 = nk_u53(o[0], o[1]);
     u1 = nk_u53(o[2], o[3]);
 }
diff --git a/nanokappa_amd/csrc/nk_engine.hip b/nanokappa_amd/csrc/nk_engine.hip
--- a/nanokappa_amd/csrc/nk_engine.hip
+++ b/nanokappa_amd/csrc/nk_engine.hip
@@ -65,6 +65,8 @@
     int g_sweep = 0;
     std::vector<int32_t> h_seg_count;
     std::vector<hipEvent_t> evpool;
+    int emit_occ[2] = {0, 0};
+    int64_t emit_occ_key[2] = {-1, -1};
     int g_sweep_key = -1;
     size_t g_sweep_lds = 0;
     int layout_key = -1;
@@ -231,11 +233,11 @@
         if (nk_geom_mode(ctx) == 1) kernel<1><<<grid, NK_WG, lds, ctx->stream>>>(__VA_ARGS__);         \
         else kernel<2><<<grid, NK_WG, lds, ctx->stream>>>(__VA_ARGS__);                                \
     } while (0)
-#define NK_EMIT_LAUNCH(kernel, grid, lds, ...)                                                        \
+#define NK_EMIT_LAUNCH(kernel, halves, grid, lds, ...)                                                \
     do {                                                                                               \
-        if (ctx->d.box) kernel<1, true><<<grid, NK_WG, lds, ctx->stream>>>(__VA_ARGS__);               \
-        else if (nk_geom_mode(ctx) == 1) kernel<1, false><<<grid, NK_WG, lds, ctx->stream>>>(__VA_ARGS__);   \
-        else kernel<2, false><<<grid, NK_WG, lds, ctx->stream>>>(__VA_ARGS__);                         \
+        if (ctx->d.box) { if ((halves) == 2) kernel<1, true, 2><<<grid, NK_WG, lds, ctx->stream>>>(__VA_ARGS__); else kernel<1, true, 1><<<grid, NK_WG, lds, ctx->stream>>>(__VA_ARGS__); }   \
+        else if (nk_geom_mode(ctx) == 1) { if ((halves) == 2) kernel<1, false, 2><<<grid, NK_WG, lds, ctx->stream>>>(__VA_ARGS__); else kernel<1, false, 1><<<grid, NK_WG, lds, ctx->stream>>>(__VA_ARGS__); }   \
+        else kernel<2, false, 1><<<grid, NK_WG, lds, ctx->stream>>>(__VA_ARGS__);                      \
     } while (0)
 static inline int nk_sweep_grid(const nk_ctx *ctx) { return ctx->num_cu * 8; }
 #define NK_SWEEP_CASE(G, R, B, P, S, lrec, STMT) { if (lrec) { auto KERNEL = k_sweep<G, R, B, P, S, true>; STMT; } else { auto KERNEL = k_sweep<G, R, B, P, S, false>; STMT; } }
@@ -1246,6 +1248,35 @@
     return ctx->g_sweep;
 }
 
+static inline int nk_emit_halves(const nk_ctx *ctx) {
+    if (!(ctx->d.box || nk_geom_mode(ctx) == 1) || ctx->d.res_gen == 2 || ctx->d.qx) return 1;
+    if (const char *e = getenv("NK_EMIT_HALVES")) { if (atoi(e) == 2) return 2; }
+    return 1;
+}
+static inline size_t nk_lds_emit(const nk_ctx *ctx) { return nk_lds(ctx, true, (ctx->d.box && NK_EMIT_LDS_ONLY) ? NK_LDS_EMIT_ONLY : 1); }
+static int nk_emit_occ(nk_ctx *ctx, size_t lds_t, bool group) {
+    const int w = group ? 1 : 0;
+    const int64_t key = (int64_t)lds_t * 4 + (ctx->d.box ? 1 : 0);
+    if (ctx->emit_occ[w] == 0 || ctx->emit_occ_key[w] != key) {
+        int per_cu = 0;
+        hipError_t e_;
+        if (group) e_ = nk_group_tail_occupancy((bool)ctx->d.box, lds_t, &per_cu);
+        else if (ctx->d.box) e_ = hipOccupancyMaxActiveBlocksPerMultiprocessor(&per_cu, k_tail<1, true, 2>, NK_WG, lds_t);
+        else e_ = hipOccupancyMaxActiveBlocksPerMultiprocessor(&per_cu, k_tail<1, false, 2>, NK_WG, lds_t);
+        if (e_ != hipSuccess || per_cu < 1) { (void)hipGetLastError(); per_cu = 1; }
+        if (per_cu > 8) per_cu = 8;
+        ctx->emit_occ[w] = per_cu;
+        ctx->emit_occ_key[w] = key;
+        if (getenv("NK_VERBOSE")) fprintf(stderr, "[nanokappa_hip] tail, two waves per segment: %d workgroups per CU (occupancy query rc %d), %zu B LDS each\n", per_cu, (int)e_, lds_t);
+    }
+    return ctx->emit_occ[w];
+}
+static int nk_emit_grid(nk_ctx *ctx, int halves, size_t lds_t, bool group) {
+    const int per = NK_WG / 64 / halves, need = (ctx->d.nseg + per - 1) / per;
+    const int cap = halves == 2 ? ctx->num_cu * nk_emit_occ(ctx, lds_t, group) : ctx->num_cu * 8;
+    return cap < need ? cap : need;
+}
+
 static inline int nk_mode_seg(const nk_ctx *ctx, int m, int nseg) {
     return (ctx->map_nseg == nseg && !ctx->h_m2s.empty()) ? ctx->h_m2s[(size_t)m] % nseg : m % nseg;
 }
@@ -1951,13 +1982,15 @@
     const int S = d.S, R = d.R, NB = d.NB;
     const int HROW = NB + 2 * S + 8;
     { int rch_ = nk_batch_hist(ctx, nsteps); if (rch_) return rch_; }
-    const size_t lds_g = nk_lds(ctx, true), lds_w = nk_lds(ctx, true, d.pid ? 3 : 2), lds_e = nk_lds(ctx, true, 1);
+    const size_t lds_g = nk_lds(ctx, true), lds_w = nk_lds(ctx, true, d.pid ? 3 : 2), lds_e = nk_lds_emit(ctx);
     const int gm_ = nk_geom_mode(ctx);
     const bool rough_ = d.Fr > 0, rbf_ = d.sv_interp == 3, pid_ = (bool)d.pid, split_ = d.qx != nullptr;
     const bool lrec_ = nk_want_lrec(ctx);
     (void)nk_sweep_blocks(ctx);
     const int g_sweep = ctx->g_sweep < (d.nseg + 3) / 4 ? ctx->g_sweep : (d.nseg + 3) / 4;
-    const int g_emit = ctx->num_cu * 8 < (d.nseg + 3) / 4 ? ctx->num_cu * 8 : (d.nseg + 3) / 4;
+    const int g_deliver = ctx->num_cu * 8 < (d.nseg + 3) / 4 ? ctx->num_cu * 8 : (d.nseg + 3) / 4;
+    const int halves = nk_emit_halves(ctx);
+    const int g_emit = nk_emit_grid(ctx, halves, lds_e > (size_t)(NK_WG * 8 + 16) ? lds_e : (size_t)(NK_WG * 8 + 16), false);
     const int g_ev = split_ ? ctx->num_cu * NK_EV_PER_CU : 0;
     size_t lds_ev = lds_g;
     d.tree_lds_fam0 = d.tree_nfam; d.tree_lds_off = 0;
@@ -2009,7 +2042,7 @@
         const int do_flux = (fe > 0 && ((stepno + 1) % fe) == 0) ? 1 : 0;
         if (s < nev) NK_HIP(hipEventRecord(ev[4 * s], ctx->stream));
         if (R > 0 && d.res_gen == 2) k_emit_one_to_one<<<ctx->num_cu * 4, NK_WG, 0, ctx->stream>>>(d, step);
-        if (R > 0 && !emitted_ahead) NK_EMIT_LAUNCH(k_emit, g_emit, lds_e, d, step);
+        if (R > 0 && !emitted_ahead) NK_EMIT_LAUNCH(k_emit, halves, g_emit, lds_e, d, step);
         if (s < nev) NK_HIP(hipEventRecord(ev[4 * s + 1], ctx->stream));
         {
             const int rl = pending ? 1 : 0;
@@ -2029,7 +2062,7 @@
                 k_events_end<<<(d.nseg + 255) / 256, 256, 0, ctx->stream>>>(d);
             }
         }
-        if (d.mig_buf) k_deliver<<<g_emit, NK_WG, 0, ctx->stream>>>(d, 1);
+        if (d.mig_buf) k_deliver<<<g_deliver, NK_WG, 0, ctx->stream>>>(d, 1);
         if (s < nev) NK_HIP(hipEventRecord(ev[4 * s + 2], ctx->stream));
         if (bands_ && do_flux) {
             int rcb_ = nk_band_pass(ctx, false, ctx->band_rows_d + band_s.size() * 4 * (size_t)S * ctx->band_B);
@@ -2054,13 +2087,13 @@
         double *hrow = ctx->hist + (size_t)s * HROW;
         const bool ahead = tail_emit;
         if (ctx->comm) {
-            if (ahead) NK_EMIT_LAUNCH(k_tail, NB + g_emit, lds_t, d, step + 1u, rows, ctx->acc, hrow, do_flux, 0, NB);
+            if (ahead) NK_EMIT_LAUNCH(k_tail, halves, NB + g_emit, lds_t, d, step + 1u, rows, ctx->acc, hrow, do_flux, 0, NB);
             else k_reduce<<<NB, NK_WG, 0, ctx->stream>>>(d, rows, ctx->acc, hrow, do_flux, 0);
             ncclResult_t nrc = ctx->rccl.AllReduce(ctx->acc, ctx->acc, (size_t)NB + 2, ncclDouble, ncclSum, ctx->comm, ctx->stream);
             if (nrc != ncclSuccess) { ctx->err = "ncclAllReduce failed"; return NK_ERR_COMM; }
             k_update<<<1, NK_WG, 0, ctx->stream>>>(d, ctx->acc, hrow, do_flux);
         } else if (ahead) {
-            NK_EMIT_LAUNCH(k_tail, NB + g_emit, lds_t, d, step + 1u, rows, ctx->acc, hrow, do_flux, 1, NB);
+            NK_EMIT_LAUNCH(k_tail, halves, NB + g_emit, lds_t, d, step + 1u, rows, ctx->acc, hrow, do_flux, 1, NB);
         } else {
             k_reduce<<<NB, NK_WG, 0, ctx->stream>>>(d, rows, ctx->acc, hrow, do_flux, 1);
         }
@@ -2542,7 +2575,7 @@
     }
     size_t lds_w = 0, lds_t = 0;
     for (int r = 0; r < R; ++r) {
-        const size_t w = nk_lds(m[r], true, m[r]->d.pid ? 3 : 2), e = nk_lds(m[r], true, 1);
+        const size_t w = nk_lds(m[r], true, m[r]->d.pid ? 3 : 2), e = nk_lds_emit(m[r]);
         const size_t tl = e > (size_t)(NK_WG * 8 + 16) ? e : (size_t)(NK_WG * 8 + 16);
         if (w > 64 * 1024 || tl > 64 * 1024) { err = "nk_group: member " + std::to_string(r) + " is outside the grouped path: its tables need more than 64 KB of LDS"; return NK_ERR_ARG; }
         lds_w = std::max(lds_w, w); lds_t = std::max(lds_t, tl);
@@ -2636,7 +2669,7 @@
     NkDev *devs = reinterpret_cast<NkDev *>(g->stage + sizeof(NkGroupHead));
     for (int k = 0; k <= NK_GROUP_MAX; ++k) head->pre_sweep[k] = head->pre_tail[k] = INT32_MAX;
     for (int k = 0; k < NK_GROUP_MAX; ++k) head->rows[k] = 0;
-    head->NB = NB; head->pad_ = 0;
+    head->NB = NB;
     if (nsteps > g->recs_cap) {
         if (g->recs_d) hipFree(g->recs_d);
         if (g->recs_h) hipHostFree(g->recs_h);
@@ -2646,6 +2679,8 @@
         NK_GHIP(hipHostMalloc((void **)&g->recs_h, (size_t)cap * R * sizeof(NkGroupRec), hipHostMallocDefault));
         g->recs_cap = cap;
     }
+    const int halves = nk_emit_halves(g->m[0]);
+    head->emit_halves = halves;
     struct Member { int g_sweep = 0, g_emit = 0; bool alt = false, pending = false, relax0 = false, flushed0 = false, emitted_ahead = false, tail_emit = false; };
     std::vector<Member> mem((size_t)R);
     int grid_sweep = 0, grid_tail = 0;
@@ -2657,7 +2692,7 @@
         (void)nk_sweep_blocks(ctx);
         me.g_sweep = ctx->g_sweep < (d.nseg + 3) / 4 ? ctx->g_sweep : (d.nseg + 3) / 4;
         me.tail_emit = d.R > 0;
-        me.g_emit = me.tail_emit ? (ctx->num_cu * 8 < (d.nseg + 3) / 4 ? ctx->num_cu * 8 : (d.nseg + 3) / 4) : 0;
+        me.g_emit = me.tail_emit ? nk_emit_grid(ctx, halves, lds_t, true) : 0;
         d.tree_lds_fam0 = d.tree_nfam; d.tree_lds_off = 0;
         me.relax0 = me.pending = ctx->pending_relax;
         me.emitted_ahead = me.tail_emit && ctx->emitted_for == ctx->step;
@@ -2713,7 +2748,7 @@
                 if (fl_ && s == 0) me.flushed0 = true;
             }
             if (d.R > 0 && !me.emitted_ahead) {
-                NK_EMIT_LAUNCH(k_emit, me.g_emit, nk_lds(ctx, true, 1), d, (uint32_t)stepno);
+                NK_EMIT_LAUNCH(k_emit, halves, me.g_emit, nk_lds_emit(ctx), d, (uint32_t)stepno);
                 g->rep.member_launches += 1;
             }
             if (me.alt) ctx->walked = true;
diff --git a/nanokappa_amd/csrc/nk_group.h b/nanokappa_amd/csrc/nk_group.h
--- a/nanokappa_amd/csrc/nk_group.h
+++ b/nanokappa_amd/csrc/nk_group.h
@@ -11,7 +11,7 @@
     int32_t pre_tail[NK_GROUP_MAX + 1];
     int32_t rows[NK_GROUP_MAX];
     int32_t NB;
-    int32_t pad_;
+    int32_t emit_halves;
 };
 struct NkGroupRec {
     uint32_t step;
@@ -27,3 +27,4 @@
 hipError_t nk_group_launch_sweep_fast(const NkGroupKind &k, int grid, size_t lds, hipStream_t stream, const NkGroupHead *head, const NkDev *devs,
                                       const NkGroupRec *recs);
 hipError_t nk_group_launch_tail(bool box, int grid, size_t lds, hipStream_t stream, const NkGroupHead *head, const NkDev *devs, const NkGroupRec *recs);
+hipError_t nk_group_tail_occupancy(bool box, size_t lds, int *blocks);
diff --git a/nanokappa_amd/csrc/nk_group.hip b/nanokappa_amd/csrc/nk_group.hip
--- a/nanokappa_amd/csrc/nk_group.hip
+++ b/nanokappa_amd/csrc/nk_group.hip
@@ -72,7 +72,8 @@
         int &last = *reinterpret_cast<int *>(smem + NK_WG * sizeof(double));
         nk_reduce_body(d, head->rows[r], rec->acc, rec->hist_row, rec->do_flux, 1, wg, n_reduce, sh, last);
     } else {
-        nk_emit_body<1, BOX>(d, rec->step + 1u, smem, wg - n_reduce, nwg - n_reduce, true);
+        if (head->emit_halves == 2) nk_emit_body<1, BOX, 2>(d, rec->step + 1u, smem, wg - n_reduce, nwg - n_reduce, true);
+        else nk_emit_body<1, BOX, 1>(d, rec->step + 1u, smem, wg - n_reduce, nwg - n_reduce, true);
     }
 }
 
@@ -95,5 +96,9 @@
     else k_tail_group<false><<<grid, NK_WG, lds, stream>>>(head, devs, recs);
     return hipGetLastError();
 }
+hipError_t nk_group_tail_occupancy(bool box, size_t lds, int *blocks) {
+    if (box) return hipOccupancyMaxActiveBlocksPerMultiprocessor(blocks, k_tail_group<true>, NK_WG, lds);
+    return hipOccupancyMaxActiveBlocksPerMultiprocessor(blocks, k_tail_group<false>, NK_WG, lds);
+}
 
 #endif
diff --git a/nanokappa_amd/csrc/nk_kernels.h b/nanokappa_amd/csrc/nk_kernels.h
--- a/nanokappa_amd/csrc/nk_kernels.h
+++ b/nanokappa_amd/csrc/nk_kernels.h
@@ -61,8 +61,20 @@
 #ifndef NK_BOX_GENERAL_CAST
 #define NK_BOX_GENERAL_CAST 0
 #endif
+#ifndef NK_EMIT_WIDE_PHILOX
+#define NK_EMIT_WIDE_PHILOX 1
+#endif
+#ifndef NK_EMIT_LDS_ONLY
+#define NK_EMIT_LDS_ONLY 1
+#endif
+#define NK_LDS_EMIT_ONLY 6
 #define NK_COLSUM_DOUBLES 768
 __host__ __device__ inline size_t nk_lds_bytes(int S, int R, int F, int NP, int Fc, int geom, int kind, int nrf, int rbfP, int nlrec = 0, int carry = 0) {
+    if (kind == NK_LDS_EMIT_ONLY) {
+        const size_t nd6 = 2 * (size_t)R + 10 * (size_t)nrf + 2 * (size_t)(NK_WG / 64) * NK_EMIT_CHUNK + 4;
+        const size_t by6 = nd6 * 8 + (size_t)(R + 1 + 3 * (NK_WG / 64) * NK_EMIT_CHUNK) * 4 + 32;
+        return (by6 + 15) & ~(size_t)15;
+    }
     const bool emit = kind == 1 || kind >= 4;
     int Fl = geom == 1 ? F : 0;
     int Pl = Fl ? NP : 0;
@@ -190,6 +202,42 @@
     __syncthreads();
 }
 
+template <int GEOM>
+__device__ __forceinline__ int nk_lds_setup_emit(const NkDev &d, unsigned char *smem, NkLds &L) {
+    const int R = d.R;
+    const int nrf = (GEOM == 1 && d.res_lds) ? d.res_nf : 0;
+    double *p = (double *)smem;
+    double *resT = p; p += 2 * R;
+    double *rf_cdf = p; p += nrf;
+    double *rf_verts = p; p += 9 * (size_t)nrf;
+    L.sp_cv = p; p += (NK_WG / 64) * NK_EMIT_CHUNK;
+    L.sp_pr = p; p += (NK_WG / 64) * NK_EMIT_CHUNK;
+    unsigned int *u = (unsigned int *)p;
+    int *rf_off = (int *)u; u += R + 1;
+    L.sp_pref = u; u += (NK_WG / 64) * NK_EMIT_CHUNK;
+    L.sp_cnt = u; u += (NK_WG / 64) * NK_EMIT_CHUNK;
+    L.sp_rm = u; u += (NK_WG / 64) * NK_EMIT_CHUNK;
+    L.resT = resT; L.rf_off = rf_off; L.rf_cdf = rf_cdf; L.rf_verts = rf_verts;
+    const int t = threadIdx.x, nth = blockDim.x;
+    const int halted = d.halt[0];
+    const double l_rT = t < R ? d.res_T[t] : 1.0;
+    const int l_off = (nrf > 0 && t <= R) ? d.res_face_off[t] : 0;
+    const double l_cdf = t < nrf ? d.res_face_cdf[t] : 0.0;
+    const double l_vert = t < 9 * nrf ? d.res_face_verts[t] : 0.0;
+    if (t < R) { resT[2 * t] = l_rT; resT[2 * t + 1] = 1.0 / l_rT; }
+    if (nrf > 0 && t <= R) rf_off[t] = l_off;
+    if (t < nrf) rf_cdf[t] = l_cdf;
+    if (t < 9 * nrf) rf_verts[t] = l_vert;
+    for (int i = t + nth; i < R; i += nth) { const double T = d.res_T[i]; resT[2 * i] = T; resT[2 * i + 1] = 1.0 / T; }
+    if (nrf > 0) {
+        for (int i = t + nth; i <= R; i += nth) rf_off[i] = d.res_face_off[i];
+        for (int i = t + nth; i < nrf; i += nth) rf_cdf[i] = d.res_face_cdf[i];
+        for (int i = t + nth; i < 9 * nrf; i += nth) rf_verts[i] = d.res_face_verts[i];
+    }
+    __syncthreads();
+    return halted;
+}
+
 __device__ __forceinline__ void nk_lds_flush(const NkDev &d, const NkLds &L, int64_t row) {
     __syncthreads();
     const int S = d.S, R = d.R;
@@ -264,17 +312,17 @@
         else nk_find_boundary((L).planes, (L).faces, (d).NP, (d).tol, x, y, z, vx, vy, vz, tc, fc);                   \
     } while (0)
 
-__device__ __forceinline__ void nk_emit_entry(const NkDev &d, uint32_t step, int64_t rm, int64_t at, double prob, int &c, int &c_mine, double &cv) {
+__device__ __forceinline__ void nk_emit_entry(const NkDev &d, uint32_t step, int64_t rm, int64_t at, double prob, int &c, int &c_mine, double &cv, bool write = true) {
     const double fixed = floor(prob);
     int mask;
     if (d.res_gen == 0) {
         cv = d.rc_p[(int64_t)(step & 1u) * d.rc_len + at] + (prob - fixed);
         mask = cv >= 1.0;
         cv -= (double)mask;
-        d.rc_p[(int64_t)((step + 1u) & 1u) * d.rc_len + at] = cv;
+        if (write) d.rc_p[(int64_t)((step + 1u) & 1u) * d.rc_len + at] = cv;
     } else {
         double d1;
-        nk_uniform2_dev(d.seed, (uint64_t)rm | 0xFFFFFFFF00000000ull, step, NK_TAG_DICE, cv, d1);
+        nk_uniform2_dev<NK_EMIT_WIDE_PHILOX != 0>(d.seed, (uint64_t)rm | 0xFFFFFFFF00000000ull, step, NK_TAG_DICE, cv, d1);
         mask = cv <= (prob - fixed);
     }
     c = (int)fixed + mask;
@@ -315,10 +363,10 @@
     nts = tc / d.dt - dt_in / d.dt;
 }
 
-template <int GEOM, bool BOX>
+template <int GEOM, bool BOX, int HALVES = 1>
 __device__ __forceinline__ int nk_emit_one(const NkDev &d, const NkLds &L, uint32_t step, int seg, int lane, unsigned int *sp_pref,
                                            unsigned int *sp_cnt, unsigned int *sp_rm, double *sp_cv, double *sp_pr, bool ahead, bool to_queue,
-                                           int &bound_out
+                                           int &bound_out, int h = 0
 #ifdef NK_STAMPS
                                            , unsigned long long em_t0, unsigned long long em_t1, unsigned long long &em_t2
 #endif
@@ -350,7 +398,7 @@
                     const int64_t rm = (int64_t)r * d.M + sm.entry_mode(l);
                     const int64_t at = ((int64_t)seg * d.R + r) * d.nlmax + l;
                     prob = d.ep_p[at];
-                    nk_emit_entry(d, step, rm, at, prob, c, cmine, cv);
+                    nk_emit_entry(d, step, rm, at, prob, c, cmine, cv, HALVES == 1 || h == 0);
                     rm32 = (unsigned int)rm;
                     sp_bound += ((int)floor(prob) + 1 + d.nranks - 1) / d.nranks;
                 }
@@ -370,7 +418,7 @@
 #ifdef NK_STAMPS
         if (!em_t2) em_t2 = __builtin_amdgcn_s_memrealtime();
 #endif
-        for (int spj = 0; spj < spn; spj += NK_TILE) {
+        for (int spj = HALVES == 2 ? h * NK_TILE : 0; spj < spn; spj += HALVES * NK_TILE) {
             const int j = spj + lane;
             if (j >= spn) continue;
             int64_t rm;
@@ -409,8 +457,8 @@
             const uint64_t pid = level > 0 ? ((uint64_t)((step + 1u) & 0xFFFFFFu) << 40) | ((uint64_t)rm << 12) | (uint64_t)level
                                            : ((uint64_t)((step + 1u) & 0xFFFFFFu) << 40) | ((uint64_t)r << 32) | o2o;
             double uf, us, ur, ut;
-            nk_uniform2_dev(d.seed, pid, step, NK_TAG_EMIT, uf, us);
-            nk_uniform2_dev(d.seed, pid, step, NK_TAG_EMIT + 1, ur, ut);
+            nk_uniform2_dev<NK_EMIT_WIDE_PHILOX != 0>(d.seed, pid, step, NK_TAG_EMIT, uf, us);
+            nk_uniform2_dev<NK_EMIT_WIDE_PHILOX != 0>(d.seed, pid, step, NK_TAG_EMIT + 1, ur, ut);
             const double iprob = level > 0 ? nk_rcp(prob) : 0.0;
             const double dt_in = (level == 0) ? d.dt * ut
                                : (level == 1) ? d.dt * (1.0 - cval * iprob)
@@ -453,7 +501,7 @@
                 if (!BOX) d.nts.p[q.od] = na;
                 d.w0.p[q.ow] = BOX ? (NK_NEWBORN | (uint32_t)idx) : (NK_NEWBORN | ((uint32_t)(facet + 1) << d.lb) | (uint32_t)idx);
                 if (d.pid) d.pid.p[q.od] = pid;
-            } else if (!(ahead && d.halt[1])) atomicOr(d.overflow, 1);
+            } else if (HALVES == 1 && !(ahead && d.halt[1])) atomicOr(d.overflow, 1);
         }
         made += spn;
         __builtin_amdgcn_fence(__ATOMIC_SEQ_CST, "wavefront");
@@ -462,7 +510,8 @@
     for (int o = 32; o > 0; o >>= 1) sp_bound += __shfl_xor(sp_bound, o, 64);
     const int room = d.segcap - plo - count;
     const int put = (GEOM == 2 && to_queue) ? 0 : (made < room ? made : (room > 0 ? room : 0));
-    if (lane == 0) {
+    if (HALVES == 2 && h == 0 && lane == 0 && made > 0 && made > room && !(ahead && d.halt[1])) atomicOr(d.overflow, 1);
+    if (lane == 0 && (HALVES == 1 || h == 0)) {
         if (GEOM == 2 && to_queue) { d.seg_new[seg] = 0; d.seg_evq[seg] = made < d.segcap ? made : d.segcap; }
         else d.seg_new[seg] = put;
         d.seg_bound[seg] = sp_bound;
@@ -475,7 +524,7 @@
     return put;
 }
 
-template <int GEOM, bool BOX = false>
+template <int GEOM, bool BOX = false, int HALVES = 1>
 __device__ __forceinline__ void nk_emit_segments(const NkDev &d, NkLds L, uint32_t step, int bid, int nblocks, bool ahead
 #ifdef NK_STAMPS
                                                  , unsigned long long em_t0, unsigned long long em_t1
@@ -488,37 +537,43 @@
     unsigned int *sp_pref = L.sp_pref + wave * NK_EMIT_CHUNK, *sp_cnt = L.sp_cnt + wave * NK_EMIT_CHUNK,
                  *sp_rm = L.sp_rm + wave * NK_EMIT_CHUNK;
     double *sp_cv = L.sp_cv + wave * NK_EMIT_CHUNK, *sp_pr = L.sp_pr + wave * NK_EMIT_CHUNK;
-    const int nwaves = nblocks * (NK_WG / 64);
+    static_assert(HALVES == 1 || (HALVES == 2 && GEOM == 1), "two waves per segment: small meshes only");
+    const int nwaves = nblocks * (NK_WG / 64 / HALVES);
+    const int h = HALVES == 2 ? (wave & 1) : 0;
     const bool to_queue = GEOM == 2 && d.NG > 0 && d.qx != nullptr;
-    for (int seg = bid * (NK_WG / 64) + wave; seg < d.nseg; seg += nwaves) {
+    for (int seg = bid * (NK_WG / 64 / HALVES) + wave / HALVES; seg < d.nseg; seg += nwaves) {
         int bound_;
 #ifdef NK_STAMPS
-        (void)nk_emit_one<GEOM, BOX>(d, L, step, seg, lane, sp_pref, sp_cnt, sp_rm, sp_cv, sp_pr, ahead, to_queue, bound_, em_t0, em_t1, em_t2);
+        (void)nk_emit_one<GEOM, BOX, HALVES>(d, L, step, seg, lane, sp_pref, sp_cnt, sp_rm, sp_cv, sp_pr, ahead, to_queue, bound_, h, em_t0, em_t1, em_t2);
 #else
-        (void)nk_emit_one<GEOM, BOX>(d, L, step, seg, lane, sp_pref, sp_cnt, sp_rm, sp_cv, sp_pr, ahead, to_queue, bound_);
-#endif
-    }
-}
-
-template <int GEOM, bool BOX = false>
+        (void)nk_emit_one<GEOM, BOX, HALVES>(d, L, step, seg, lane, sp_pref, sp_cnt, sp_rm, sp_cv, sp_pr, ahead, to_queue, bound_, h);
+#endif
+    }
+}
+
+template <int GEOM, bool BOX = false, int HALVES = 1>
 __device__ __forceinline__ void nk_emit_body(const NkDev &d, uint32_t step, unsigned char *smem, int bid, int nblocks, bool ahead = false) {
 #ifdef NK_STAMPS
     const unsigned long long em_t0 = __builtin_amdgcn_s_memrealtime();
 #endif
-    if (d.halt[0]) return;
     NkLds L;
-    nk_lds_setup<GEOM, 1>(d, smem, L);
-#ifdef NK_STAMPS
-    nk_emit_segments<GEOM, BOX>(d, L, step, bid, nblocks, ahead, em_t0, __builtin_amdgcn_s_memrealtime());
+    if (BOX && NK_EMIT_LDS_ONLY) {
+        if (nk_lds_setup_emit<GEOM>(d, smem, L)) return;
+    } else {
+        if (d.halt[0]) return;
+        nk_lds_setup<GEOM, 1>(d, smem, L);
+    }
+#ifdef NK_STAMPS
+    nk_emit_segments<GEOM, BOX, HALVES>(d, L, step, bid, nblocks, ahead, em_t0, __builtin_amdgcn_s_memrealtime());
 #else
-    nk_emit_segments<GEOM, BOX>(d, L, step, bid, nblocks, ahead);
-#endif
-}
-
-template <int GEOM, bool BOX = false>
+    nk_emit_segments<GEOM, BOX, HALVES>(d, L, step, bid, nblocks, ahead);
+#endif
+}
+
+template <int GEOM, bool BOX = false, int HALVES = 1>
 __global__ __launch_bounds__(NK_WG) void k_emit(NkDev d, uint32_t step) {
     extern __shared__ __align__(16) unsigned char smem[];
-    nk_emit_body<GEOM, BOX>(d, step, smem, (int)blockIdx.x, (int)gridDim.x);
+    nk_emit_body<GEOM, BOX, HALVES>(d, step, smem, (int)blockIdx.x, (int)gridDim.x);
 }
 
 template <bool PID>
@@ -1391,7 +1446,7 @@
     __shared__ int last;
     nk_reduce_body(d, rows, acc, hist_row, do_flux, fuse, (int)blockIdx.x, (int)gridDim.x, sh, last);
 }
-template <int GEOM, bool BOX = false>
+template <int GEOM, bool BOX = false, int HALVES = 1>
 __global__ __launch_bounds__(NK_WG) void k_tail(NkDev d, uint32_t step_next, int rows, double *acc, double *hist_row, int do_flux, int fuse,
                                                 int n_reduce) {
     extern __shared__ __align__(16) unsigned char smem[];
@@ -1400,7 +1455,7 @@
         int &last = *reinterpret_cast<int *>(smem + NK_WG * sizeof(double));
         nk_reduce_body(d, rows, acc, hist_row, do_flux, fuse, (int)blockIdx.x, n_reduce, sh, last);
     } else {
-        nk_emit_body<GEOM, BOX>(d, step_next, smem, (int)blockIdx.x - n_reduce, (int)gridDim.x - n_reduce, true);
+        nk_emit_body<GEOM, BOX, HALVES>(d, step_next, smem, (int)blockIdx.x - n_reduce, (int)gridDim.x - n_reduce, true);
     }
 }
 
```

Result: no change. 53.50 billion, median of 3 (+0.1%).
